# Symb0x76/ChineseChessZero

Hardware: AMD Instinct MI355X
Metric: self-play MCTS simulations/sec (higher is better)
Workload: dtype u8 rules / f32 Q (reference CPU path) / f64 PUCT (net: fp16)

## Files before the change

chinesechesszero_amd/_lib.py:

```python
from __future__ import annotations

import ctypes as C
import os

import torch

_HERE = os.path.dirname(os.path.abspath(__file__))
LIB_PATH = os.path.join(_HERE, "libcczero.so")

NSQ = 90
SQ_STRIDE = 96
NMOVES = 2086
MAX_LEGAL = 128
MASK_WORDS = 66
PLANES = 10710
REC_BYTES, REC_HDR, REC_IDS, REC_PI = 880, 96, 112, 368
REC_FLAGS, REC_FAST = 103, 1
REC_RESIGNED, REC_PLAYON, REC_VALUE = 2, 4, 8
REC_VALUE_OFF = 92
RESIGN_RESIGNED, RESIGN_PLAYON = 2, 4
HEAD_POL_STRIDE, HEAD_VAL_STRIDE = 1536, 640

ABI_VERSION = 9
CONV_RELU, CONV_DESCENDING, CONV_FORCE_SMALL, CONV_FORCE_TILE, CONV_G16, CONV_G16_EDGE_TILES = 1, 2, 16, 32, 64, 128
CONV_G16_ONE_LAUNCH = 512
CONV_G16_QUAD = 1 << 16
RULE_PERPETUAL_CHECK = 1
RULE_PAWN_MOVE_RESETS_CLOCK = 2
FLAG_REFERENCE_QUIRKS = 1
FLAG_NO_MIRROR = 2
FLAG_VALUE_F16 = 4
FLAG_CACHE_VERIFY = 8
ERR_PRUNED, ERR_TRUNCATED = 256, 512
ERR_BAD_TEMP = 1024
FLAG_STRICT = 16
LEAF_EXPAND, LEAF_DRAW, LEAF_LOSS, LEAF_SKIP = 0, 1, 2, 3
LEAF_WIN = 4
PROOF_UNKNOWN, PROOF_WIN, PROOF_LOSS, PROOF_DRAW = 0, 1, 2, 3

ERR_BITS = {1: "node pool exhausted (raise max_nodes)", 2: "selection path deeper than max_depth", 64: "history chain overflow (> 128 positions since the last capture)",
            4: "more than 128 legal moves or pseudo-move overflow", 8: "pi record arena overflow",
            16: "forced move is not a legal move of the root, or nothing searched and nothing forced (that board neither recorded nor moved)", 32: "NaN priors",
            128: "index out of bounds (bounds-checked diagnostic build)",
            256: "strict mode: a kept subtree was pruned to fit the node pool (the reference's tree is unbounded: raise max_nodes)",
            512: "strict mode: a game was adjudicated at max_plies (the reference's game has no ply cap: raise max_plies)",
            1024: "a per-board temperature was NaN or <= 0 (that board neither recorded nor moved)"}


class CczError(RuntimeError):
    pass


class Config(C.Structure):
    _fields_ = [
        ("n_boards", C.c_int32), ("n_playout", C.c_int32), ("c_puct", C.c_float), ("eps", C.c_float),
        ("alpha", C.c_float), ("temp", C.c_float), ("max_nodes", C.c_int32), ("max_depth", C.c_int32),
        ("max_plies", C.c_int32), ("flags", C.c_uint32), ("seed", C.c_uint64), ("board_id_base", C.c_uint64),
        ("device", C.c_int32), ("reserve_nodes", C.c_int32),
        ("move_rank_host", C.c_void_p), ("plane_of_type", C.c_uint8 * 8), ("rule_flags", C.c_uint32), ("eval_cache_log2", C.c_uint32),
        ("type_rank", C.c_uint8 * 8),
    ]


class Stats(C.Structure):
    _fields_ = [
        ("sims", C.c_int64), ("moves", C.c_int64), ("games", C.c_int64), ("truncated_games", C.c_int64),
        ("nodes_peak", C.c_int64), ("depth_peak", C.c_int64), ("sum_depth", C.c_int64), ("sum_children", C.c_int64),
        ("expansions", C.c_int64), ("terminal_leaves", C.c_int64), ("error_flags", C.c_int32), ("reserved", C.c_int32),
        ("hbm_bytes", C.c_int64), ("pruned_subtrees", C.c_int64),
        ("cache_probes", C.c_int64), ("cache_hits", C.c_int64), ("cache_shared_rows", C.c_int64), ("cache_stores", C.c_int64),
        ("cache_verified", C.c_int64), ("cache_verify_mismatches", C.c_int64),
    ]


class ResignStats(C.Structure):
    _fields_ = [("resigned_games", C.c_int64), ("resigned_by_red", C.c_int64), ("resigned_plies", C.c_int64), ("playon_games", C.c_int64),
                ("playon_won", C.c_int64), ("playon_drawn", C.c_int64), ("playon_plies_after", C.c_int64)]


class ExplorationStats(C.Structure):
    _fields_ = [("explored_moves", C.c_int64), ("forced_selections", C.c_int64), ("visits_pruned", C.c_int64), ("children_pruned", C.c_int64)]


class GumbelStats(C.Structure):
    _fields_ = [("gumbel_moves", C.c_int64), ("considered_sum", C.c_int64), ("offvisit_moves", C.c_int64)]


class SearchCfg(C.Structure):
    _fields_ = [("enabled", C.c_int32), ("fpu_mode", C.c_int32), ("fpu_root_mode", C.c_int32), ("reserved", C.c_int32),
                ("fpu_value", C.c_double), ("fpu_root_value", C.c_double), ("c_base", C.c_double), ("c_factor", C.c_double)]


class WideStats(C.Structure):
    _fields_ = [("steps", C.c_int64), ("leaves", C.c_int64), ("collisions", C.c_int64), ("inflight_now", C.c_int64)]


class SolverStats(C.Structure):
    _fields_ = [("nodes_proven", C.c_int64), ("proven_stops", C.c_int64), ("roots_proven", C.c_int64)]


_P = C.c_void_p
PROTOTYPES = {
    "ccz_abi_version": (C.c_int, []),
    "ccz_last_error": (C.c_char_p, []),
    "ccz_device_count": (C.c_int, []),
    "ccz_action_table": (C.c_int, [_P, _P, _P]),
    "ccz_flip_map": (C.c_int, [_P]),
    "ccz_create": (C.c_int, [C.POINTER(Config), C.POINTER(_P)]),
    "ccz_destroy": (C.c_int, [_P]),
    "ccz_reset": (C.c_int, [_P, _P, _P]),
    "ccz_set_position": (C.c_int, [_P, _P, C.c_int32, _P, C.c_int32, C.c_int32]),
    "ccz_set_positions": (C.c_int, [_P, _P, _P, _P, _P, _P, _P, C.c_int32, _P, _P]),
    "ccz_reset_tree": (C.c_int, [_P, _P, _P]),
    "ccz_select_leaves": (C.c_int, [_P, _P, _P]),
    "ccz_zero_leaf_input": (C.c_int, [_P, _P, _P]),
    "ccz_expand_backup": (C.c_int, [_P, _P, _P, _P]),
    "ccz_step": (C.c_int, [_P, _P, _P, _P, _P]),
    "ccz_gather_priors": (C.c_int, [_P, _P, _P, C.c_int32]),
    "ccz_step_compact": (C.c_int, [_P, _P, _P, _P]),
    "ccz_expand_backup_compact": (C.c_int, [_P, _P, _P]),
    "ccz_eval_plan": (C.c_int, [_P, _P, _P, _P]),
    "ccz_set_scouts": (C.c_int, [_P, C.c_int32]),
    "ccz_scout": (C.c_int, [_P, _P, _P]),
    "ccz_eval_plan_scouted": (C.c_int, [_P, _P, _P, _P, _P]),
    "ccz_scout_and_plan": (C.c_int, [_P, _P, _P, _P, _P, _P]),
    "ccz_scouted_run": (C.c_int, [_P, _P, _P, _P, _P, _P, _P]),
    "ccz_gather_priors_planned": (C.c_int, [_P, _P, _P, C.c_int32, _P]),
    "ccz_eval_cache_clear": (C.c_int, [_P, _P]),
    "ccz_set_routing": (C.c_int, [_P, _P, _P, C.c_uint64, C.c_uint64]),
    "ccz_eval_plan_routed": (C.c_int, [_P, _P, _P, _P]),
    "ccz_gather_priors_routed": (C.c_int, [_P, _P, _P, _P, C.c_int32, _P, _P]),
    "ccz_set_budgets": (C.c_int, [_P, _P, _P, _P]),
    "ccz_draw_budgets": (C.c_int, [_P, _P, C.c_int32, C.c_int32, C.c_double, _P]),
    "ccz_set_resign": (C.c_int, [_P, _P, C.c_int32, C.c_float, C.c_int32, C.c_int32, C.c_double]),
    "ccz_get_resign_stats": (C.c_int, [_P, _P, C.POINTER(ResignStats)]),
    "ccz_resign_status": (C.c_int, [_P, _P, _P, _P, _P, _P]),
    "ccz_set_root_exploration": (C.c_int, [_P, _P, C.c_int32, C.c_double, C.c_double, C.c_double, C.c_int32]),
    "ccz_get_exploration_stats": (C.c_int, [_P, _P, C.POINTER(ExplorationStats)]),
    "ccz_root_noise": (C.c_int, [_P, _P, _P, _P]),
    "ccz_set_gumbel": (C.c_int, [_P, _P, C.c_int32, C.c_int32, C.c_int32, C.c_double, C.c_double]),
    "ccz_get_gumbel_stats": (C.c_int, [_P, _P, C.POINTER(GumbelStats)]),
    "ccz_gumbel_root": (C.c_int, [_P, _P, _P, _P, _P, _P, _P]),
    "ccz_gumbel_sequence": (C.c_int, [_P, C.c_int32, C.c_int32, _P]),
    "ccz_set_search": (C.c_int, [_P, _P, C.c_int32, C.c_int32, C.c_double, C.c_int32, C.c_double, C.c_double, C.c_double]),
    "ccz_get_search": (C.c_int, [_P, _P, C.POINTER(SearchCfg)]),
    "ccz_set_solver": (C.c_int, [_P, _P, C.c_int32]),
    "ccz_root_proof": (C.c_int, [_P, _P, _P, _P, _P, _P]),
    "ccz_get_solver_stats": (C.c_int, [_P, _P, C.POINTER(SolverStats)]),
    "ccz_proof_combine": (C.c_int, [_P, _P, _P, C.c_int32, _P]),
    "ccz_set_width": (C.c_int, [_P, _P, C.c_int32]),
    "ccz_select_wide": (C.c_int, [_P, _P, _P, _P]),
    "ccz_step_wide": (C.c_int, [_P, _P, _P, _P, _P]),
    "ccz_get_wide_stats": (C.c_int, [_P, _P, C.POINTER(WideStats)]),
    "ccz_finish_move": (C.c_int, [_P, _P, _P, _P, _P, C.c_int32]),
    "ccz_root_children": (C.c_int, [_P, _P, _P, _P, _P, _P, _P, _P]),
    "ccz_principal_variations": (C.c_int, [_P, _P, C.c_int32, C.c_int32, _P, _P, _P, _P, _P, _P]),
    "ccz_root_pi": (C.c_int, [_P, _P, _P, _P]),
    "ccz_move_distribution": (C.c_int, [_P, _P, _P, _P, _P, _P]),
    "ccz_game_status": (C.c_int, [_P, _P, _P, _P, _P, _P]),
    "ccz_root_positions": (C.c_int, [_P, _P, _P]),
    "ccz_leaf_info": (C.c_int, [_P, _P, _P, _P, _P, _P]),
    "ccz_leaf_priors": (C.c_int, [_P, _P, _P, _P]),
    "ccz_leaf_keys": (C.c_int, [_P, _P, _P, _P]),
    "ccz_harvest_rows": (C.c_int, [_P, _P, C.POINTER(C.c_int64)]),
    "ccz_harvest": (C.c_int, [_P, _P, _P, _P, _P, C.c_int64, C.POINTER(C.c_int64)]),
    "ccz_harvest_records": (C.c_int, [_P, _P, _P, C.c_int64, C.POINTER(C.c_int64)]),
    "ccz_expand_records": (C.c_int, [_P, _P, C.c_int64, C.c_uint32, _P, _P, _P, _P, C.c_int64, C.c_int64, _P, _P, _P]),
    "ccz_ring_retire": (C.c_int, [_P, _P, C.c_int64, _P, C.c_int64, C.c_int32, _P]),
    "ccz_sample_records": (C.c_int, [_P, _P, C.c_int64, _P, _P, C.c_int64, C.c_uint32, _P, _P, _P, _P, _P, _P, _P]),
    "ccz_get_stats": (C.c_int, [_P, _P, C.POINTER(Stats)]),
    "ccz_legal_moves": (C.c_int, [_P, C.c_int32, _P, _P, _P, _P, _P, _P]),
    "ccz_apply_moves": (C.c_int, [_P, C.c_int32, _P, _P, _P, _P]),
    "ccz_bias_act_f16": (C.c_int, [_P, _P, _P, _P, C.c_int64, C.c_int32]),
    "ccz_conv3x3_c256_f16": (C.c_int, [_P, _P, _P, _P, _P, _P, C.c_int64, C.c_int32]),
    "ccz_conv3x3_stem_f16": (C.c_int, [_P, _P, _P, _P, _P, C.c_int64, C.c_int32]),
    "ccz_pack_live_planes_f16": (C.c_int, [_P, _P, _P, C.c_int32]),
    "ccz_pack_live_planes_rows_f16": (C.c_int, [_P, _P, _P, C.c_int32, _P, _P]),
    "ccz_pack_live_planes_g16_f16": (C.c_int, [_P, _P, _P, C.c_int32, _P, _P]),
    "ccz_pack_conv_weights_g16_f16": (C.c_int, [_P, _P, _P, C.c_int32]),
    "ccz_conv3x3_c256_f16_live": (C.c_int, [_P, _P, _P, _P, _P, _P, C.c_int64, C.c_int32, _P, C.c_int32, C.c_int32]),
    "ccz_conv3x3_stem_f16_live": (C.c_int, [_P, _P, _P, _P, _P, C.c_int64, C.c_int32, _P, C.c_int32, C.c_int32]),
    "ccz_conv3x3_c256_heads_f16": (C.c_int, [_P, _P, _P, _P, _P, _P, _P, _P, _P, C.c_int64, C.c_int32, _P, C.c_int32, C.c_int32]),
    "ccz_heads_conv1x1_f16": (C.c_int, [_P, _P, _P, _P, _P, _P, C.c_int32, C.c_int32, _P]),
    "ccz_fc_f16": (C.c_int, [_P, _P, C.c_int32, _P, _P, _P, C.c_int32, C.c_int32, C.c_int32, C.c_int32, C.c_int32, _P]),
    "ccz_value_out_f32": (C.c_int, [_P, _P, _P, C.c_float, _P, C.c_int32, _P]),
}

_lib = None


def source_hash() -> str | None:
    import glob
    import hashlib
    csrc = os.path.join(_HERE, "csrc")
    files = sorted(glob.glob(os.path.join(csrc, "*.h")) + glob.glob(os.path.join(csrc, "*.hip")), key=os.path.basename)
    files.append(os.path.join(os.path.dirname(_HERE), "include", "cczero.h"))
    if len(files) < 2 or not all(os.path.exists(f) for f in files):
        return None
    h = hashlib.sha256()
    for f in files:
        with open(f, "rb") as fh:
            h.update(fh.read())
    return h.hexdigest()[:16]


def stale_build() -> str | None:
    if LIB_PATH != os.path.join(_HERE, "libcczero.so"):
        return None
    want = source_hash()
    if want is None:
        return None
    stamp = LIB_PATH + ".srchash"
    if not os.path.exists(stamp):
        return f"{LIB_PATH} carries no source stamp ({stamp} is missing): it was not built by the current Makefile"
    with open(stamp) as f:
        got = f.read().strip()
    if got != want:
        return f"{LIB_PATH} was built from other sources (stamp {got}, the tree hashes to {want}): a kernel was edited after the last build"
    return None


def lib() -> C.CDLL:
    global _lib
    if _lib is None:
        if not os.path.exists(LIB_PATH):
            raise CczError(
                f"{LIB_PATH} is missing: build it with `python -c 'import __graft_entry__ as g; g.build()'` "
                "(hipcc --offload-arch=gfx950). The engine has no CPU fallback.")
        why = stale_build()
        if why:
            raise CczError(why + " -- rebuild with `python -c 'import __graft_entry__ as g; g.build()'`")
        L = C.CDLL(LIB_PATH)
        for name, (res, args) in PROTOTYPES.items():
            fn = getattr(L, name)
            fn.restype = res
            fn.argtypes = args
        if L.ccz_abi_version() != ABI_VERSION:
            raise CczError("libcczero.so ABI version mismatch")
        _lib = L
    return _lib


def check(rc: int) -> None:
    if rc != 0:
        raise CczError(f"libcczero error {rc}: {lib().ccz_last_error().decode(errors='replace')}")
```

chinesechesszero_amd/csrc/cczero.hip:

```cpp
#include "../../include/cczero.h"

#include <hip/hip_runtime.h>

#include <cmath>
#include <cstdarg>
#include <cstdio>
#include <cstdlib>
#include <cstring>
#include <new>
#include <vector>

#include "cczero_kernels.h"
#include "cczero_netops.h"
#include "cczero_conv.h"
#include "cczero_conv_small.h"
#include "cczero_conv_g16.h"
#include "cczero_conv_g16e.h"
#include "cczero_heads.h"

using namespace ccz;

namespace {

thread_local char g_err[512] = "";
// ... 1250 lines not shown
    HIP_TRY(hipStreamSynchronize(s));
    return 0;
}

int ccz_leaf_info(ccz_engine *e, void *stream, uint8_t *status_host, int32_t *k_host, uint16_t *ids_host, int32_t *depth_host)
{
    NEED(e);
    hipStream_t s = (hipStream_t)stream;
    const size_t B = (size_t)e->d.B;
    if (status_host) HIP_TRY(hipMemcpyAsync(status_host, e->d.leaf_status, B, hipMemcpyDeviceToHost, s));
    if (k_host) HIP_TRY(hipMemcpyAsync(k_host, e->d.leaf_k, B * 4, hipMemcpyDeviceToHost, s));
    if (ids_host) HIP_TRY(hipMemcpyAsync(ids_host, e->d.leaf_ids, B * kMaxLegal * 2, hipMemcpyDeviceToHost, s));
    if (depth_host) HIP_TRY(hipMemcpyAsync(depth_host, e->d.path_len, B * 4, hipMemcpyDeviceToHost, s));
    HIP_TRY(hipStreamSynchronize(s));
    return 0;
}

int ccz_leaf_priors(ccz_engine *e, void *stream, float *prior_host, float *value_host)
{
    NEED(e);
    hipStream_t s = (hipStream_t)stream;
    const size_t B = (size_t)e->d.B;
    if (value_host && !e->d.cache) return fail(-1, "ccz_leaf_priors: engine-owned leaf values exist only with an evaluation cache (pass value_host = NULL)");
    if (prior_host) HIP_TRY(hipMemcpyAsync(prior_host, e->d.prior128, B * kMaxLegal * 4, hipMemcpyDeviceToHost, s));
    if (value_host) HIP_TRY(hipMemcpyAsync(value_host, e->d.vleaf, B * 4, hipMemcpyDeviceToHost, s));
    HIP_TRY(hipStreamSynchronize(s));
    return 0;
}

int ccz_leaf_keys(ccz_engine *e, void *stream, uint64_t *keys_dev, uint8_t *status_dev)
{
    NEED(e);
    hipStream_t s = (hipStream_t)stream;
    if (keys_dev) HIP_TRY(hipMemcpyAsync(keys_dev, e->d.leaf_key, (size_t)e->d.B * 8, hipMemcpyDeviceToDevice, s));
    if (status_dev) HIP_TRY(hipMemcpyAsync(status_dev, e->d.leaf_status, (size_t)e->d.B, hipMemcpyDeviceToDevice, s));
    return 0;
}

int ccz_harvest_rows(ccz_engine *e, void *stream, int64_t *rows_host)
{
    NEED(e);
    if (!rows_host) return fail(-1, "ccz_harvest_rows: null output");
    const int rc = fetch_meta(e, (hipStream_t)stream);
    if (rc) return rc;
    const int mul = (e->d.flags & CCZ_FLAG_NO_MIRROR) ? 1 : 2;
    int64_t rows = 0;
    for (int b = 0; b < e->d.B; ++b)
        if (e->h_meta[b].over) rows += (int64_t)e->h_meta[b].ply * mul;
    *rows_host = rows;
    return 0;
}

struct HarvestPlan {
    std::vector<long long> base;
    std::vector<uint8_t> mask;
    int64_t total = 0;
    bool any = false;
};

static int plan_harvest(ccz_engine *e, hipStream_t s, int mul, int64_t capacity, const char *first_fmt, HarvestPlan &p)
{
    const int rc = fetch_meta(e, s);
    if (rc) return rc;
    const int B = e->d.B;
    p.base.assign((size_t)B, -1);
    p.mask.assign((size_t)B, 0);
    for (int b = 0; b < B; ++b)
        if (e->h_meta[b].over && e->h_meta[b].ply > 0) {
            const int64_t add = (int64_t)e->h_meta[b].ply * mul;
            if (p.total + add > capacity) {
                if (!p.any) return fail(-5, first_fmt, (long long)add, (long long)capacity);
                break;
            }
            p.base[b] = p.total;
            p.mask[b] = 1;
            p.any = true;
            p.total += add;
        }
    return 0;
}

static int restart_harvested(ccz_engine *e, hipStream_t s, const HarvestPlan &p)
{
    HIP_TRY(hipMemcpyAsync(e->st_mask, p.mask.data(), (size_t)e->d.B, hipMemcpyHostToDevice, s));
    hipLaunchKernelGGL(k_reset, dim3(e->d.B), dim3(64), 0, s, e->d, (const uint8_t *)e->st_mask);
    HIP_TRY(hipGetLastError());
    HIP_TRY(hipStreamSynchronize(s));
    return 0;
}

int ccz_harvest(ccz_engine *e, void *stream, void *states_f16_dev, float *pi_dev, float *z_dev, int64_t capacity_rows,
                int64_t *rows_host)
{
    NEED(e);
    hipStream_t s = (hipStream_t)stream;
    HarvestPlan p;
    const int rc = plan_harvest(e, s, (e->d.flags & CCZ_FLAG_NO_MIRROR) ? 1 : 2, capacity_rows,
                                "ccz_harvest: the first finished game needs %lld rows, capacity %lld", p);
    if (rc) return rc;
    if (rows_host) *rows_host = p.total;
    if (!p.any) return 0;
    if (p.total > 0) {
        if (!states_f16_dev || !pi_dev || !z_dev) return fail(-1, "ccz_harvest: null output buffer");
        HIP_TRY(hipMemcpyAsync(e->st_rowbase, p.base.data(), (size_t)e->d.B * 8, hipMemcpyHostToDevice, s));
        hipLaunchKernelGGL(k_harvest, dim3(e->d.B, kHarvestSlices), dim3(256), 0, s, e->d, (const long long *)e->st_rowbase,
                           (uint16_t *)states_f16_dev, pi_dev, z_dev);
        HIP_TRY(hipGetLastError());
    }
    return restart_harvested(e, s, p);
}

int ccz_harvest_records(ccz_engine *e, void *stream, void *records_dev, int64_t capacity_plies, int64_t *plies_host)
{
    NEED(e);
    hipStream_t s = (hipStream_t)stream;
    HarvestPlan p;
    if (const int rc = plan_harvest(e, s, 1, capacity_plies, "ccz_harvest_records: the first finished game has %lld plies, capacity %lld", p)) return rc;
    if (plies_host) *plies_host = p.total;
    if (!p.any) return 0;
    if (p.total > 0) {
        if (!records_dev) return fail(-1, "ccz_harvest_records: null output buffer");
        HIP_TRY(hipMemcpyAsync(e->st_rowbase, p.base.data(), (size_t)e->d.B * 8, hipMemcpyHostToDevice, s));
        hipLaunchKernelGGL(k_harvest_records, dim3(e->d.B, kHarvestSlices), dim3(256), 0, s, e->d, (const long long *)e->st_rowbase, (uint8_t *)records_dev);
        HIP_TRY(hipGetLastError());
    }
    return restart_harvested(e, s, p);
}

static int typepack_of(const char *who, const uint8_t *plane_of_type_host, uint32_t *typepack)
{
    uint8_t pot[8] = {0, 0, 1, 2, 3, 4, 5, 6};
    if (plane_of_type_host) {
        bool all_zero = true;
        for (int t = 0; t < 8; ++t) all_zero = all_zero && plane_of_type_host[t] == 0;
        if (!all_zero) {
            unsigned seen = 0;
            for (int t = 1; t <= 7; ++t) {
                const int c = plane_of_type_host[t];
                if (c > 6 || (seen >> c & 1u)) return fail(-1, "%s: plane_of_type[1..7] must be a permutation of 0..6", who);
                seen |= 1u << c;
                pot[t] = (uint8_t)c;
            }
        }
    }
    *typepack = 0;
    for (int t = 1; t <= 7; ++t) *typepack |= (uint32_t)(t - 1) << (3 * pot[t]);
    return 0;
}

static int check_expand_args(const char *who, const void *records_dev, int64_t n_plies, uint32_t flags, const void *states_f16_dev, const float *value_dev,
                             int64_t ring_rows, int64_t head_row)
{
    if (!records_dev) return fail(-1, "%s: null buffer", who);
    if (((uintptr_t)records_dev | (uintptr_t)states_f16_dev) & 3) return fail(-1, "%s: buffers must be 4-byte aligned", who);
    if ((uintptr_t)value_dev & 3) return fail(-1, "%s: the values must be 4-byte aligned", who);
    if (n_plies > (int64_t)INT32_MAX) return fail(-1, "%s: too many records for one launch", who);
    const int64_t rows = n_plies * ((flags & CCZ_FLAG_NO_MIRROR) ? 1 : 2);
    if (ring_rows > 0 && rows > ring_rows) return fail(-1, "%s: %lld rows do not fit a ring of %lld", who, (long long)rows, (long long)ring_rows);
    if (ring_rows == 0 && head_row != 0) return fail(-1, "%s: head_row needs ring_rows", who);
    return 0;
}

static int check_sample_args(const char *who, const void *ring_dev, const int64_t *window_dev, const int64_t *draws_dev, int64_t batch,
                             const void *states_f16_dev, const float *pi_dev, const float *z_dev, const float *value_dev)
{
    if (!ring_dev || !window_dev || !draws_dev || !states_f16_dev || !pi_dev || !z_dev) return fail(-1, "%s: null buffer", who);
    if (((uintptr_t)ring_dev | (uintptr_t)states_f16_dev) & 3) return fail(-1, "%s: buffers must be 4-byte aligned", who);
    if ((uintptr_t)value_dev & 3) return fail(-1, "%s: the values must be 4-byte aligned", who);
    if (((uintptr_t)window_dev | (uintptr_t)draws_dev) & 7) return fail(-1, "%s: window and draws must be 8-byte aligned", who);
    if (batch > (int64_t)INT32_MAX) return fail(-1, "%s: too many rows for one launch", who);
    return 0;
}

int ccz_expand_records(void *stream, const void *records_dev, int64_t n_plies, uint32_t flags, const uint8_t *plane_of_type_host,
                       void *states_f16_dev, float *pi_dev, float *z_dev, int64_t ring_rows, int64_t head_row, int32_t *bad_records_dev,
                       uint8_t *target_dev, float *value_dev)
{
    const char *who = "ccz_expand_records";
    if (n_plies < 0 || ring_rows < 0 || head_row < 0) return fail(-1, "%s: negative size", who);
    if (n_plies == 0) return 0;
    const int dense = (states_f16_dev != nullptr) + (pi_dev != nullptr) + (z_dev != nullptr);
    if (dense != 3 && !(dense == 0 && (target_dev || value_dev))) return fail(-1, "%s: null buffer", who);
    if (const int rc = check_expand_args(who, records_dev, n_plies, flags, states_f16_dev, value_dev, ring_rows, head_row)) return rc;
    uint32_t typepack = 0;
    if (const int rc = typepack_of(who, plane_of_type_host, &typepack)) return rc;
    hipLaunchKernelGGL(k_expand_records, dim3((unsigned)n_plies), dim3(256), 0, (hipStream_t)stream, (const uint8_t *)records_dev, (long long)n_plies,
                       flags & (CCZ_FLAG_REFERENCE_QUIRKS | CCZ_FLAG_NO_MIRROR), typepack, (uint16_t *)states_f16_dev, pi_dev, z_dev,
                       (long long)ring_rows, (long long)head_row, bad_records_dev, target_dev, value_dev);
    HIP_TRY(hipGetLastError());
    return 0;
}

int ccz_ring_retire(void *stream, const void *ring_dev, int64_t cap_plies, int64_t *window_dev, int64_t head_new, int32_t max_game_plies,
                    int32_t *bad_records_dev)
{
    if (cap_plies <= 0 || head_new < 0) return fail(-1, "ccz_ring_retire: capacity must be positive and head_new non-negative");
    if (max_game_plies <= 0 || max_game_plies > 65535) return fail(-1, "ccz_ring_retire: max_game_plies must be 1..65535 (the header's T is 16 bits)");
    if (cap_plies < 2 * (int64_t)max_game_plies) return fail(-1, "ccz_ring_retire: a ring of %lld plies is smaller than two games of %d", (long long)cap_plies, max_game_plies);
    if (!ring_dev || !window_dev) return fail(-1, "ccz_ring_retire: null buffer");
    if (((uintptr_t)ring_dev & 3) || ((uintptr_t)window_dev & 7)) return fail(-1, "ccz_ring_retire: the ring must be 4-byte, the window 8-byte aligned");
    hipLaunchKernelGGL(k_ring_retire, dim3(1), dim3(64), 0, (hipStream_t)stream, (const uint8_t *)ring_dev, (long long)cap_plies,
                       (long long *)window_dev, (long long)head_new, (int)max_game_plies, bad_records_dev);
    HIP_TRY(hipGetLastError());
    return 0;
}

int ccz_sample_records(void *stream, const void *ring_dev, int64_t cap_plies, const int64_t *window_dev, const int64_t *draws_dev, int64_t batch,
                       uint32_t flags, const uint8_t *plane_of_type_host, void *states_f16_dev, float *pi_dev, float *z_dev, int32_t *bad_records_dev,
                       uint8_t *target_dev, float *value_dev)
{
    const char *who = "ccz_sample_records";
    if (cap_plies <= 0 || batch < 0) return fail(-1, "%s: capacity must be positive and batch non-negative", who);
    if (batch == 0) return 0;
    if (const int rc = check_sample_args(who, ring_dev, window_dev, draws_dev, batch, states_f16_dev, pi_dev, z_dev, value_dev)) return rc;
    uint32_t typepack = 0;
    if (const int rc = typepack_of(who, plane_of_type_host, &typepack)) return rc;
    hipLaunchKernelGGL(k_sample_records, dim3((unsigned)batch), dim3(256), 0, (hipStream_t)stream, (const uint8_t *)ring_dev, (long long)cap_plies,
                       (const long long *)window_dev, (const long long *)draws_dev, (long long)batch,
                       flags & (CCZ_FLAG_REFERENCE_QUIRKS | CCZ_FLAG_NO_MIRROR), typepack, (uint16_t *)states_f16_dev, pi_dev, z_dev, bad_records_dev,
                       target_dev, value_dev);
    HIP_TRY(hipGetLastError());
    return 0;
}

int ccz_get_stats(ccz_engine *e, void *stream, ccz_stats *out)
{
    NEED(e);
    if (!out) return fail(-1, "ccz_get_stats: null output");
    hipStream_t s = (hipStream_t)stream;
    std::vector<BoardStats> st((size_t)e->d.B);
    int32_t err[2] = {0, 0};
    HIP_TRY(hipMemcpyAsync(st.data(), e->d.stats, st.size() * sizeof(BoardStats), hipMemcpyDeviceToHost, s));
    HIP_TRY(hipMemcpyAsync(err, e->d.err, 8, hipMemcpyDeviceToHost, s));
    HIP_TRY(hipStreamSynchronize(s));
    memset(out, 0, sizeof *out);
    for (const BoardStats &b : st) {
        out->sims += (int64_t)b.sims;
        out->moves += (int64_t)b.moves;
        out->games += (int64_t)b.games;
        out->truncated_games += (int64_t)b.truncated;
        out->sum_depth += (int64_t)b.sum_depth;
        out->sum_children += (int64_t)b.sum_children;
        out->expansions += (int64_t)b.expansions;
        out->terminal_leaves += (int64_t)b.terminal;
        out->pruned_subtrees += (int64_t)b.pruned;
        out->cache_probes += (int64_t)b.cache_probes;
        out->cache_hits += (int64_t)b.cache_hits;
        out->cache_shared_rows += (int64_t)b.cache_shared;
        out->cache_stores += (int64_t)b.cache_stores;
        out->cache_verified += (int64_t)b.cache_verified;
        out->cache_verify_mismatches += (int64_t)b.cache_mismatch;
        if (b.nodes_peak > out->nodes_peak) out->nodes_peak = b.nodes_peak;
        if (b.depth_peak > out->depth_peak) out->depth_peak = b.depth_peak;
    }
    out->error_flags = err[0];
    out->reserved = err[1];
    out->hbm_bytes = (int64_t)e->bytes;
    return 0;
}

int ccz_legal_moves(void *stream, int32_t n, const uint8_t *sq_dev, const uint8_t *turn_dev, const int32_t *halfmove_dev,
                    uint32_t *mask_dev, int32_t *count_dev, uint8_t *flags_dev)
{
    if (n < 0 || !sq_dev || !turn_dev) return fail(-1, "ccz_legal_moves: bad arguments");
    if (n == 0) return 0;
    hipLaunchKernelGGL(k_legal_moves, dim3(n), dim3(64), 0, (hipStream_t)stream, n, sq_dev, turn_dev, halfmove_dev, mask_dev,
                       count_dev, flags_dev);
    HIP_TRY(hipGetLastError());
    return 0;
}

int ccz_apply_moves(void *stream, int32_t n, uint8_t *sq_dev, uint8_t *turn_dev, const int32_t *move_ids_dev, uint8_t *captured_dev)
{
    if (n < 0 || !sq_dev || !turn_dev || !move_ids_dev) return fail(-1, "ccz_apply_moves: bad arguments");
    if (n == 0) return 0;
    hipLaunchKernelGGL(k_apply_moves, dim3((n + 255) / 256), dim3(256), 0, (hipStream_t)stream, n, sq_dev, turn_dev, move_ids_dev,
                       captured_dev);
    HIP_TRY(hipGetLastError());
    return 0;
}

int ccz_bias_act_f16(void *stream, void *y_dev, const void *bias_dev, const void *residual_dev, int64_t rows, int32_t channels)
{
    if (!y_dev || !bias_dev || rows < 0 || channels <= 0 || (channels & 7)) return fail(-1, "ccz_bias_act_f16: bad arguments (channels must be a multiple of 8)");
    if ((((uintptr_t)y_dev) | ((uintptr_t)bias_dev) | ((uintptr_t)residual_dev)) & 15) return fail(-1, "ccz_bias_act_f16: pointers must be 16-byte aligned");
    const long n_vec = rows * (long)(channels / 8);
    if (n_vec == 0) return 0;
    long blocks = (n_vec + 255) / 256;
    if (blocks > 4096) blocks = 4096;
    if (residual_dev)
        hipLaunchKernelGGL(k_bias_act<true>, dim3((unsigned)blocks), dim3(256), 0, (hipStream_t)stream, (half8_t *)y_dev, (const half8_t *)bias_dev,
                           (const half8_t *)residual_dev, n_vec, channels / 8);
    else
        hipLaunchKernelGGL(k_bias_act<false>, dim3((unsigned)blocks), dim3(256), 0, (hipStream_t)stream, (half8_t *)y_dev, (const half8_t *)bias_dev,
                           (const half8_t *)nullptr, n_vec, channels / 8);
    HIP_TRY(hipGetLastError());
    return 0;
}

static_assert(((int64_t)INT32_MAX / kCvC) * kCvC * 2 <= (int64_t)UINT32_MAX, "the largest accepted activation tensor must fit 32-bit byte offsets / num_records");
constexpr int64_t kSmallMaxPixels = 64 * 90;

static int conv3x3_launch(const char *who, void *stream, const void *x_dev, const void *w_dev, const void *bias_f32_dev, const void *residual_dev, void *y_dev,
                          int64_t n_pixels, int32_t relu, int cin, const int32_t *live_rows_dev = nullptr, int32_t row0 = 0)
{
    if (!x_dev || !w_dev || !bias_f32_dev || !y_dev || n_pixels < 0 || n_pixels % 90 || n_pixels > (int64_t)INT32_MAX / kCvC)
        return fail(-1, "%s: bad arguments (n_pixels must be boards * 90, at most 93206 boards per call)", who);
    if ((((uintptr_t)x_dev) | ((uintptr_t)w_dev) | ((uintptr_t)bias_f32_dev) | ((uintptr_t)residual_dev) | ((uintptr_t)y_dev)) & 15)
        return fail(-1, "%s: pointers must be 16-byte aligned", who);
    if (x_dev == y_dev) return fail(-1, "%s: the output may alias the residual but not the input", who);
    if (n_pixels == 0) return 0;
    if (relu & CCZ_CONV_G16) {
        if (relu & (256 | (0xffe << 16)))
            return fail(-1, "%s: flag 256 / bits 17..27 were CCZ_CONV_G16_PERSISTENT, retired in ABI 8", who);
        if (n_pixels % 1440) return fail(-1, "%s: CCZ_CONV_G16 needs a multiple of 16 boards", who);
        const int groups = (int)(n_pixels / 1440);
        const int fl = relu & 3;
        hipStream_t s = (hipStream_t)stream;
        const G16Shape shape = g16_shape(groups, relu);
        const G16Args a = {(const _Float16 *)x_dev, (const _Float16 *)w_dev, (const float *)bias_f32_dev, (const _Float16 *)residual_dev, (_Float16 *)y_dev,
                           (int)n_pixels, cin, (const int *)live_rows_dev, (int)row0};
        const bool res = residual_dev != nullptr;
        if (cin == 64) {
            hipLaunchKernelGGL(k_conv3x3_g16_stem, dim3((unsigned)(groups * 5)), dim3(512), 0, s, (const _Float16 *)x_dev, (const _Float16 *)w_dev,
                               (const float *)bias_f32_dev, (_Float16 *)y_dev, (int)n_pixels, (int)fl, cin, (const int *)live_rows_dev, (int)row0);
            HIP_TRY(hipGetLastError());
            return 0;
        }
        if (!shape.edge) {
            g16_launch(CCZ_G16_RES(k_conv3x3_g16, res), shape.mid, s, a, fl);
            HIP_TRY(hipGetLastError());
            return 0;
        }
        const bool quad = (relu & CCZ_CONV_G16_QUAD) != 0;
        if (relu & CCZ_CONV_G16_ONE_LAUNCH) {
            g16_launch(quad ? CCZ_G16_RES(k_conv3x3_g16_one_quad, res) : CCZ_G16_RES(k_conv3x3_g16_one, res), shape.mid + shape.edge, s, a, fl);
            HIP_TRY(hipGetLastError());
            return 0;
        }
        if (quad) g16_launch(CCZ_G16_RES(k_conv3x3_g16_quad, res), shape.mid, s, a, fl);
        else g16_launch(CCZ_G16_RES(k_conv3x3_g16, res), shape.mid, s, a, fl | 4);
        HIP_TRY(hipGetLastError());
        g16_launch(CCZ_G16_RES(k_conv3x3_g16_edge, res), shape.edge, s, a, fl);
        HIP_TRY(hipGetLastError());
        return 0;
    }
    if (!live_rows_dev && !(relu & 32) && ((relu & 16) || n_pixels <= kSmallMaxPixels)) {
        const dim3 grid((unsigned)((n_pixels + kSmPix - 1) / kSmPix), 16);
        const int rl = relu & 1;
#define CCZ_SMALL(RES_, CIN_)                                                                                                  \
        hipLaunchKernelGGL((k_conv3x3_small<RES_, CIN_>), grid, dim3(256), 0, (hipStream_t)stream, (const _Float16 *)x_dev, (const _Float16 *)w_dev, \
                           (const float *)bias_f32_dev, (const _Float16 *)residual_dev, (_Float16 *)y_dev, (int)n_pixels, rl)
        if (cin == 64) CCZ_SMALL(false, 64);
        else if (residual_dev) CCZ_SMALL(true, 256);
        else CCZ_SMALL(false, 256);
#undef CCZ_SMALL
        HIP_TRY(hipGetLastError());
        return 0;
    }
    const unsigned tiles = (unsigned)((n_pixels + kCvBM - 1) / kCvBM);
#ifndef CCZ_STAMPS
    relu &= 3;
#endif
    if (residual_dev)
        hipLaunchKernelGGL(k_conv3x3_c256<true>, dim3(tiles), dim3(512), 0, (hipStream_t)stream, (const _Float16 *)x_dev, (const _Float16 *)w_dev,
                           (const float *)bias_f32_dev, (const _Float16 *)residual_dev, (_Float16 *)y_dev, (int)n_pixels, (int)relu, cin, (const int *)live_rows_dev, (int)row0);
    else
        hipLaunchKernelGGL(k_conv3x3_c256<false>, dim3(tiles), dim3(512), 0, (hipStream_t)stream, (const _Float16 *)x_dev, (const _Float16 *)w_dev,
                           (const float *)bias_f32_dev, (const _Float16 *)nullptr, (_Float16 *)y_dev, (int)n_pixels, (int)relu, cin, (const int *)live_rows_dev, (int)row0);
    HIP_TRY(hipGetLastError());
    return 0;
}

int ccz_conv3x3_c256_f16(void *stream, const void *x_dev, const void *w_dev, const void *bias_f32_dev, const void *residual_dev, void *y_dev,
                         int64_t n_pixels, int32_t relu)
{
    return conv3x3_launch("ccz_conv3x3_c256_f16", stream, x_dev, w_dev, bias_f32_dev, residual_dev, y_dev, n_pixels, relu, 256);
}

int ccz_conv3x3_c256_heads_f16(void *stream, const void *x_dev, const void *w_dev, const void *bias_f32_dev, const void *residual_dev,
                               const void *head_w32_dev, const void *head_b32_dev, void *pol_dev, void *val_dev, int64_t n_pixels, int32_t flags,
                               const int32_t *live_rows_dev, int32_t part, int32_t n_parts)
{
    const char *who = "ccz_conv3x3_c256_heads_f16";
    if (!x_dev || !w_dev || !bias_f32_dev || !residual_dev || !head_w32_dev || !head_b32_dev || !pol_dev || !val_dev || n_pixels < 0 || n_pixels % 1440 ||
        n_pixels > (int64_t)INT32_MAX / kCvC)
        return fail(-1, "%s: bad arguments (n_pixels must be a multiple of 16 boards * 90, at most 93200 boards per call)", who);
    if (!(flags & CCZ_CONV_G16)) return fail(-1, "%s: rows must be in the group-of-16 layout (CCZ_CONV_G16)", who);
    if ((((uintptr_t)x_dev) | ((uintptr_t)w_dev) | ((uintptr_t)bias_f32_dev) | ((uintptr_t)residual_dev) | ((uintptr_t)head_w32_dev) | ((uintptr_t)head_b32_dev)) & 15)
        return fail(-1, "%s: pointers must be 16-byte aligned", who);
    if ((((uintptr_t)pol_dev) | ((uintptr_t)val_dev)) & 1) return fail(-1, "%s: outputs must be 2-byte aligned", who);
    if (live_rows_dev && g16_bad_part(part, n_parts)) return fail(-1, "%s: bad part / n_parts", who);
    if (n_pixels == 0) return 0;
    const G16Shape shape = g16_shape((int)(n_pixels / 1440), flags);
    const int fl = flags & 3;
    const G16Args a = {(const _Float16 *)x_dev, (const _Float16 *)w_dev, (const float *)bias_f32_dev, (const _Float16 *)residual_dev, nullptr,
                       (int)n_pixels, 256, (const int *)live_rows_dev, live_rows_dev ? (part | (n_parts << 16)) : 0};
    G5Heads ha;
    ha.w32 = (const _Float16 *)head_w32_dev;
    ha.b32 = (const float *)head_b32_dev;
    ha.pol = (_Float16 *)pol_dev;
    ha.val = (_Float16 *)val_dev;
    ha.nb = (int)(n_pixels / 90);
    hipStream_t s = (hipStream_t)stream;
    g16_launch(k_conv3x3_g16_heads, shape.mid, s, a, shape.edge ? fl | 4 : fl, ha);
    HIP_TRY(hipGetLastError());
    if (!shape.edge) return 0;
    g16_launch(k_conv3x3_g16_edge_heads, shape.edge, s, a, fl, ha);
    HIP_TRY(hipGetLastError());
    return 0;
}

int ccz_conv3x3_stem_f16(void *stream, const void *x64_dev, const void *w_dev, const void *bias_f32_dev, void *y_dev, int64_t n_pixels, int32_t relu)
{
    return conv3x3_launch("ccz_conv3x3_stem_f16", stream, x64_dev, w_dev, bias_f32_dev, nullptr, y_dev, n_pixels, relu, 64);
}

int ccz_conv3x3_c256_f16_live(void *stream, const void *x_dev, const void *w_dev, const void *bias_f32_dev, const void *residual_dev, void *y_dev,
                              int64_t n_pixels, int32_t relu, const int32_t *live_rows_dev, int32_t part, int32_t n_parts)
{
    if (!live_rows_dev || g16_bad_part(part, n_parts)) return fail(-1, "ccz_conv3x3_c256_f16_live: null live-row count or bad part / n_parts");
    return conv3x3_launch("ccz_conv3x3_c256_f16_live", stream, x_dev, w_dev, bias_f32_dev, residual_dev, y_dev, n_pixels, relu, 256, live_rows_dev, part | (n_parts << 16));
}

int ccz_conv3x3_stem_f16_live(void *stream, const void *x64_dev, const void *w_dev, const void *bias_f32_dev, void *y_dev, int64_t n_pixels, int32_t relu,
                              const int32_t *live_rows_dev, int32_t part, int32_t n_parts)
{
    if (!live_rows_dev || g16_bad_part(part, n_parts)) return fail(-1, "ccz_conv3x3_stem_f16_live: null live-row count or bad part / n_parts");
    return conv3x3_launch("ccz_conv3x3_stem_f16_live", stream, x64_dev, w_dev, bias_f32_dev, nullptr, y_dev, n_pixels, relu, 64, live_rows_dev, part | (n_parts << 16));
}

int ccz_pack_live_planes_rows_f16(void *stream, const void *leaf_dev, void *x64_dev, int32_t n_boards, const int32_t *rows_dev, const int32_t *n_rows_dev)
{
    if (!leaf_dev || !x64_dev || n_boards < 0 || !rows_dev || !n_rows_dev) return fail(-1, "ccz_pack_live_planes_rows_f16: bad arguments");
    if ((uintptr_t)x64_dev & 15) return fail(-1, "ccz_pack_live_planes_rows_f16: output must be 16-byte aligned");
    if (n_boards == 0) return 0;
    hipLaunchKernelGGL(k_pack_live_planes, dim3((unsigned)n_boards), dim3(kPackThreads), 0, (hipStream_t)stream, (const _Float16 *)leaf_dev, (half8_t *)x64_dev, (int)n_boards,
                       (const int *)rows_dev, (const int *)n_rows_dev, 2);
    HIP_TRY(hipGetLastError());
    return 0;
}

int ccz_pack_conv_weights_g16_f16(void *stream, const void *w_dev, void *wp_dev, int32_t cin)
{
    if (!w_dev || !wp_dev || w_dev == wp_dev || (cin != 64 && cin != 256)) return fail(-1, "ccz_pack_conv_weights_g16_f16: bad arguments (cin must be 64 or 256, not in place)");
    if ((((uintptr_t)w_dev) | ((uintptr_t)wp_dev)) & 15) return fail(-1, "ccz_pack_conv_weights_g16_f16: pointers must be 16-byte aligned");
    const int n = 256 * 9 * (cin >> 3);
    hipLaunchKernelGGL(k_pack_conv_weights_g16, dim3((unsigned)((n + 255) / 256)), dim3(256), 0, (hipStream_t)stream, (const cv_half8 *)w_dev, (cv_half8 *)wp_dev, (int)cin);
    HIP_TRY(hipGetLastError());
    return 0;
}

int ccz_pack_live_planes_g16_f16(void *stream, const void *leaf_dev, void *x64_dev, int32_t n_boards, const int32_t *rows_dev, const int32_t *n_rows_dev)
{
    if (!leaf_dev || !x64_dev || n_boards < 0 || (!rows_dev) != (!n_rows_dev)) return fail(-1, "ccz_pack_live_planes_g16_f16: bad arguments");
    if ((uintptr_t)x64_dev & 15) return fail(-1, "ccz_pack_live_planes_g16_f16: output must be 16-byte aligned");
    if (n_boards == 0) return 0;
    hipLaunchKernelGGL(k_pack_live_planes, dim3((unsigned)n_boards), dim3(kPackThreads), 0, (hipStream_t)stream, (const _Float16 *)leaf_dev, (half8_t *)x64_dev, (int)n_boards,
                       (const int *)rows_dev, (const int *)n_rows_dev, rows_dev ? 3 : 1);
    HIP_TRY(hipGetLastError());
    return 0;
}

int ccz_pack_live_planes_f16(void *stream, const void *leaf_dev, void *x64_dev, int32_t n_boards)
{
    if (!leaf_dev || !x64_dev || n_boards < 0) return fail(-1, "ccz_pack_live_planes_f16: bad arguments");
    if ((uintptr_t)x64_dev & 15) return fail(-1, "ccz_pack_live_planes_f16: output must be 16-byte aligned");
    if (n_boards == 0) return 0;
    hipLaunchKernelGGL(k_pack_live_planes, dim3((unsigned)n_boards), dim3(kPackThreads), 0, (hipStream_t)stream, (const _Float16 *)leaf_dev, (half8_t *)x64_dev, (int)n_boards,
                       (const int *)nullptr, (const int *)nullptr, 0);
    HIP_TRY(hipGetLastError());
    return 0;
}

#ifdef CCZ_STAMPS
int ccz_debug_conv_stamps(unsigned long long *out_host)
{
    HIP_TRY(hipDeviceSynchronize());
    HIP_TRY(hipMemcpyFromSymbol(out_host, HIP_SYMBOL(g_cv_stamps), sizeof(unsigned long long) * 2048 * 2 * 16));
    return 0;
}
int ccz_debug_stamps(ccz_engine *e, void *stream, unsigned long long *out_host)
{
    NEED(e);
    hipStream_t s = (hipStream_t)stream;
    HIP_TRY(hipMemcpyAsync(out_host, e->d.stamps, (size_t)e->d.B * 16 * 8, hipMemcpyDeviceToHost, s));
    HIP_TRY(hipStreamSynchronize(s));
    return 0;
}
#endif

int ccz_heads_conv1x1_f16(void *stream, const void *x_dev, const void *w32_dev, const void *bias32_f32_dev, void *pol_dev, void *val_dev,
                          int32_t n_boards, int32_t flags, const int32_t *live_boards_dev)
{
    if (!x_dev || !w32_dev || !bias32_f32_dev || !pol_dev || !val_dev || n_boards < 0) return fail(-1, "ccz_heads_conv1x1_f16: bad arguments");
    if ((((uintptr_t)x_dev) | ((uintptr_t)w32_dev) | ((uintptr_t)bias32_f32_dev)) & 15) return fail(-1, "ccz_heads_conv1x1_f16: x, weights and bias must be 16-byte aligned");
    if (flags & ~CCZ_CONV_G16) return fail(-1, "ccz_heads_conv1x1_f16: unknown flags 0x%x", flags);
    const bool g16 = (flags & CCZ_CONV_G16) != 0;
    if (g16 && (n_boards & 15)) return fail(-1, "ccz_heads_conv1x1_f16: the group-of-16 layout holds whole groups of 16 boards (n_boards = %d)", n_boards);
    if (n_boards == 0) return 0;
    const long cells = ((long)n_boards * 90 + 15) / 16;
    const unsigned blocks = (unsigned)((cells + 3) / 4 < 768 ? (cells + 3) / 4 : 768);
    if (g16)
        hipLaunchKernelGGL(k_head_conv1x1<true>, dim3(blocks), dim3(256), 0, (hipStream_t)stream, (const _Float16 *)x_dev, (const _Float16 *)w32_dev,
                           (const float *)bias32_f32_dev, (_Float16 *)pol_dev, (_Float16 *)val_dev, (int)n_boards, (const int *)live_boards_dev);
    else
        hipLaunchKernelGGL(k_head_conv1x1<false>, dim3(blocks), dim3(256), 0, (hipStream_t)stream, (const _Float16 *)x_dev, (const _Float16 *)w32_dev,
                           (const float *)bias32_f32_dev, (_Float16 *)pol_dev, (_Float16 *)val_dev, (int)n_boards, (const int *)live_boards_dev);
    HIP_TRY(hipGetLastError());
    return 0;
}

int ccz_fc_f16(void *stream, const void *a_dev, int32_t lda, const void *w_dev, const void *bias_f32_dev, void *c_dev, int32_t ldc,
               int32_t m, int32_t n, int32_t k, int32_t relu, const int32_t *live_rows_dev)
{
    if (!a_dev || !w_dev || !bias_f32_dev || !c_dev || m < 0 || n <= 0 || k <= 0) return fail(-1, "ccz_fc_f16: bad arguments");
    if ((k & 63) || (lda & 7) || lda < k || (n & 1) || (ldc & 1) || ldc < n) return fail(-1, "ccz_fc_f16: k must be a multiple of 64, lda a multiple of 8 and >= k, n and ldc even, ldc >= n");
    if ((((uintptr_t)a_dev) | ((uintptr_t)w_dev) | ((uintptr_t)bias_f32_dev)) & 15 || ((uintptr_t)c_dev & 3)) return fail(-1, "ccz_fc_f16: a, w, bias must be 16-byte aligned, c 4-byte aligned");
    if (m == 0) return 0;
    if (!(relu & 2) && ((relu & 4) || (m >= 2048 && n >= 1024))) {
        const int wtiles = ((n + kFwBN - 1) / kFwBN) * ((m + kFwBM - 1) / kFwBM);
        const dim3 wgrid((unsigned)(8 * ((wtiles + 7) / 8)));
        if (relu & 1)
            hipLaunchKernelGGL(k_fc_wide_f16<true>, wgrid, dim3(512), 0, (hipStream_t)stream, (const _Float16 *)a_dev, (int)lda, (const _Float16 *)w_dev,
                               (const float *)bias_f32_dev, (_Float16 *)c_dev, (int)ldc, (int)m, (int)n, (int)k, (const int *)live_rows_dev, (int)(relu >> 8));
        else
            hipLaunchKernelGGL(k_fc_wide_f16<false>, wgrid, dim3(512), 0, (hipStream_t)stream, (const _Float16 *)a_dev, (int)lda, (const _Float16 *)w_dev,
                               (const float *)bias_f32_dev, (_Float16 *)c_dev, (int)ldc, (int)m, (int)n, (int)k, (const int *)live_rows_dev, (int)(relu >> 8));
        HIP_TRY(hipGetLastError());
        return 0;
    }
    if (m <= 16 && !(relu & 6)) {
        const dim3 sgrid((unsigned)((n + 15) / 16));
        if (relu & 1)
            hipLaunchKernelGGL(k_fc_skinny_f16<true>, sgrid, dim3(64), 0, (hipStream_t)stream, (const _Float16 *)a_dev, (int)lda, (const _Float16 *)w_dev,
                               (const float *)bias_f32_dev, (_Float16 *)c_dev, (int)ldc, (int)m, (int)n, (int)k, (const int *)live_rows_dev);
        else
            hipLaunchKernelGGL(k_fc_skinny_f16<false>, sgrid, dim3(64), 0, (hipStream_t)stream, (const _Float16 *)a_dev, (int)lda, (const _Float16 *)w_dev,
                               (const float *)bias_f32_dev, (_Float16 *)c_dev, (int)ldc, (int)m, (int)n, (int)k, (const int *)live_rows_dev);
        HIP_TRY(hipGetLastError());
        return 0;
    }
    const int tiles = ((n + kFcBN - 1) / kFcBN) * ((m + kFcBM - 1) / kFcBM);
    const dim3 grid((unsigned)(8 * ((tiles + 7) / 8)));
    if (relu & 1)
        hipLaunchKernelGGL(k_fc_f16<true>, grid, dim3(256), 0, (hipStream_t)stream, (const _Float16 *)a_dev, (int)lda, (const _Float16 *)w_dev,
                           (const float *)bias_f32_dev, (_Float16 *)c_dev, (int)ldc, (int)m, (int)n, (int)k, (const int *)live_rows_dev, (int)(relu >> 8));
    else
        hipLaunchKernelGGL(k_fc_f16<false>, grid, dim3(256), 0, (hipStream_t)stream, (const _Float16 *)a_dev, (int)lda, (const _Float16 *)w_dev,
                           (const float *)bias_f32_dev, (_Float16 *)c_dev, (int)ldc, (int)m, (int)n, (int)k, (const int *)live_rows_dev, (int)(relu >> 8));
    HIP_TRY(hipGetLastError());
    return 0;
}

int ccz_value_out_f32(void *stream, const void *h_dev, const void *w2_dev, float b2, float *v_dev, int32_t m, const int32_t *live_rows_dev)
{
    if (!h_dev || !w2_dev || !v_dev || m < 0) return fail(-1, "ccz_value_out_f32: bad arguments");
    if ((((uintptr_t)h_dev) | ((uintptr_t)w2_dev)) & 7) return fail(-1, "ccz_value_out_f32: h and w2 must be 8-byte aligned");
    if (m == 0) return 0;
    hipLaunchKernelGGL(k_value_out, dim3((unsigned)((m + 3) / 4)), dim3(256), 0, (hipStream_t)stream, (const _Float16 *)h_dev, (const _Float16 *)w2_dev, b2, v_dev,
                       (int)m, (const int *)live_rows_dev);
    HIP_TRY(hipGetLastError());
    return 0;
}

}
```

chinesechesszero_amd/csrc/cczero_conv_g16.h:

```cpp
#pragma once
#include "cczero_conv.h"

namespace ccz {

constexpr int kG5Rows = 288;
constexpr int kG5SlabRows = 576;
constexpr int kG5SlabBytes = kG5SlabRows * 64;
constexpr int kG5WBytes = 256 * 64;
constexpr int kG5Ring = 5, kG5Ahead = 3;
constexpr int kG5AOff = kG5Ring * kG5WBytes;
constexpr int kG5Dump = kG5AOff + 2 * kG5SlabBytes;
constexpr int kG5Lds = kG5Dump + 8 * 1024;
constexpr int kG5ERow = 528;
static_assert(kG5Rows * kG5ERow <= kG5Dump, "epilogue image must fit the operand buffers");
constexpr int kG5QRows = 576;
constexpr int kG5QSlabRows = 864;
constexpr int kG5QSlabBytes = kG5QSlabRows * 64;
constexpr int kG5QWBytes = 128 * 64;
constexpr int kG5QAOff = kG5Ring * kG5QWBytes;
constexpr int kG5QDump = kG5QAOff + 2 * kG5QSlabBytes;
constexpr int kG5QLds = kG5QDump + 8 * 1024;
constexpr int kG5QERow = 272;
static_assert(kG5QLds == 159744 && kG5QLds <= kG5Lds, "quad tile: ring + two slabs + dump must fit the workgroup's LDS");
static_assert(kG5QRows * kG5QERow == 156672 && kG5QRows * kG5QERow <= kG5QLds,
              "quad tile: the epilogue image covers the operand buffers AND most of the dump area (free once every DMA has landed)");

struct G5Ctx {
    unsigned char *lds;
    const _Float16 *X, *W;
    unsigned xbytes, wbytes;
    unsigned xbytes_part;
    unsigned xoff[5];
    unsigned xstep, whalf;
    unsigned woff;
    int zo[2], zd[2];
    int wave_dst;
    int lane16;
    int wave_dst_part, wave_step_part;
    int a_off;
    int vb[2];
    int cin, cmask;
};

__host__ __device__ constexpr bool g5_slab_tap(int t) { return t >= 1 && t <= 5; }
constexpr int kG5Split = 7;
__host__ __device__ constexpr int g5_dma(int t) { return 2 + (g5_slab_tap(t) ? 1 : 0); }
__host__ __device__ constexpr int g5_vmcnt(int t) { return g5_dma(t) + g5_dma(t - 1); }
static_assert(g5_vmcnt(0) == 4 && g5_vmcnt(1) == 5 && g5_vmcnt(2) == 6 && g5_vmcnt(3) == 6 && g5_vmcnt(4) == 6 && g5_vmcnt(5) == 6 &&
              g5_vmcnt(6) == 5 && g5_vmcnt(7) == 4 && g5_vmcnt(8) == 4, "g5_vmcnt table");
static_assert(g5_dma(0) == 2 && g5_dma(1) == 3 && g5_dma(2) == 3 && g5_dma(3) == 3 && g5_dma(4) == 3 && g5_dma(5) == 3 && g5_dma(6) == 2 &&
              g5_dma(7) == 2 && g5_dma(8) == 2, "23 DMA loads per chunk and thread: 5 slab pieces + 9 x 2 weight pieces");
__host__ __device__ constexpr int g5q_nslab(int t) { return t == 0 ? 2 : t <= 5 ? 1 : 0; }
__host__ __device__ constexpr int g5q_dma(int t) { return 1 + g5q_nslab(t); }
__host__ __device__ constexpr int g5q_vmcnt(int t) { return g5q_dma(t) + g5q_dma((t + 8) % 9); }
static_assert(g5q_vmcnt(0) == 4 && g5q_vmcnt(1) == 5 && g5q_vmcnt(2) == 4 && g5q_vmcnt(3) == 4 && g5q_vmcnt(4) == 4 && g5q_vmcnt(5) == 4 &&
              g5q_vmcnt(6) == 3 && g5q_vmcnt(7) == 2 && g5q_vmcnt(8) == 2, "g5q_vmcnt table");
static_assert(g5q_dma(0) == 3 && g5q_dma(1) == 2 && g5q_dma(2) == 2 && g5q_dma(3) == 2 && g5q_dma(4) == 2 && g5q_dma(5) == 2 && g5q_dma(6) == 1 &&
              g5q_dma(7) == 1 && g5q_dma(8) == 1, "16 DMA loads per chunk and thread: 7 slab pieces + 9 weight pieces");

template <int T, int N> __host__ __device__ constexpr bool g5_on_board()
{
    return !((T % 3 == 0 && N == 0) || (T % 3 == 2 && N == 8));
}

template <bool LDS_DONE = false> __device__ __forceinline__ void g5_barrier()
{
    if constexpr (LDS_DONE) asm volatile("s_waitcnt lgkmcnt(0)" ::: "memory");
    __builtin_amdgcn_sched_barrier(0);
    __builtin_amdgcn_s_barrier();
    __builtin_amdgcn_sched_barrier(0);
}

__device__ __forceinline__ void g5_zero_ranks(const G5Ctx &c, int buf)
{
    int l16 = c.lane16, zero = 0;
    asm volatile("" : "+v"(l16), "+v"(zero));
    typedef int g5_int4 __attribute__((ext_vector_type(4)));
    const g5_int4 z = {zero, zero, zero, zero};
#pragma unroll
    for (int j = 0; j < 2; ++j) *(g5_int4 *)(c.lds + (l16 + (c.zo[j] + buf * c.zd[j]))) = z;
    asm volatile("s_waitcnt lgkmcnt(0)" ::: "memory");
}

#define G5_CELL(TAP, N)                                                                                                   \
    {                                                                                                                     \
        if constexpr (TAP % 3 == 2)                                                                                       \
            b[N] = *(const cv_half8 *)(lds + c.vb[BUFn] + G5_REFILL(N) * 1024);                                           \
        if constexpr (g5_on_board<TAP, N>()) {                                                                            \
            constexpr int NB = N + TAP % 3 - 1;                                                                           \
            _Pragma("unroll") for (int i = 0; i < 4; ++i)                                                                 \
                acc[i][N] = __builtin_amdgcn_mfma_f32_16x16x32_f16(acur[i], b[NB], acc[i][N], 0, 0, 0);                   \
        }                                                                                                                 \
        __builtin_amdgcn_sched_barrier(0);                                                                                \
    }
#define G5_CELLS(TAP, LO, HI)                                                                                             \
    if constexpr (LO <= 0 && 0 < HI) G5_CELL(TAP, 0) if constexpr (LO <= 1 && 1 < HI) G5_CELL(TAP, 1) if constexpr (LO <= 2 && 2 < HI) G5_CELL(TAP, 2) \
    if constexpr (LO <= 3 && 3 < HI) G5_CELL(TAP, 3) if constexpr (LO <= 4 && 4 < HI) G5_CELL(TAP, 4) if constexpr (LO <= 5 && 5 < HI) G5_CELL(TAP, 5) \
    if constexpr (LO <= 6 && 6 < HI) G5_CELL(TAP, 6) if constexpr (LO <= 7 && 7 < HI) G5_CELL(TAP, 7) if constexpr (LO <= 8 && 8 < HI) G5_CELL(TAP, 8)

template <int J, bool Q = false>
__device__ __forceinline__ void g5_step(const G5Ctx &c, cv_f32x4 (&acc)[4][9], int chunk, int &ring_rd, int &ring_wr,
                                         cv_half8 (&a0)[4], cv_half8 (&a1)[4], cv_half8 (&b)[9])
{
    constexpr int T = J % 9, BUF = J / 9;
    constexpr int Tn = (T + 1) % 9, BUFn = (T == 8) ? 1 - BUF : BUF;
    constexpr int kWB = Q ? kG5QWBytes : kG5WBytes, kAOff = Q ? kG5QAOff : kG5AOff, kSlab = Q ? kG5QSlabBytes : kG5SlabBytes;
    cv_half8 (&acur)[4] = (J & 1) ? a1 : a0;
    cv_half8 (&anxt)[4] = (J & 1) ? a0 : a1;
    unsigned char *const lds = c.lds;

#define G5_REFILL(N) (9 + N + 9 * (Tn / 3 - 1))
    constexpr int T2 = (T + kG5Ahead) % 9;
    const int chunk2 = chunk + (T + kG5Ahead >= 9 ? 1 : 0);
    G5_CELLS(T, 0, 1)
    if constexpr (Q && g5q_nslab(T) > 0) {
        constexpr int pass = T == 0 ? 0 : T + 1;
        const unsigned so = (unsigned)((chunk + 1) * 64);
        const unsigned live = chunk < c.cmask ? (pass < 6 ? c.xbytes : c.xbytes_part) : 0u;
        cv_blds16(c.X, live, c.xoff[0], so + pass * c.xstep,
                  lds + (pass < 6 ? kAOff + (1 - BUF) * kSlab + pass * 8192 + c.wave_dst : c.wave_dst_part + (1 - BUF) * c.wave_step_part));
        if constexpr (g5q_nslab(T) > 1) cv_blds16(c.X, live, c.xoff[0], so + (pass + 1) * c.xstep, lds + kAOff + (1 - BUF) * kSlab + ((pass + 1) * 8192 + c.wave_dst));
        __builtin_amdgcn_sched_barrier(0);
    }
    if constexpr (!Q && g5_dma(T) > 2) {
        constexpr int pass = T - 1;
        const unsigned live = pass < 4 ? c.xbytes : c.xbytes_part;
        cv_blds16(c.X, chunk < c.cmask ? live : 0u, c.xoff[pass], (unsigned)((chunk + 1) * 64),
                  lds + (pass < 4 ? kG5AOff + (1 - BUF) * kG5SlabBytes + pass * 8192 + c.wave_dst : c.wave_dst_part + (1 - BUF) * c.wave_step_part));
        __builtin_amdgcn_sched_barrier(0);
    }
    G5_CELLS(T, 1, 2)
    if constexpr (Q) {
        cv_blds16(c.W, chunk2 <= c.cmask ? c.wbytes : 0u, c.woff, (unsigned)((T2 + 9 * chunk2) * (2 * 8192)) + c.whalf, lds + ring_wr * kWB + c.wave_dst);
        __builtin_amdgcn_sched_barrier(0);
        G5_CELLS(T, 2, 3)
    } else {
        const unsigned wlive = chunk2 <= c.cmask ? c.wbytes : 0u;
        const unsigned so = (unsigned)((T2 + 9 * chunk2) * (2 * 8192));
        unsigned char *const d = lds + ring_wr * kG5WBytes + c.wave_dst;
        cv_blds16(c.W, wlive, c.woff, so, d);
        __builtin_amdgcn_sched_barrier(0);
        G5_CELLS(T, 2, 3)
        cv_blds16(c.W, wlive, c.woff, so + 8192u, d + 8192);
        __builtin_amdgcn_sched_barrier(0);
    }
    G5_CELLS(T, 3, kG5Split)

    ring_rd = ring_rd + 1 == kG5Ring ? 0 : ring_rd + 1;
    cv_wait_vm<Q ? g5q_vmcnt(T) : g5_vmcnt(T)>();
    if constexpr (!Q && T == 7) g5_zero_ranks(c, 1 - BUF);
    g5_barrier();

    {
        const unsigned char *wa = lds + (ring_rd * kWB + c.a_off);
#pragma unroll
        for (int i = 0; i < 4; ++i) anxt[i] = *(const cv_half8 *)(wa + i * 1024);
        __builtin_amdgcn_sched_barrier(0);
    }
    G5_CELLS(T, kG5Split, 9)
    ring_wr = ring_wr + 1 == kG5Ring ? 0 : ring_wr + 1;
#undef G5_REFILL
}

struct G5Heads {
    const _Float16 *w32;
    const float *b32;
    _Float16 *pol, *val;
    int nb;
};

__device__ __forceinline__ void g5_heads_phase(const unsigned char *lds, int w, int lane, const G5Heads &ha, const long (&board0)[2],
                                               const int (&pos0)[2], bool skip1)
{
    const int r = lane & 15, q4 = lane >> 4;
    cv_half8 a[2][8];
#pragma unroll
    for (int m = 0; m < 2; ++m)
#pragma unroll
        for (int s = 0; s < 8; ++s) a[m][s] = *(const cv_half8 *)(ha.w32 + (m * 16 + r) * 256 + s * 32 + q4 * 8);
    const float4 b0 = *(const float4 *)(ha.b32 + 4 * q4), b1 = *(const float4 *)(ha.b32 + 16 + 4 * q4);
    for (int cell = w; cell < 18; cell += 8) {
        const unsigned char *row = lds + (cell * 16 + r) * kG5ERow + q4 * 16;
        cv_f32x4 acc0, acc1;
        acc0[0] = b0.x; acc0[1] = b0.y; acc0[2] = b0.z; acc0[3] = b0.w;
        acc1[0] = b1.x; acc1[1] = b1.y; acc1[2] = b1.z; acc1[3] = b1.w;
#pragma unroll
        for (int s = 0; s < 8; ++s) {
            const cv_half8 b = *(const cv_half8 *)(row + s * 64);
            acc0 = __builtin_amdgcn_mfma_f32_16x16x32_f16(a[0][s], b, acc0, 0, 0, 0);
            acc1 = __builtin_amdgcn_mfma_f32_16x16x32_f16(a[1][s], b, acc1, 0, 0, 0);
        }
        const int wnr = cell >= 9 ? 1 : 0, n = cell - 9 * wnr;
        const long board = board0[wnr] + r;
        if (board < ha.nb && !(skip1 && wnr)) {
            const int pos = pos0[wnr] + n;
            _Float16 *po = ha.pol + board * 1536 + pos * 17;
            _Float16 *vo = ha.val + board * 640 + pos * 7;
#pragma unroll
            for (int e = 0; e < 4; ++e) po[4 * q4 + e] = (_Float16)fmaxf(acc0[e], 0.0f);
            if (q4 == 0) {
                po[16] = (_Float16)fmaxf(acc1[0], 0.0f);
                vo[0] = (_Float16)fmaxf(acc1[1], 0.0f);
                vo[1] = (_Float16)fmaxf(acc1[2], 0.0f);
                vo[2] = (_Float16)fmaxf(acc1[3], 0.0f);
            } else if (q4 == 1) {
#pragma unroll
                for (int e = 0; e < 4; ++e) vo[3 + e] = (_Float16)fmaxf(acc1[e], 0.0f);
            }
        }
    }
}

__device__ __forceinline__ int g5_live_groups(const int *live_rows, int row0, int cap, int &first)
{
    const int part = row0 & 0xffff, n_parts = row0 >> 16;
    const int G = (*live_rows + 15) >> 4;
    const int per = (G + n_parts - 1) / n_parts;
    first = part * per;
    int live = G - first;
    live = live < 0 ? 0 : (live > per ? per : live);
    return live > cap ? cap : live;
}

template <bool RES, bool HEADS>
__device__ __forceinline__ void g5_live_part(int first, int cin, const _Float16 *__restrict__ &X, const _Float16 *&R, _Float16 *&Y, long &first_board)
{
    const long off = (long)first * 1440 * kCvC;
    X += (long)first * 1440 * cin;
    if (!HEADS) Y += off;
    if (RES) R += off;
    first_board = (long)first * 16;
}

__device__ __forceinline__ int g5_xcd_tile(int blk, int tiles, int flags)
{
    const int b = blk, x = b & 7, per = tiles >> 3, rem = tiles & 7;
    const int tile = x * per + (x < rem ? x : rem) + (b >> 3);
    return __builtin_amdgcn_readfirstlane((flags & 2) ? tiles - 1 - tile : tile);
}

__device__ __forceinline__ void g5_ctx_common(G5Ctx &c, unsigned char *lds, const _Float16 *X, const _Float16 *W, int w, unsigned xbytes, int cin, int chunks)
{
    c.lds = lds;
    c.X = X;
    c.W = W;
    c.wave_dst = w * 1024;
    c.cin = cin;
    c.cmask = chunks - 1;
    c.xbytes = xbytes;
    c.wbytes = 9u * 256u * (unsigned)cin * 2u;
}

__device__ __forceinline__ void g5_ctx_frags(G5Ctx &c, int r, int q4, int wm, int cell0, int aoff, int slab)
{
    const int lane1 = r * 64 + ((q4 ^ ((0 - (r >> 2)) & 3)) << 4);
    c.a_off = wm * 4096 + lane1;
    c.vb[0] = aoff + cell0 * 1024 + lane1;
    c.vb[1] = c.vb[0] + slab;
}

template <int EROW>
__device__ __forceinline__ void g5_image_store(unsigned char *lds, cv_f32x4 (&acc)[4][9], int wm, int wn, int r, int q4)
{
#pragma unroll
    for (int i = 0; i < 4; ++i) {
        const int col = wm * 64 + i * 16 + 4 * q4;
#pragma unroll
        for (int n = 0; n < 9; ++n) {
            cv_half4 o;
            o[0] = (_Float16)acc[i][n][0];
            o[1] = (_Float16)acc[i][n][1];
            o[2] = (_Float16)acc[i][n][2];
            o[3] = (_Float16)acc[i][n][3];
            *(cv_half4 *)(lds + ((wn * 9 + n) * 16 + r) * EROW + col * 2) = o;
        }
    }
}

template <int EROW, int STEP, bool RES, bool HEADS>
__device__ __forceinline__ void g5_rows_out(unsigned char *lds, int irow, int piece, long pbase, int gcol, _Float16 *Y, int relu, const cv_half8 (&rv)[18])
{
    const cv_half8 zero = (cv_half8)(_Float16)0;
    unsigned char *eb = lds + irow * EROW + piece * 16;
#pragma unroll
    for (int it = 0; it < 18; ++it) {
        cv_half8 v = *(const cv_half8 *)(eb + it * STEP * EROW);
        if (RES) v = v + rv[it];
        if (relu) v = __builtin_elementwise_max(v, zero);
        if constexpr (HEADS) *(cv_half8 *)(eb + it * STEP * EROW) = v;
        else *(cv_half8 *)(Y + (pbase + it * STEP) * kCvC + gcol) = v;
    }
}

__device__ __forceinline__ void g5_acc_row_from_bias(cv_f32x4 (&row)[9], const float *bias4)
{
    const float4 bv = *(const float4 *)bias4;
#pragma unroll
    for (int n = 0; n < 9; ++n) {
        row[n][0] = bv.x; row[n][1] = bv.y; row[n][2] = bv.z; row[n][3] = bv.w;
    }
}

template <bool RES, bool HEADS, bool ONE = false>
__device__ __forceinline__ void g5_tile(unsigned char *lds, int blk, int grid, const _Float16 *__restrict__ X, const _Float16 *__restrict__ W,
                                        const float *__restrict__ bias, const _Float16 *R,
                                        _Float16 *Y, int M, int relu, int cin, const int *live_rows, int row0, const G5Heads &ha)
{
    [[maybe_unused]] long first_board = 0;
    const int tid = threadIdx.x, lane = tid & 63;
    const int w = __builtin_amdgcn_readfirstlane(tid >> 6);
    const int r = lane & 15, q4 = lane >> 4;
    const int wm = w & 3, wn = w >> 2;
    int tiles = grid;
    if (live_rows) {
        int first;
        const int live = g5_live_groups(live_rows, row0, M / 1440, first);
        M = live * 1440;
        tiles = live * ((relu & 4) ? 4 : 5);
        if (blk >= tiles) return;
        g5_live_part<RES, HEADS>(first, cin, X, R, Y, first_board);
    }
    const int tile = g5_xcd_tile(blk, tiles, relu);
    const int mid = relu & 4;
    const int k = mid ? 2 : tile % 5;
    const long p0 = mid ? (long)(tile >> 2) * 1440 + 144 + (long)(tile & 3) * kG5Rows
                        : (long)tile * kG5Rows;
    relu &= 1;

    G5Ctx c;
    {
        const int piece[2] = {k == 0 ? 0 : k == 4 ? (w >= 3 ? 3 : 4) : -1, (k == 0 && w == 0) ? 1 : (k == 4 && w == 3) ? 4 : -1};
#pragma unroll
        for (int j = 0; j < 2; ++j) {
            c.zo[j] = __builtin_amdgcn_readfirstlane(piece[j] >= 0 ? kG5AOff + piece[j] * 8192 + w * 1024 : kG5Dump + w * 1024);
            c.zd[j] = __builtin_amdgcn_readfirstlane(piece[j] >= 0 ? kG5SlabBytes : 0);
        }
    }
    g5_ctx_common(c, lds, X, W, w, (unsigned)M * (unsigned)cin * 2u, cin, ONE ? 1 : cin >> 5);
    c.lane16 = lane * 16;
    c.wave_dst_part = w < 4 ? kG5AOff + 4 * 8192 + w * 1024 : kG5Dump + w * 1024;
    c.wave_step_part = w < 4 ? kG5SlabBytes : 0;
    c.xbytes_part = w < 4 ? c.xbytes : 0u;
    {
#pragma unroll
        for (int it = 0; it < 5; ++it) {
            const int piece = (it < 4 || w < 4) ? it * 512 + tid : 3 * 512 + tid;
            const int sr = piece >> 2, pos = piece & 3;
            const int schunk = pos ^ ((0 - (sr >> 2)) & 3);
            long p = p0 - 144 + sr;
            p = p < 0 ? 0 : (p > (long)M - 1 ? (long)M - 1 : p);
            c.xoff[it] = (unsigned)(p * cin + schunk * 8) * 2u;
        }
        c.woff = (unsigned)(tid * 16);
    }
#pragma unroll
    for (int it = 0; it < 5; ++it)
        cv_blds16(X, it < 4 ? c.xbytes : c.xbytes_part, c.xoff[it], 0u, lds + (it < 4 ? kG5AOff + it * 8192 + c.wave_dst : c.wave_dst_part));
#pragma unroll
    for (int u = 0; u < kG5Ahead; ++u) {
        unsigned char *d = lds + u * kG5WBytes + c.wave_dst;
        cv_blds16(W, c.wbytes, c.woff, (unsigned)(u * 2 * 8192), d);
        cv_blds16(W, c.wbytes, c.woff, (unsigned)(u * 2 * 8192 + 8192), d + 8192);
    }
    g5_ctx_frags(c, r, q4, wm, wn * 9, kG5AOff, kG5SlabBytes);

    cv_f32x4 acc[4][9];
#pragma unroll
    for (int i = 0; i < 4; ++i) g5_acc_row_from_bias(acc[i], bias + wm * 64 + i * 16 + 4 * q4);

    cv_wait_vm<4>();
    g5_zero_ranks(c, 0);
    g5_barrier<true>();

    int ring_rd = 0, ring_wr = kG5Ahead;
    cv_half8 a0[4], a1[4], b[9];
#pragma unroll
    for (int i = 0; i < 4; ++i) a0[i] = *(const cv_half8 *)(lds + c.a_off + i * 1024);
#pragma unroll
    for (int n = 0; n < 9; ++n) b[n] = *(const cv_half8 *)(lds + c.vb[0] + (9 + n - 9) * 1024);
#define G5_S(j) g5_step<j>(c, acc, chunk + (j) / 9, ring_rd, ring_wr, a0, a1, b)
    if constexpr (ONE) {
        const int chunk = 0;
        G5_S(0); G5_S(1); G5_S(2); G5_S(3); G5_S(4); G5_S(5); G5_S(6); G5_S(7); G5_S(8);
    } else {
        for (int chunk = 0; chunk <= c.cmask; chunk += 2) {
            G5_S(0); G5_S(1); G5_S(2); G5_S(3); G5_S(4); G5_S(5); G5_S(6); G5_S(7); G5_S(8);
            G5_S(9); G5_S(10); G5_S(11); G5_S(12); G5_S(13); G5_S(14); G5_S(15); G5_S(16); G5_S(17);
        }
    }
#undef G5_S
    cv_wait_vm<0>();

    g5_barrier();
    const int lane_e = (int)__builtin_amdgcn_mbcnt_hi(~0u, __builtin_amdgcn_mbcnt_lo(~0u, 0u));
    const int re = lane_e & 15, q4e = lane_e >> 4;
    const int prow = lane_e >> 5, piece = lane_e & 31;
    const long pbase = p0 + w * 36 + prow;
    cv_half8 rv[18];
    g5_image_store<kG5ERow>(lds, acc, wm, wn, re, q4e);
    if (RES) {
#pragma unroll
        for (int it = 0; it < 18; ++it) rv[it] = *(const cv_half8 *)(R + (pbase + it * 2) * kCvC + piece * 8);
    }
    g5_barrier<true>();
    g5_rows_out<kG5ERow, 2, RES, HEADS>(lds, w * 36 + prow, piece, pbase, piece * 8, Y, relu, rv);
    if constexpr (HEADS) {
        g5_barrier<true>();
        const long grp = p0 / 1440;
        const int rank0 = (int)((p0 - grp * 1440) / 144);
        const long board0[2] = {first_board + grp * 16, first_board + grp * 16};
        const int pos0[2] = {rank0 * 9, rank0 * 9 + 9};
        g5_heads_phase(lds, w, lane_e, ha, board0, pos0, false);
    }
}

template <bool RES>
__device__ __forceinline__ void g5q_tile(unsigned char *lds, int blk, int grid, const _Float16 *__restrict__ X, const _Float16 *__restrict__ W,
                                         const float *__restrict__ bias, const _Float16 *R, _Float16 *Y, int M, int relu, int cin,
                                         const int *live_rows, int row0)
{
    const int tid = threadIdx.x, lane = tid & 63;
    const int w = __builtin_amdgcn_readfirstlane(tid >> 6);
    const int r = lane & 15, q4 = lane >> 4;
    const int wm = w & 1, wn = w >> 1;
    int tiles = grid;
    if (live_rows) {
        int first;
        const int live = g5_live_groups(live_rows, row0, M / 1440, first);
        M = live * 1440;
        tiles = live * 4;
        if (blk >= tiles) return;
        long first_board;
        g5_live_part<RES, false>(first, cin, X, R, Y, first_board);
    }
    const int tile = g5_xcd_tile(blk, tiles, relu);
    const int h = tile & 1;
    const long p0 = (long)(tile >> 2) * 1440 + 144 + (long)((tile >> 1) & 1) * kG5QRows;
    relu &= 1;

    G5Ctx c;
    g5_ctx_common(c, lds, X, W, w, (unsigned)M * (unsigned)cin * 2u, cin, cin >> 5);
    c.wave_dst_part = w < 6 ? kG5QAOff + 6 * 8192 + w * 1024 : kG5QDump + w * 1024;
    c.wave_step_part = w < 6 ? kG5QSlabBytes : 0;
    c.xbytes_part = w < 6 ? c.xbytes : 0u;
    c.xstep = 128u * (unsigned)cin * 2u;
    c.whalf = (unsigned)h * 8192u;
    {
        const int sr = tid >> 2, pos = tid & 3;
        const int schunk = pos ^ ((0 - (sr >> 2)) & 3);
        c.xoff[0] = (unsigned)((p0 - 144 + sr) * cin + schunk * 8) * 2u;
        c.woff = (unsigned)(tid * 16);
    }
#pragma unroll
    for (int it = 0; it < 7; ++it)
        cv_blds16(X, it < 6 ? c.xbytes : c.xbytes_part, c.xoff[0], it * c.xstep, lds + (it < 6 ? kG5QAOff + it * 8192 + c.wave_dst : c.wave_dst_part));
#pragma unroll
    for (int u = 0; u < kG5Ahead; ++u) cv_blds16(W, c.wbytes, c.woff, (unsigned)(u * 2 * 8192) + c.whalf, lds + u * kG5QWBytes + c.wave_dst);
    g5_ctx_frags(c, r, q4, wm, wn * 9, kG5QAOff, kG5QSlabBytes);

    cv_f32x4 acc[4][9];
#pragma unroll
    for (int i = 0; i < 4; ++i) g5_acc_row_from_bias(acc[i], bias + h * 128 + wm * 64 + i * 16 + 4 * q4);

    cv_wait_vm<2>();
    g5_barrier();

    int ring_rd = 0, ring_wr = kG5Ahead;
    cv_half8 a0[4], a1[4], b[9];
#pragma unroll
    for (int i = 0; i < 4; ++i) a0[i] = *(const cv_half8 *)(lds + c.a_off + i * 1024);
#pragma unroll
    for (int n = 0; n < 9; ++n) b[n] = *(const cv_half8 *)(lds + c.vb[0] + n * 1024);
    for (int chunk = 0; chunk <= c.cmask; chunk += 2) {
#define G5Q_S(j) g5_step<j, true>(c, acc, chunk + (j) / 9, ring_rd, ring_wr, a0, a1, b)
        G5Q_S(0); G5Q_S(1); G5Q_S(2); G5Q_S(3); G5Q_S(4); G5Q_S(5); G5Q_S(6); G5Q_S(7); G5Q_S(8);
        G5Q_S(9); G5Q_S(10); G5Q_S(11); G5Q_S(12); G5Q_S(13); G5Q_S(14); G5Q_S(15); G5Q_S(16); G5Q_S(17);
#undef G5Q_S
    }
    cv_wait_vm<0>();

    g5_barrier();
    const int lane_e = (int)__builtin_amdgcn_mbcnt_hi(~0u, __builtin_amdgcn_mbcnt_lo(~0u, 0u));
    const int re = lane_e & 15, q4e = lane_e >> 4;
    const int prow = lane_e >> 4, piece = lane_e & 15;
    const long pbase = p0 + w * 72 + prow;
    const int gcol = h * 128 + piece * 8;
    cv_half8 rv[18];
    g5_image_store<kG5QERow>(lds, acc, wm, wn, re, q4e);
    if (RES) {
#pragma unroll
        for (int it = 0; it < 18; ++it) rv[it] = *(const cv_half8 *)(R + (pbase + it * 4) * kCvC + gcol);
    }
    g5_barrier<true>();
    g5_rows_out<kG5QERow, 4, RES, false>(lds, w * 72 + prow, piece, pbase, gcol, Y, relu, rv);
}

template <bool RES>
__global__ __launch_bounds__(512) void k_conv3x3_g16(const _Float16 *__restrict__ X, const _Float16 *__restrict__ W,
                                                         const float *__restrict__ bias, const _Float16 *R,
                                                         _Float16 *Y, int M, int relu, int cin, const int *live_rows, int row0)
{
    __shared__ __attribute__((aligned(16))) unsigned char lds[kG5Lds];
    g5_tile<RES, false>(lds, blockIdx.x, gridDim.x, X, W, bias, R, Y, M, relu, cin, live_rows, row0, G5Heads{});
}

template <bool RES>
__global__ __launch_bounds__(512) void k_conv3x3_g16_quad(const _Float16 *__restrict__ X, const _Float16 *__restrict__ W,
                                                            const float *__restrict__ bias, const _Float16 *R,
                                                            _Float16 *Y, int M, int relu, int cin, const int *live_rows, int row0)
{
    __shared__ __attribute__((aligned(16))) unsigned char lds[kG5Lds];
    g5q_tile<RES>(lds, blockIdx.x, gridDim.x, X, W, bias, R, Y, M, relu, cin, live_rows, row0);
}

__global__ __launch_bounds__(512) void k_conv3x3_g16_stem(const _Float16 *__restrict__ X, const _Float16 *__restrict__ W,
                                                            const float *__restrict__ bias, _Float16 *Y, int M, int relu, int cin,
                                                            const int *live_rows, int row0)
{
    __shared__ __attribute__((aligned(16))) unsigned char lds[kG5Lds];
    g5_tile<false, false, true>(lds, blockIdx.x, gridDim.x, X, W, bias, nullptr, Y, M, relu, cin, live_rows, row0, G5Heads{});
}

__global__ __launch_bounds__(512) void k_conv3x3_g16_heads(const _Float16 *__restrict__ X, const _Float16 *__restrict__ W,
                                                             const float *__restrict__ bias, const _Float16 *R, _Float16 *Y, int M,
                                                             int relu, int cin, const int *live_rows, int row0, G5Heads ha)
{
    __shared__ __attribute__((aligned(16))) unsigned char lds[kG5Lds];
    if (live_rows) ha.nb = *live_rows;
    g5_tile<true, true>(lds, blockIdx.x, gridDim.x, X, W, bias, R, Y, M, relu, cin, live_rows, row0, ha);
}

__global__ __launch_bounds__(256) void k_pack_conv_weights_g16(const cv_half8 *__restrict__ w, cv_half8 *__restrict__ wp, int cin)
{
    const int n = 256 * 9 * (cin >> 3);
    const int i = blockIdx.x * 256 + threadIdx.x;
    if (i >= n) return;
    const int pos = i & 3, co = (i >> 2) & 255, h = i >> 10, tap = h % 9, c32 = h / 9;
    const int chunk = pos ^ ((0 - (co >> 2)) & 3);
    wp[i] = w[(co * 9 + tap) * (cin >> 3) + c32 * 4 + chunk];
}

}
```

chinesechesszero_amd/csrc/cczero_conv_g16e.h:

```cpp
#pragma once
#include "cczero_conv_g16.h"

namespace ccz {

__host__ __device__ constexpr int g5e_nslab(int h) { return h == 0 ? 2 : h == 1 ? 2 : h == 2 ? 1 : 0; }
__host__ __device__ constexpr int g5e_dma(int h) { return 2 + g5e_nslab(h); }
__host__ __device__ constexpr int g5e_vmcnt(int h) { return g5e_dma(h) + g5e_dma((h + 5) % 6); }
static_assert(g5e_vmcnt(0) == 6 && g5e_vmcnt(1) == 8 && g5e_vmcnt(2) == 7 && g5e_vmcnt(3) == 5 && g5e_vmcnt(4) == 4 && g5e_vmcnt(5) == 4, "g5e_vmcnt table");
static_assert(g5e_dma(0) == 4 && g5e_dma(1) == 4 && g5e_dma(2) == 3 && g5e_dma(3) == 2 && g5e_dma(4) == 2 && g5e_dma(5) == 2,
              "17 DMA loads per chunk and thread: 5 slab pieces + 6 x 2 weight pieces");

template <int J>
__device__ __forceinline__ void g5e_step(const G5Ctx &c, cv_f32x4 (&acc)[4][9], int chunk, int &ring_rd, int &ring_wr,
                                          cv_half8 (&a0)[4], cv_half8 (&a1)[4], cv_half8 (&b)[9], int toff)
{
    constexpr int H = J % 6, BUF = J / 6;
    constexpr int Hn = (H + 1) % 6, BUFn = (H == 5) ? 1 - BUF : BUF;
    cv_half8 (&acur)[4] = (J & 1) ? a1 : a0;
    cv_half8 (&anxt)[4] = (J & 1) ? a0 : a1;
    unsigned char *const lds = c.lds;
#define G5_REFILL(N) ((Hn / 3) * 9 + N)
    constexpr int H2 = (H + kG5Ahead) % 6;
    const int chunk2 = chunk + (H + kG5Ahead >= 6 ? 1 : 0);
    G5_CELLS(H, 0, 1)
    if constexpr (g5e_dma(H) > 2) {
        constexpr int p0 = H * 2;
        const unsigned so = (unsigned)((chunk + 1) * 64);
        const unsigned live = chunk < c.cmask ? (p0 < 4 ? c.xbytes : c.xbytes_part) : 0u;
        cv_blds16(c.X, live, c.xoff[p0], so,
                  lds + (p0 < 4 ? kG5AOff + (1 - BUF) * kG5SlabBytes + p0 * 8192 + c.wave_dst : c.wave_dst_part + (1 - BUF) * c.wave_step_part));
        if constexpr (g5e_dma(H) > 3)
            cv_blds16(c.X, live, c.xoff[p0 + 1], so, lds + kG5AOff + (1 - BUF) * kG5SlabBytes + ((p0 + 1) * 8192 + c.wave_dst));
        __builtin_amdgcn_sched_barrier(0);
    }
    G5_CELLS(H, 1, 2)
    {
        const unsigned wlive = chunk2 <= c.cmask ? c.wbytes : 0u;
        const unsigned so = (unsigned)((H2 + toff + 9 * chunk2) * (2 * 8192));
        unsigned char *const d = lds + ring_wr * kG5WBytes + c.wave_dst;
        cv_blds16(c.W, wlive, c.woff, so, d);
        __builtin_amdgcn_sched_barrier(0);
        G5_CELLS(H, 2, 3)
        cv_blds16(c.W, wlive, c.woff, so + 8192u, d + 8192);
        __builtin_amdgcn_sched_barrier(0);
    }
    G5_CELLS(H, 3, kG5Split)

    ring_rd = ring_rd + 1 == kG5Ring ? 0 : ring_rd + 1;
    cv_wait_vm<g5e_vmcnt(H)>();
    g5_barrier();

    {
        const unsigned char *wa = lds + (ring_rd * kG5WBytes + c.a_off);
#pragma unroll
        for (int i = 0; i < 4; ++i) anxt[i] = *(const cv_half8 *)(wa + i * 1024);
        __builtin_amdgcn_sched_barrier(0);
    }
    G5_CELLS(H, kG5Split, 9)
    ring_wr = ring_wr + 1 == kG5Ring ? 0 : ring_wr + 1;
#undef G5_REFILL
}

template <bool RES, bool HEADS>
__device__ __forceinline__ void g5e_tile(unsigned char *lds, int blk, const _Float16 *__restrict__ X, const _Float16 *__restrict__ W,
                                         const float *__restrict__ bias, const _Float16 *R, _Float16 *Y, int M,
                                         int relu, int cin, const int *live_rows, int row0, const G5Heads &ha)
{
    [[maybe_unused]] long first_board = 0;
    const int tid = threadIdx.x, lane = tid & 63;
    const int w = __builtin_amdgcn_readfirstlane(tid >> 6);
    const int r = lane & 15, q4 = lane >> 4;
    const int wm = w & 3, wn = w >> 2;
    int groups = M / 1440;
    if (live_rows) {
        int first;
        groups = g5_live_groups(live_rows, row0, groups, first);
        g5_live_part<RES, HEADS>(first, cin, X, R, Y, first_board);
    }
    const int e = __builtin_amdgcn_readfirstlane(blk);
    if (e >= 2 * ((groups + 1) >> 1)) return;
    const int side = e & 1, gA = (e >> 1) * 2;
    const bool dup = gA + 1 >= groups;
    const int gB = dup ? gA : gA + 1;
    const int toff = __builtin_amdgcn_readfirstlane(side ? 0 : 3);
    const long srcA = (long)gA * 1440 + (side ? 8 : 0) * 144;
    const long srcB = (long)gB * 1440 + (side ? 8 : 0) * 144;
    const long outA = (long)gA * 1440 + (side ? 9 : 0) * 144;
    const long outB = (long)gB * 1440 + (side ? 9 : 0) * 144;
    relu &= 1;

    G5Ctx c;
    g5_ctx_common(c, lds, X, W, w, (unsigned)groups * (1440u * 2u) * (unsigned)cin, cin, cin >> 5);
    c.wave_dst_part = w < 4 ? kG5AOff + 4 * 8192 + w * 1024 : kG5Dump + w * 1024;
    c.wave_step_part = w < 4 ? kG5SlabBytes : 0;
    c.xbytes_part = w < 4 ? c.xbytes : 0u;
    {
#pragma unroll
        for (int it = 0; it < 5; ++it) {
            const int piece = (it < 4 || w < 4) ? it * 512 + tid : 3 * 512 + tid;
            const int sr = piece >> 2, pos = piece & 3;
            const int schunk = pos ^ ((0 - (sr >> 2)) & 3);
            const long p = sr < 288 ? srcA + sr : srcB + (sr - 288);
            c.xoff[it] = (unsigned)(p * cin + schunk * 8) * 2u;
        }
        c.woff = (unsigned)(tid * 16);
    }
#pragma unroll
    for (int it = 0; it < 5; ++it)
        cv_blds16(X, it < 4 ? c.xbytes : c.xbytes_part, c.xoff[it], 0u, lds + (it < 4 ? kG5AOff + it * 8192 + c.wave_dst : c.wave_dst_part));
#pragma unroll
    for (int u = 0; u < kG5Ahead; ++u) {
        unsigned char *d = lds + u * kG5WBytes + c.wave_dst;
        cv_blds16(W, c.wbytes, c.woff, (unsigned)((u + toff) * 2 * 8192), d);
        cv_blds16(W, c.wbytes, c.woff, (unsigned)((u + toff) * 2 * 8192 + 8192), d + 8192);
    }
    g5_ctx_frags(c, r, q4, wm, wn * 18, kG5AOff, kG5SlabBytes);

    cv_f32x4 acc[4][9];
#pragma unroll
    for (int i = 0; i < 4; ++i) g5_acc_row_from_bias(acc[i], bias + wm * 64 + i * 16 + 4 * q4);

    cv_wait_vm<4>();
    g5_barrier();

    int ring_rd = 0, ring_wr = kG5Ahead;
    cv_half8 a0[4], a1[4], b[9];
#pragma unroll
    for (int i = 0; i < 4; ++i) a0[i] = *(const cv_half8 *)(lds + c.a_off + i * 1024);
#pragma unroll
    for (int n = 0; n < 9; ++n) b[n] = *(const cv_half8 *)(lds + c.vb[0] + n * 1024);
    for (int chunk = 0; chunk <= c.cmask; chunk += 2) {
#define G5E_S(j) g5e_step<j>(c, acc, chunk + (j) / 6, ring_rd, ring_wr, a0, a1, b, toff)
        G5E_S(0); G5E_S(1); G5E_S(2); G5E_S(3); G5E_S(4); G5E_S(5);
        G5E_S(6); G5E_S(7); G5E_S(8); G5E_S(9); G5E_S(10); G5E_S(11);
#undef G5E_S
    }
    cv_wait_vm<0>();

    g5_barrier();
    g5_image_store<kG5ERow>(lds, acc, wm, wn, r, q4);
    const int prow = lane >> 5, piece = lane & 31;
    const long pbase = (w < 4 ? outA : outB) + (w & 3) * 36 + prow;
    const bool store = !(dup && w >= 4);
    cv_half8 rv[18];
    if (RES) {
#pragma unroll
        for (int it = 0; it < 18; ++it) rv[it] = *(const cv_half8 *)(R + (pbase + it * 2) * kCvC + piece * 8);
    }
    g5_barrier<true>();
    if (store) {
        const cv_half8 zero = (cv_half8)(_Float16)0;
        unsigned char *eb = lds + (w * 36 + prow) * kG5ERow + piece * 16;
#pragma unroll
        for (int it = 0; it < 18; ++it) {
            cv_half8 v = *(const cv_half8 *)(eb + it * 2 * kG5ERow);
            if (RES) v = v + rv[it];
            if (relu) v = __builtin_elementwise_max(v, zero);
            if constexpr (HEADS) *(cv_half8 *)(eb + it * 2 * kG5ERow) = v;
            else *(cv_half8 *)(Y + (pbase + it * 2) * kCvC + piece * 8) = v;
        }
    }
    if constexpr (HEADS) {
        g5_barrier<true>();
        const long board0[2] = {first_board + (long)gA * 16, first_board + (long)gB * 16};
        const int pos0[2] = {side ? 81 : 0, side ? 81 : 0};
        g5_heads_phase(lds, w, lane, ha, board0, pos0, dup);
    }
}

template <bool RES>
__global__ __launch_bounds__(512) void k_conv3x3_g16_edge(const _Float16 *__restrict__ X, const _Float16 *__restrict__ W,
                                                            const float *__restrict__ bias, const _Float16 *R, _Float16 *Y, int M,
                                                            int relu, int cin, const int *live_rows, int row0)
{
    __shared__ __attribute__((aligned(16))) unsigned char lds[kG5Lds];
    g5e_tile<RES, false>(lds, blockIdx.x, X, W, bias, R, Y, M, relu, cin, live_rows, row0, G5Heads{});
}

__global__ __launch_bounds__(512) void k_conv3x3_g16_edge_heads(const _Float16 *__restrict__ X, const _Float16 *__restrict__ W,
                                                                  const float *__restrict__ bias, const _Float16 *R, _Float16 *Y,
                                                                  int M, int relu, int cin, const int *live_rows, int row0, G5Heads ha)
{
    __shared__ __attribute__((aligned(16))) unsigned char lds[kG5Lds];
    if (live_rows) ha.nb = *live_rows;
    g5e_tile<true, true>(lds, blockIdx.x, X, W, bias, R, Y, M, relu, cin, live_rows, row0, ha);
}

template <bool RES, bool QUAD>
__device__ __forceinline__ void g5_one_launch(unsigned char *lds, const _Float16 *__restrict__ X, const _Float16 *__restrict__ W,
                                              const float *__restrict__ bias, const _Float16 *R, _Float16 *Y, int M,
                                              int relu, int cin, const int *live_rows, int row0)
{
    int groups = M / 1440;
    if (live_rows) {
        int first;
        groups = g5_live_groups(live_rows, row0, groups, first);
    }
    const int mid = groups * 4, blk = blockIdx.x;
    if (blk < mid) {
        if constexpr (QUAD) g5q_tile<RES>(lds, blk, mid, X, W, bias, R, Y, M, relu, cin, live_rows, row0);
        else g5_tile<RES, false>(lds, blk, mid, X, W, bias, R, Y, M, relu | 4, cin, live_rows, row0, G5Heads{});
    } else g5e_tile<RES, false>(lds, blk - mid, X, W, bias, R, Y, M, relu, cin, live_rows, row0, G5Heads{});
}

template <bool RES>
__global__ __launch_bounds__(512) void k_conv3x3_g16_one(const _Float16 *__restrict__ X, const _Float16 *__restrict__ W,
                                                           const float *__restrict__ bias, const _Float16 *R, _Float16 *Y, int M,
                                                           int relu, int cin, const int *live_rows, int row0)
{
    __shared__ __attribute__((aligned(16))) unsigned char lds[kG5Lds];
    g5_one_launch<RES, false>(lds, X, W, bias, R, Y, M, relu, cin, live_rows, row0);
}

template <bool RES>
__global__ __launch_bounds__(512) void k_conv3x3_g16_one_quad(const _Float16 *__restrict__ X, const _Float16 *__restrict__ W,
                                                                const float *__restrict__ bias, const _Float16 *R, _Float16 *Y, int M,
                                                                int relu, int cin, const int *live_rows, int row0)
{
    __shared__ __attribute__((aligned(16))) unsigned char lds[kG5Lds];
    g5_one_launch<RES, true>(lds, X, W, bias, R, Y, M, relu, cin, live_rows, row0);
}

#undef G5_CELLS
#undef G5_CELL

}
```

chinesechesszero_amd/net.py:

```python
from __future__ import annotations

import ctypes as C
import os

import numpy as np
import torch
import torch.nn.functional as F
from torch import nn

PIECES = 7
PLAYS = 17


class ResBlock(nn.Module):

    def __init__(self, num_channels=256):
        super().__init__()
        self.conv1 = nn.Conv2d(num_channels, num_channels, kernel_size=(3, 3), stride=(1, 1), padding=1)
        self.conv1_bn = nn.BatchNorm2d(num_channels)
        self.conv1_act = nn.ReLU()
        self.conv2 = nn.Conv2d(num_channels, num_channels, kernel_size=(3, 3), stride=(1, 1), padding=1)
        self.conv2_bn = nn.BatchNorm2d(num_channels)
        self.conv2_act = nn.ReLU()

    def forward(self, x):
        y = self.conv1_act(self.conv1_bn(self.conv1(x)))
        y = self.conv2_bn(self.conv2(y))
        return self.conv2_act(x + y)


class Net(nn.Module):

    def __init__(self, num_channels=256, resblocks_num=40):
        super().__init__()
        self.input_channels = PLAYS * PIECES
        self.conv_block = nn.Conv2d(self.input_channels, num_channels, kernel_size=(3, 3), stride=(1, 1), padding=1)
        self.conv_block_bn = nn.BatchNorm2d(num_channels)
        self.conv_block_act = nn.ReLU()
        self.res_blocks = nn.ModuleList([ResBlock(num_channels=num_channels) for _ in range(resblocks_num)])
        self.policy_conv = nn.Conv2d(num_channels, PLAYS, kernel_size=(1, 1), stride=(1, 1))
        self.policy_bn = nn.BatchNorm2d(PLAYS)
        self.policy_act = nn.ReLU()
        self.policy_fc = nn.Linear(PLAYS * 10 * 9, 2086)
        self.value_conv = nn.Conv2d(num_channels, PIECES, kernel_size=(1, 1), stride=(1, 1))
        self.value_bn = nn.BatchNorm2d(PIECES)
        self.value_act1 = nn.ReLU()
        self.value_fc1 = nn.Linear(PIECES * 10 * 9, 256)
        self.value_act2 = nn.ReLU()
        self.value_fc2 = nn.Linear(256, 1)

    def forward(self, x):
        x = x.view(x.shape[0], -1, 10, 9)
        x = self.conv_block_act(self.conv_block_bn(self.conv_block(x)))
        for blk in self.res_blocks:
            x = blk(x)
        policy = self.policy_act(self.policy_bn(self.policy_conv(x)))
        policy = F.log_softmax(self.policy_fc(torch.reshape(policy, [-1, PLAYS * 10 * 9])), dim=1)
        value = self.value_act1(self.value_bn(self.value_conv(x)))
        value = self.value_act2(self.value_fc1(torch.reshape(value, [-1, PIECES * 10 * 9])))
        value = torch.tanh(self.value_fc2(value))
        return policy, value


def _fold(conv: nn.Conv2d, bn: nn.BatchNorm2d):
    scale = bn.weight.detach().double() / torch.sqrt(bn.running_var.detach().double() + bn.eps)
    w = conv.weight.detach().double() * scale.view(-1, 1, 1, 1)
    b = (conv.bias.detach().double() - bn.running_mean.detach().double()) * scale + bn.bias.detach().double()
    return w, b


def pack_conv_weights_g16(w):
    co, cin = w.shape[0], w.shape[-1]
    w5 = w.reshape(co, 9, cin // 32, 4, 8)
    f = (-(torch.arange(co, device=w.device) >> 2)) & 3
    idx = torch.arange(4, device=w.device)[None, :] ^ f[:, None]
    w5 = torch.gather(w5, 3, idx[:, None, None, :, None].expand(co, 9, cin // 32, 4, 8))
    return w5.permute(2, 1, 0, 3, 4).contiguous().view(cin // 32, 9, co, 32)


class EvalOptions:

    FIELDS = ("fused_conv", "fused_stem", "fused_heads", "fused_last", "layout", "force", "groups", "chains", "zigzag", "edge_tiles", "one_launch",
              "quad")

    def __init__(self, env=None):
        env = os.environ if env is None else env
        self.fused_conv = env.get("CCZ_FUSED_CONV", "1") != "0"
        self.fused_stem = env.get("CCZ_FUSED_STEM", "1") != "0"
        self.fused_heads = env.get("CCZ_FUSED_HEADS", "1") != "0"
        self.fused_last = env.get("CCZ_FUSED_LAST", "1") != "0"
        self.layout = env.get("CCZ_CONV_LAYOUT", "auto")
        self.force = {"small": 16, "tile": 32}.get(env.get("CCZ_CONV_FORCE", ""), 0)
        self.groups = int(env.get("CCZ_TOWER_GROUPS", "0"))
        self.chains = int(env.get("CCZ_TOWER_CHAINS", "0"))
        self.zigzag = env.get("CCZ_CONV_ZIGZAG", "1") == "1"
        self.edge_tiles = {"0": False, "1": True}.get(env.get("CCZ_CONV_EDGE_TILES", "auto"), "auto")
        self.one_launch = env.get("CCZ_CONV_ONE_LAUNCH", "1") != "0"
        self.quad = env.get("CCZ_CONV_QUAD", "1") != "0"
        if self.layout not in ("auto", "nhwc", "g16"):
            raise ValueError("CCZ_CONV_LAYOUT must be auto, nhwc or g16")

    def non_default(self):
        d = EvalOptions(env={})
        return {f: getattr(self, f) for f in self.FIELDS if getattr(self, f) != getattr(d, f)}


def _ptr(t, offset: int = 0):
    return C.c_void_p(t.data_ptr() + offset)


_CHAIN_STREAMS: dict = {}
CHAIN_STREAM_PRIORITY = -1
N_CHAIN_STREAMS = 8


def chain_streams(device):
    device = torch.device(device)
    if device.index is None:
        device = torch.device("cuda", torch.cuda.current_device())
    got = _CHAIN_STREAMS.get(device)
    if got is None:
        got = [torch.cuda.Stream(device=device, priority=CHAIN_STREAM_PRIORITY) for _ in range(N_CHAIN_STREAMS)]
        cur = torch.cuda.current_stream(device)
        ev = torch.cuda.Event()
        ev.record(cur)
        for st in got:
            st.wait_event(ev)
            with torch.cuda.stream(st):
                torch.zeros(1, device=device).add_(1.0)
            done = torch.cuda.Event()
            done.record(st)
            cur.wait_event(done)
        _CHAIN_STREAMS[device] = got
    return got


class InferenceNet(nn.Module):

    LIVE = list(range(7 * 7, 8 * 7)) + list(range(15 * 7, 17 * 7))

    def __init__(self, net: Net, dtype=torch.float16, live_only: bool = True):
        super().__init__()
        self.dtype = dtype
        self.live_only = live_only
        self.opt = EvalOptions()
        if self.opt.non_default():
            from .tools import log
            log(f"evaluator options from the environment: {self.opt.non_default()}")
        cl = torch.channels_last
        w, b = _fold(net.conv_block, net.conv_block_bn)
        if live_only:
            w = w[:, self.LIVE]
        self.stem_w = nn.Parameter(w.to(dtype).contiguous(memory_format=cl), requires_grad=False)
        self.stem_b = nn.Parameter(b.to(dtype), requires_grad=False)
        if live_only and w.shape[0] == 256:
            w64 = torch.zeros(256, 3, 3, 64, dtype=w.dtype, device=w.device)
            w64[..., :len(self.LIVE)] = w.permute(0, 2, 3, 1)
            self.stem_w64 = nn.Parameter(w64.to(dtype).contiguous(), requires_grad=False)
            self.stem_b32 = nn.Parameter(b.detach().float().clone(), requires_grad=False)
        ws, bs = [], []
        for blk in net.res_blocks:
            for conv, bn in ((blk.conv1, blk.conv1_bn), (blk.conv2, blk.conv2_bn)):
                w, b = _fold(conv, bn)
                ws.append(nn.Parameter(w.to(dtype).contiguous(memory_format=cl), requires_grad=False))
                bs.append(nn.Parameter(b.to(dtype), requires_grad=False))
        self.ws = nn.ParameterList(ws)
        self.bs = nn.ParameterList(bs)
        if ws and ws[0].shape[0] == 256 and ws[0].shape[1] == 256:
            self.ws_g16 = nn.ParameterList([nn.Parameter(pack_conv_weights_g16(w.permute(0, 2, 3, 1)), requires_grad=False) for w in ws])
        if hasattr(self, "stem_w64"):
            self.stem_w64_g16 = nn.Parameter(pack_conv_weights_g16(self.stem_w64), requires_grad=False)
        self.bs32 = nn.ParameterList([nn.Parameter(b.detach().float().clone(), requires_grad=False) for b in bs])
        wp, bp = _fold(net.policy_conv, net.policy_bn)
        wv, bv = _fold(net.value_conv, net.value_bn)
        C_in = wp.shape[1]
        self.head_wT = nn.Parameter(torch.cat([wp, wv], 0).reshape(PLAYS + PIECES, C_in).t().contiguous().to(dtype), requires_grad=False)
        self.head_b = nn.Parameter(torch.cat([bp, bv], 0).to(dtype), requires_grad=False)
        pc = lambda w, c: w.detach().reshape(w.shape[0], c, 90).permute(0, 2, 1).reshape(w.shape[0], c * 90).contiguous()
        self.policy_fc_w = nn.Parameter(pc(net.policy_fc.weight, PLAYS).to(dtype), requires_grad=False)
        self.policy_fc_b = nn.Parameter(net.policy_fc.bias.detach().to(dtype), requires_grad=False)
        self.value_fc1_w = nn.Parameter(pc(net.value_fc1.weight, PIECES).to(dtype), requires_grad=False)
        self.value_fc1_b = nn.Parameter(net.value_fc1.bias.detach().to(dtype), requires_grad=False)
        self.value_fc2_w = nn.Parameter(net.value_fc2.weight.detach().to(dtype), requires_grad=False)
        self.value_fc2_b = nn.Parameter(net.value_fc2.bias.detach().to(dtype), requires_grad=False)
        if C_in == 256 and dtype == torch.float16:
            w32 = torch.zeros(32, C_in, dtype=torch.float64)
            w32[:PLAYS + PIECES] = torch.cat([wp, wv], 0).reshape(PLAYS + PIECES, C_in)
            b32 = torch.zeros(32, dtype=torch.float64)
            b32[:PLAYS + PIECES] = torch.cat([bp, bv], 0)
            self.head_w32 = nn.Parameter(w32.to(dtype), requires_grad=False)
            self.head_b32 = nn.Parameter(b32.float(), requires_grad=False)

            def padded(w, rows, cols):
                out = torch.zeros(rows, cols, dtype=dtype)
                out[:w.shape[0], :w.shape[1]] = w.to(dtype)
                return out

            def padded_bias(b, rows):
                out = torch.zeros(rows, dtype=torch.float32)
                out[:b.shape[0]] = b.detach().to(dtype).float()
                return out
            self.policy_fc_wp = nn.Parameter(padded(pc(net.policy_fc.weight, PLAYS), 2176, 1536), requires_grad=False)
            self.policy_fc_b32 = nn.Parameter(padded_bias(net.policy_fc.bias, 2176), requires_grad=False)
            self.value_fc1_wp = nn.Parameter(padded(pc(net.value_fc1.weight, PIECES), 256, 640), requires_grad=False)
            self.value_fc1_b32 = nn.Parameter(padded_bias(net.value_fc1.bias, 256), requires_grad=False)

    def set_options(self, **kw):
        for k, v in kw.items():
            if k not in EvalOptions.FIELDS:
                raise KeyError(k)
            if k == "force" and isinstance(v, str):
                v = {"small": 16, "tile": 32, "": 0}[v]
            setattr(self.opt, k, v)
        if self.opt.layout not in ("auto", "nhwc", "g16"):
            raise ValueError("layout must be auto, nhwc or g16")
        self.__dict__.pop("_path_cache", None)
        return self

    def opt_fused_conv(self) -> bool:
        return self.opt.fused_conv

    def tower_groups(self, B: int, g16: bool) -> int:
        return self.opt.groups or -(-B // (self.TOWER_GROUP_BOARDS_G16 if g16 else self.TOWER_GROUP_BOARDS))

    EDGE_TILES_MIN_BOARDS = 4096
    TOWER_CHAINS_EDGE = 3

    def _edge(self, B: int, g16: bool = True) -> bool:
        et = self.opt.edge_tiles
        return bool(g16 and (et is True or (et == "auto" and B >= self.EDGE_TILES_MIN_BOARDS)))

    TOWER_CHAINS_SMALL = 3
    TOWER_CHAINS_SMALL_BOARDS = (768, 1536)

    def tower_chains(self, B: int, groups: int = 1, edge: bool = False) -> int:
        per_group = -(-B // groups)
        default = self.TOWER_CHAINS_EDGE if edge else (self.TOWER_CHAINS_SMALL if self.TOWER_CHAINS_SMALL_BOARDS[0] <= per_group < self.TOWER_CHAINS_SMALL_BOARDS[1]
                                                       else self.TOWER_CHAINS)
        return max(1, min(self.opt.chains or default, 8, per_group // 256))

    def bind_chain_streams(self, device):
        device = torch.device(device)
        if device.type == "cuda":
            self._chain_streams = (device, chain_streams(device))

    def derived_parameter_names(self) -> set:
        names = set()
        if hasattr(self, "ws_g16"):
            names |= {f"ws_g16.{i}" for i in range(len(self.ws_g16))}
        if hasattr(self, "stem_w64_g16"):
            names.add("stem_w64_g16")
        return names

    @torch.no_grad()
    def repack_derived(self):
        done = set()
        if hasattr(self, "ws_g16"):
            for i, (dst, w) in enumerate(zip(self.ws_g16, self.ws)):
                dst.copy_(pack_conv_weights_g16(w.permute(0, 2, 3, 1)))
                done.add(f"ws_g16.{i}")
        if hasattr(self, "stem_w64_g16"):
            self.stem_w64_g16.copy_(pack_conv_weights_g16(self.stem_w64))
            done.add("stem_w64_g16")
        if done != self.derived_parameter_names():
            raise RuntimeError(f"repack_derived rebuilt {sorted(done)} but derived_parameter_names() lists {sorted(self.derived_parameter_names())}")
        self.__dict__.pop("_b2", None)

    def _epilogue(self, y, bias, residual=None):
        if y.is_cuda and y.dtype == torch.float16 and y.is_contiguous(memory_format=torch.channels_last) \
                and (residual is None or residual.is_contiguous(memory_format=torch.channels_last)):
            from . import _lib
            n, c, h, w = y.shape
            _lib.check(_lib.lib().ccz_bias_act_f16(C.c_void_p(torch.cuda.current_stream(y.device).cuda_stream), _ptr(y), _ptr(bias),
                                                   _ptr(residual) if residual is not None else None, n * h * w, c))
            return y
        y = y + bias.view(1, -1, 1, 1)
        if residual is not None:
            y = y + residual
        return F.relu_(y)

    FUSED_MIN_BOARDS = 1

    def _use_fused_tower(self, x) -> bool:
        if not self.opt.fused_conv:
            return False
        return bool(x.is_cuda and x.dtype == torch.float16 and x.shape[1] == 256 and x.shape[0] >= self.FUSED_MIN_BOARDS
                    and x.is_contiguous(memory_format=torch.channels_last))

    G16_MIN_BOARDS = 640

    def _g16(self, B) -> bool:
        mode = self.opt.layout
        if mode == "nhwc" or self.opt.force:
            return False
        return B >= (65 if mode == "g16" else self.G16_MIN_BOARDS)

    TOWER_GROUP_BOARDS_G16 = 4096
    TOWER_GROUP_BOARDS = 2048
    TOWER_CHAINS = 2

    def _tower_fused(self, x, plan=None, g16=None, heads=None):
        if g16 is None:
            g16 = self._g16(x.shape[0]) and x.shape[0] % 16 == 0
        sched = self.tower_schedule(x.shape[0], g16, plan is not None, torch.cuda.is_current_stream_capturing())
        self._tower_enqueue(sched, x, torch.empty_like(x), plan, heads)
        return x

    def tower_schedule(self, B: int, g16: bool, planned: bool = False, capturing: bool = False):
        from . import _lib
        groups = 1 if capturing else self.tower_groups(B, g16)
        edge = self._edge(B, g16)
        f2 = 1 | ((_lib.CONV_G16 | self._edge_flags(edge)) if g16 else 0) | (0 if planned else self.opt.force)
        f1 = f2 | (2 if self.opt.zigzag else 0)
        if planned:
            chains = 1 if capturing else self.tower_chains(B, groups, edge)
            n_parts = groups * chains
            if g16:
                cap = -(-(B // 16) // n_parts) * 1440
            else:
                cap = -(-(-(-B // n_parts)) // 8) * 8 * 90
            return [[(cap, g * chains + k, n_parts, f1, f2) for k in range(chains)] for g in range(groups)]
        gstep = -(-(-(-B // groups)) // 128) * 128 if groups > 1 else B
        sched = []
        for g0 in range(0, B, gstep):
            n = min(B, g0 + gstep) - g0
            chains = 1 if capturing else self.tower_chains(n, 1, edge)
            step = -(-n // chains)
            if chains > 1:
                step = -(-step // 128) * 128
            sched.append([(g0 + b0, g0 + min(n, b0 + step), f1, f2) for b0 in range(0, n, step)])
        return sched

    def _tower_enqueue(self, sched, x, y, plan=None, heads=None):
        from . import _lib
        L = _lib.lib()
        cur = torch.cuda.current_stream(x.device)
        wsrc = self.ws_g16 if sched[0][0][-1] & _lib.CONV_G16 else self.ws
        layers = [(_ptr(w), _ptr(b)) for w, b in zip(wsrc, self.bs32)]
        hw, hb = (_ptr(self.head_w32), _ptr(self.head_b32)) if heads is not None else (None, None)
        conv = L.ccz_conv3x3_c256_f16 if plan is None else L.ccz_conv3x3_c256_f16_live
        row = 90 * 256 * x.element_size()

        def chain(st, d):
            s = C.c_void_p(st.cuda_stream)
            if plan is None:
                lo, hi, f1, f2 = d
                return s, _ptr(x, lo * row), _ptr(y, lo * row), [_ptr(h, lo * h.stride(0) * 2) for h in heads or ()], (hi - lo) * 90, f1, f2, (), (None, 0, 1)
            cap, part, n_parts, f1, f2 = d
            live = (_ptr(plan[1]), part, n_parts)
            return s, _ptr(x), _ptr(y), [_ptr(h) for h in heads or ()], cap, f1, f2, live, live

        for group in sched:
            streams = [cur] if len(group) == 1 else self._chain_pool(x.device, len(group))[:len(group)]
            if len(group) > 1:
                fork = torch.cuda.Event()
                fork.record(cur)
                for st in streams:
                    st.wait_event(fork)
            chains = [chain(st, d) for st, d in zip(streams, group)]
            for i in range(0, len(layers), 2):
                (w1, b1), (w2, b2) = layers[i], layers[i + 1]
                for s, xp, yp, _, n, f1, _, tail, _ in chains:
                    _lib.check(conv(s, xp, w1, b1, None, yp, n, f1, *tail))
                if heads is not None and i == len(layers) - 2:
                    for s, xp, yp, hd, n, _, f2, _, tail in chains:
                        _lib.check(L.ccz_conv3x3_c256_heads_f16(s, yp, w2, b2, xp, hw, hb, *hd, n, f2, *tail))
                    continue
                for s, xp, yp, _, n, _, f2, tail, _ in chains:
                    _lib.check(conv(s, yp, w2, b2, xp, xp, n, f2, *tail))
            for st in streams if len(group) > 1 else ():
                join = torch.cuda.Event()
                join.record(st)
                cur.wait_event(join)

    def _chain_pool(self, device, n):
        pool = getattr(self, "_chain_streams", None)
        if pool is None or pool[0] != device or len(pool[1]) < n:
            pool = (device, chain_streams(device))
            self._chain_streams = pool
        return pool[1]

    def _edge_flags(self, edge: bool) -> int:
        from . import _lib
        return (_lib.CONV_G16_EDGE_TILES | (_lib.CONV_G16_ONE_LAUNCH if self.opt.one_launch else 0)
                | (_lib.CONV_G16_QUAD if self.opt.quad else 0)) if edge else 0

    def _stem_fused(self, leaf_input, plan=None, g16=None):
        from . import _lib
        L = _lib.lib()
        B, dev = leaf_input.shape[0], leaf_input.device
        if g16 is None:
            g16 = self._g16(B)
        s = C.c_void_p(torch.cuda.current_stream(dev).cuda_stream)
        Bp = -(-B // 16) * 16 if g16 else B
        lay = _lib.CONV_G16 if g16 else 0
        if plan is None:
            x64 = (torch.zeros if Bp != B else torch.empty)((Bp, 90, 64), dtype=torch.float16, device=dev)
            y = torch.empty((Bp, 256, 10, 9), dtype=torch.float16, device=dev, memory_format=torch.channels_last)
            pack, gather = (L.ccz_pack_live_planes_g16_f16, (None, None)) if g16 else (L.ccz_pack_live_planes_f16, ())
            stem, tail = L.ccz_conv3x3_stem_f16, (Bp * 90, 1 | self.opt.force | lay)
        else:
            bufs = self.__dict__.setdefault("_plan_bufs", {})
            key = (Bp, dev, g16)
            if key not in bufs:
                bufs[key] = (torch.zeros((Bp, 90, 64), dtype=torch.float16, device=dev),
                             torch.empty((Bp, 256, 10, 9), dtype=torch.float16, device=dev, memory_format=torch.channels_last).zero_())
            x64, y = bufs[key]
            pack, gather = (L.ccz_pack_live_planes_g16_f16 if g16 else L.ccz_pack_live_planes_rows_f16), (_ptr(plan[0]), _ptr(plan[1]))
            stem, tail = L.ccz_conv3x3_stem_f16_live, (Bp * 90 if g16 else -(-B // 8) * 8 * 90, 1 | lay, _ptr(plan[1]), 0, 1)
        _lib.check(pack(s, _ptr(leaf_input), _ptr(x64), B, *gather))
        _lib.check(stem(s, _ptr(x64), _ptr(self.stem_w64_g16 if g16 else self.stem_w64), _ptr(self.stem_b32), _ptr(y), *tail))
        return y

    @torch.no_grad()
    def tower_activations(self, leaf_input):
        B = leaf_input.shape[0]
        g16 = self._g16(B)
        x = self._tower_fused(self._stem_fused(leaf_input, None, g16), None, g16)
        if not g16:
            return x
        Bp, Cn = x.shape[0], x.shape[1]
        rows = x.permute(0, 2, 3, 1).reshape(Bp // 16, 90, 16, Cn).permute(0, 2, 1, 3).reshape(Bp, 10, 9, Cn)[:B]
        return rows.permute(0, 3, 1, 2)

    def _path(self, leaf_input) -> str:
        B = leaf_input.shape[0]
        key = (B, leaf_input.is_cuda, leaf_input.dtype, leaf_input.is_contiguous())
        cache = self.__dict__.setdefault("_path_cache", {})
        if key not in cache:
            o = self.opt
            fused = (hasattr(self, "stem_w64") and leaf_input.is_cuda and leaf_input.dtype == torch.float16 and leaf_input.is_contiguous()
                     and B >= self.FUSED_MIN_BOARDS and self.dtype == torch.float16 and o.fused_conv and o.fused_stem)
            if fused:
                cache[key] = "g16" if self._g16(B) else "nhwc"
            else:
                cache[key] = "torch_stem" if (o.fused_conv and leaf_input.is_cuda and self.dtype == torch.float16
                                              and self.ws and self.ws[0].shape[0] == 256 and self.ws[0].shape[1] == 256) else "torch"
        return cache[key]

    @torch.no_grad()
    def forward(self, leaf_input: torch.Tensor, return_logits: bool = False, plan=None):
        B = leaf_input.shape[0]
        path = self._path(leaf_input)
        if plan is not None and path not in ("g16", "nhwc"):
            leaf_input = leaf_input.index_select(0, plan[0].long().clamp_(0, B - 1))
            plan = None
        g16 = path == "g16"
        if path in ("g16", "nhwc"):
            x = self._stem_fused(leaf_input, plan, g16)
            probe = self.__dict__.get("tower_probe")
            if probe is not None:
                p0, p1 = torch.cuda.Event(enable_timing=True), torch.cuda.Event(enable_timing=True)
                p0.record()
            heads = self._head_buffers(x.shape[0], x.device)[:2] if (g16 and self.opt.fused_last and self._fused_heads_ok(x)) else None
            x = self._tower_fused(x, plan, g16, heads)
            if probe is not None:
                p1.record()
                probe.append((p0, p1))
            if heads is not None:
                return self._heads(x, B, g16, plan, return_logits, conv_done=True)
        else:
            x = leaf_input.view(B, PLAYS * PIECES, 10, 9)
            if self.live_only:
                x = torch.cat([x[:, 49:56], x[:, 105:119]], dim=1)
            x = x.to(self.dtype).contiguous(memory_format=torch.channels_last)
            x = self._epilogue(F.conv2d(x, self.stem_w, None, padding=1), self.stem_b)
            if path == "torch_stem" and self._use_fused_tower(x):
                x = self._tower_fused(x, None, False)
            else:
                if x.is_cuda and x.dtype == torch.float16 and self.opt.fused_conv:
                    key = (int(x.shape[0]), int(x.shape[1]))
                    seen = self.__dict__.setdefault("_off_fused_seen", set())
                    if key not in seen:
                        seen.add(key)
                        from .tools import log
                        log(f"evaluator: batch of {key[0]} boards x {key[1]} channels is off the fused tower kernels "
                            f"(k_conv3x3_g16 / k_conv3x3_small serve 256-channel towers): MIOpen convolutions + one-pass epilogue")
                for i in range(0, len(self.ws), 2):
                    y = self._epilogue(F.conv2d(x, self.ws[i], None, padding=1), self.bs[i])
                    x = self._epilogue(F.conv2d(y, self.ws[i + 1], None, padding=1), self.bs[i + 1], x)
        return self._heads(x, B, g16, plan, return_logits)

    def _fused_heads_ok(self, x) -> bool:
        return bool(self.opt.fused_heads and hasattr(self, "head_w32") and x.is_cuda and x.dtype == torch.float16 and x.shape[1] == 256
                    and x.is_contiguous(memory_format=torch.channels_last))

    def _head_buffers(self, Bx, dev):
        from . import _lib
        bufs = self.__dict__.setdefault("_head_bufs", {})
        key = (Bx, dev)
        if key not in bufs:
            bufs[key] = (torch.zeros((Bx, _lib.HEAD_POL_STRIDE), dtype=torch.float16, device=dev),
                         torch.zeros((Bx, _lib.HEAD_VAL_STRIDE), dtype=torch.float16, device=dev),
                         torch.empty((Bx, 256), dtype=torch.float16, device=dev))
        return bufs[key]

    def _heads_fused(self, x, B, g16, plan, conv_done=False):
        from . import _lib
        L = _lib.lib()
        Bx, dev = x.shape[0], x.device
        pol, val, h1 = self._head_buffers(Bx, dev)
        logits = torch.empty((B, 2086), dtype=torch.float16, device=dev)
        v = torch.empty((B,), dtype=torch.float32, device=dev)
        s = C.c_void_p(torch.cuda.current_stream(dev).cuda_stream)
        live = _ptr(plan[1]) if plan is not None else None
        if not conv_done:
            _lib.check(L.ccz_heads_conv1x1_f16(s, _ptr(x), _ptr(self.head_w32), _ptr(self.head_b32), _ptr(pol), _ptr(val), Bx, _lib.CONV_G16 if g16 else 0, live))
        _lib.check(L.ccz_fc_f16(s, _ptr(pol), _lib.HEAD_POL_STRIDE, _ptr(self.policy_fc_wp), _ptr(self.policy_fc_b32), _ptr(logits), 2086, B, 2086, 1536, 0, live))
        _lib.check(L.ccz_fc_f16(s, _ptr(val), _lib.HEAD_VAL_STRIDE, _ptr(self.value_fc1_wp), _ptr(self.value_fc1_b32), _ptr(h1), 256, B, 256, 640, 1, live))
        _lib.check(L.ccz_value_out_f32(s, _ptr(h1), _ptr(self.value_fc2_w), self._value_b2(), _ptr(v), B, live))
        return logits, v

    def _value_b2(self) -> float:
        b2 = self.__dict__.get("_b2")
        if b2 is None:
            b2 = self.__dict__["_b2"] = float(self.value_fc2_b.detach().float().cpu().item())
        return b2

    def _heads(self, x, B, g16, plan, return_logits, conv_done=False):
        if self._fused_heads_ok(x):
            logits, v = self._heads_fused(x, B, g16, plan, conv_done)
            if return_logits:
                return logits, v
            return torch.exp(F.log_softmax(logits.float(), dim=1)).contiguous(), v
        Bx = x.shape[0]
        rows = x.permute(0, 2, 3, 1).reshape(Bx * 90, x.shape[1])
        h = F.relu_(torch.addmm(self.head_b, rows, self.head_wT))
        if g16:
            h = h.view(Bx // 16, 90, 16, PLAYS + PIECES).permute(0, 2, 1, 3).reshape(Bx, 90, PLAYS + PIECES)[:B]
        else:
            h = h.view(B, 90, PLAYS + PIECES)
        pol = h[:, :, :PLAYS].reshape(B, 90 * PLAYS)
        val = h[:, :, PLAYS:].reshape(B, 90 * PIECES)
        logits = F.linear(pol, self.policy_fc_w, self.policy_fc_b)
        v = F.relu_(F.linear(val, self.value_fc1_w, self.value_fc1_b))
        v = torch.tanh(F.linear(v, self.value_fc2_w, self.value_fc2_b).float()).view(B)
        if return_logits:
            return logits.contiguous(), v.contiguous()
        prob = torch.exp(F.log_softmax(logits.float(), dim=1))
        return prob.contiguous(), v.contiguous()


class PolicyValueNet:

    def __init__(self, model=None, use_gpu=True, device=None, num_channels=256, resblocks_num=40):
        self.use_gpu = use_gpu
        self.l2_const = 2e-3
        if device is not None:
            self.device = torch.device(device)
        else:
            self.device = torch.device("cuda") if (use_gpu and torch.cuda.is_available()) else torch.device("cpu")
        self.policy_value_net = Net(num_channels, resblocks_num).to(self.device)
        self.optimizer = torch.optim.Adam(params=self.policy_value_net.parameters(), lr=1e-3, betas=(0.9, 0.999),
                                          eps=1e-8, weight_decay=self.l2_const)
        if model:
            self.policy_value_net.load_state_dict(torch.load(model, map_location=self.device))
            from . import tools
            tools.log(f"weights loaded from {model}: piece planes and legal-move order follow rule preset '{tools.PRESET}' "
                      "(reference-trained weights: try tools.set_rules(preset='python-chess-lineage') [unverified] if this one plays nonsense)")
        self._infer = None
        self._graph = None
        self._miopen_find = os.environ.get("CCZ_MIOPEN_FIND", "1") != "0"
        self.weights_version = 0

    def invalidate_inference_copy(self):
        self._infer = None
        self.weights_version += 1

    def refresh_inference_copy(self):
        self._require_current_fp32("refresh_inference_copy")
        self.policy_value_net.eval()
        self._infer = InferenceNet(self.policy_value_net).to(self.device).eval()
        self._infer.bind_chain_streams(self.device)
        self._graph = None
        self.weights_version += 1
        return self._infer

    def _require_current_fp32(self, what: str):
        if getattr(self, "_fp32_stale", False):
            raise RuntimeError(f"{what}: this rank's fp32 net does not hold the weights of the last broadcast_model(what='inference') "
                               "(only the inference copy was sent): call broadcast_model(what='state') before training, saving or "
                               "rebuilding the inference copy here")

    @torch.no_grad()
    def evaluate_leaves(self, leaf_input: torch.Tensor):
        if self._infer is None:
            self.refresh_inference_copy()
        if not self._miopen_find:
            return self._infer(leaf_input)
        with torch.backends.cudnn.flags(enabled=True, benchmark=True):
            return self._infer(leaf_input)

    evaluate_leaves.batched = True
    evaluate_leaves.graph_safe = True

    @torch.no_grad()
    def evaluate_leaves_logits(self, leaf_input: torch.Tensor, plan=None):
        if self._infer is None:
            self.refresh_inference_copy()
        if not self._miopen_find:
            return self._infer(leaf_input, return_logits=True, plan=plan)
        with torch.backends.cudnn.flags(enabled=True, benchmark=True):
            return self._infer(leaf_input, return_logits=True, plan=plan)

    evaluate_leaves_logits.batched = True
    evaluate_leaves_logits.graph_safe = True
    evaluate_leaves_logits.returns_logits = True
    evaluate_leaves_logits.accepts_plan = True

    def policy_value(self, state_batch):
        self.policy_value_net.eval()
        if isinstance(state_batch, torch.Tensor):
            state_batch = state_batch.to(self.device)
        else:
            state_batch = torch.tensor(np.asarray(state_batch), dtype=torch.float).to(self.device)
        with torch.no_grad():
            log_act_probs, value = self.policy_value_net(state_batch.float())
        return np.exp(log_act_probs.cpu().numpy()), value.cpu().numpy()

    def policy_value_fn(self, board, red_states=None, black_states=None):
        from .tools import decode_board
        self.policy_value_net.eval()
        legal_positions = board.legal_ids()
        if red_states is None or black_states is None:
            red_state, black_state = decode_board(board)
            red_states = [np.zeros((PIECES, 10, 9), dtype=np.float16) for _ in range(PIECES)] + [red_state]
            black_states = [np.zeros((PIECES, 10, 9), dtype=np.float16) for _ in range(PIECES)] + [black_state]
        current_player = (np.ones if board.turn else np.zeros)((1, PIECES, 10, 9), dtype=np.float16)
        states = np.concatenate((red_states, black_states, current_player), axis=0)
        x = torch.as_tensor(np.ascontiguousarray(states.reshape(-1, PLAYS, PIECES, 10, 9)).astype("float16"))
        with torch.no_grad():
            if self.device.type == "cuda":
                with torch.autocast("cuda"):
                    log_act_probs, value = self.policy_value_net(x.to(self.device))
            else:
                log_act_probs, value = self.policy_value_net(x.float().to(self.device))
        act_probs = np.exp(log_act_probs.float().cpu().numpy().flatten())
        return zip(legal_positions, act_probs[legal_positions]), value.float().cpu().numpy()

    def save_model(self, model_file):
        self._require_current_fp32("save_model")
        torch.save(self.policy_value_net.state_dict(), model_file)

    def train_step(self, state_batch, mcts_probs, winner_batch, lr=0.002):
        self._require_current_fp32("train_step")
        self.policy_value_net.train()
        to = lambda t: (t if isinstance(t, torch.Tensor) else torch.as_tensor(np.asarray(t))).to(self.device, dtype=torch.float)
        state_batch, mcts_probs, winner_batch = to(state_batch), to(mcts_probs), to(winner_batch)
        self.optimizer.zero_grad()
        log_act_probs, value = self.policy_value_net(state_batch)
        value_loss = F.mse_loss(input=torch.reshape(value, shape=[-1]), target=winner_batch)
        policy_loss = -torch.mean(torch.sum(mcts_probs * log_act_probs, dim=1))
        loss = value_loss + policy_loss
        loss.backward()
        self.optimizer.step()
        with torch.no_grad():
            entropy = -torch.mean(torch.sum(torch.exp(log_act_probs) * log_act_probs, dim=1))
        self.invalidate_inference_copy()
        return loss.detach().cpu().numpy(), entropy.detach().cpu().numpy()


def uniform_evaluator(leaf_input: torch.Tensor):
    B = leaf_input.shape[0]
    key = (B, leaf_input.device)
    cache = uniform_evaluator.__dict__.setdefault("_cache", {})
    if key not in cache:
        cache[key] = (torch.full((B, 2086), 1.0 / 2086, dtype=torch.float32, device=leaf_input.device),
                      torch.zeros((B,), dtype=torch.float32, device=leaf_input.device))
    return cache[key]


uniform_evaluator.batched = True
```

include/cczero.h:

```cpp
#ifndef CCZERO_H
#define CCZERO_H

#include <stdint.h>

#ifdef __cplusplus
extern "C" {
#endif

#define CCZ_ABI_VERSION 9
#define CCZ_NSQ 90
#define CCZ_SQ_STRIDE 96
#define CCZ_NMOVES 2086
#define CCZ_MAX_LEGAL 128
#define CCZ_MASK_WORDS 66
#define CCZ_PLANES 10710


#define CCZ_RULE_PAWN_MOVE_RESETS_CLOCK 2u
#define CCZ_RULE_PERPETUAL_CHECK 1u

#define CCZ_FLAG_REFERENCE_QUIRKS 1u
#define CCZ_FLAG_NO_MIRROR 2u
#define CCZ_FLAG_VALUE_F16 4u

#define CCZ_FLAG_CACHE_VERIFY 8u

#define CCZ_FLAG_STRICT 16u

#define CCZ_LEAF_EXPAND 0
#define CCZ_LEAF_DRAW 1
#define CCZ_LEAF_LOSS 2
#define CCZ_LEAF_NONE 3
#define CCZ_LEAF_WIN 4

typedef struct ccz_engine ccz_engine;

typedef struct ccz_config {
    int32_t n_boards;
    int32_t n_playout;
    float c_puct;
    float eps;
    float alpha;
    float temp;
    int32_t max_nodes;
    int32_t max_depth;
    int32_t max_plies;
    uint32_t flags;
    uint64_t seed;
    uint64_t board_id_base;
    int32_t device;
    int32_t reserve_nodes;
    const uint16_t *move_rank_host;
    uint8_t plane_of_type[8];
    uint32_t rule_flags;
    uint32_t eval_cache_log2;
    uint8_t type_rank[8];
} ccz_config;

typedef struct ccz_stats {
    int64_t sims;
    int64_t moves;
    int64_t games;
    int64_t truncated_games;
    int64_t nodes_peak;
    int64_t depth_peak;
    int64_t sum_depth;
    int64_t sum_children;
    int64_t expansions;
    int64_t terminal_leaves;
    int32_t error_flags;
    int32_t reserved;
    int64_t hbm_bytes;
    int64_t pruned_subtrees;
    int64_t cache_probes;
    int64_t cache_hits;
    int64_t cache_shared_rows;
    int64_t cache_stores;
    int64_t cache_verified;
    int64_t cache_verify_mismatches;
} ccz_stats;

#define CCZ_ERR_NODE_POOL 1
#define CCZ_ERR_DEPTH 2
#define CCZ_ERR_CHAIN 64
#define CCZ_ERR_MOVES 4
#define CCZ_ERR_RECORD 8
#define CCZ_ERR_BAD_MOVE 16
#define CCZ_ERR_NAN 32
#define CCZ_ERR_BOUNDS 128
#define CCZ_ERR_PRUNED 256
#define CCZ_ERR_TRUNCATED 512
#define CCZ_ERR_BAD_TEMP 1024

int ccz_abi_version(void);
const char *ccz_last_error(void);
int ccz_device_count(void);

int ccz_action_table(char *uci_out_host, uint8_t *from_out_host, uint8_t *to_out_host);
int ccz_flip_map(int32_t *flip_out_host);

int ccz_create(const ccz_config *cfg, ccz_engine **out);
int ccz_destroy(ccz_engine *e);
int ccz_reset(ccz_engine *e, void *stream, const uint8_t *mask_host);
int ccz_set_position(ccz_engine *e, void *stream, int32_t board, const uint8_t *sq_host,
                     int32_t turn, int32_t halfmove);
int ccz_set_positions(ccz_engine *e, void *stream, const uint8_t *sq_dev, const uint8_t *turn_dev, const int32_t *halfmove_dev,
                      const int32_t *moves_dev, const int32_t *n_moves_dev, int32_t max_moves, const uint8_t *mask_host,
                      int32_t *status_dev);
int ccz_reset_tree(ccz_engine *e, void *stream, const uint8_t *mask_host);

int ccz_select_leaves(ccz_engine *e, void *stream, void *leaf_input_f16_dev);
int ccz_zero_leaf_input(ccz_engine *e, void *stream, void *leaf_input_f16_dev);
int ccz_expand_backup(ccz_engine *e, void *stream, const float *prob_dev, const float *value_dev);

int ccz_step(ccz_engine *e, void *stream, const float *prob_dev, const float *value_dev,
             void *leaf_input_f16_dev);

int ccz_gather_priors(ccz_engine *e, void *stream, const void *logits_dev, int32_t logits_f16);
int ccz_step_compact(ccz_engine *e, void *stream, const float *value_dev, void *leaf_input_f16_dev);
int ccz_expand_backup_compact(ccz_engine *e, void *stream, const float *value_dev);

int ccz_set_scouts(ccz_engine *e, int32_t n_scouts);
int ccz_scout(ccz_engine *e, void *stream, void *leaf_input_f16_dev);
int ccz_eval_plan_scouted(ccz_engine *e, void *stream, int32_t *miss_rows_dev, int32_t *n_miss_dev, int32_t *state_dev);
int ccz_scout_and_plan(ccz_engine *e, void *stream, void *leaf_input_f16_dev, int32_t *miss_rows_dev, int32_t *n_miss_dev, int32_t *state_dev);
int ccz_scouted_run(ccz_engine *e, void *stream, void *leaf_input_f16_dev, int32_t *miss_rows_dev, int32_t *n_miss_dev, int32_t *state_dev,
                    int32_t *run_dev);

int ccz_eval_plan(ccz_engine *e, void *stream, int32_t *miss_rows_dev, int32_t *n_miss_dev);
int ccz_gather_priors_planned(ccz_engine *e, void *stream, const void *logits_compact_dev, int32_t logits_f16,
                              const float *value_compact_dev);
int ccz_eval_cache_clear(ccz_engine *e, void *stream);

int ccz_set_routing(ccz_engine *e, void *stream, const uint8_t *red_net_host, uint64_t salt0, uint64_t salt1);
int ccz_eval_plan_routed(ccz_engine *e, void *stream, int32_t *miss_rows_dev, int32_t *n_miss_dev);
int ccz_gather_priors_routed(ccz_engine *e, void *stream, const void *logits0_dev, const void *logits1_dev, int32_t logits_f16,
                             const float *value0_dev, const float *value1_dev);

#define CCZ_REC_FAST 1
int ccz_set_budgets(ccz_engine *e, void *stream, const int32_t *budgets_dev, const uint8_t *targets_dev);
int ccz_draw_budgets(ccz_engine *e, void *stream, int32_t n_full, int32_t n_fast, double p_full, int32_t *budgets_out_dev);

#define CCZ_REC_RESIGNED 2
#define CCZ_REC_PLAYON 4
#define CCZ_REC_VALUE 8
#define CCZ_REC_VALUE_OFF 92
#define CCZ_RESIGN_RESIGNED 2
#define CCZ_RESIGN_PLAYON 4
typedef struct ccz_resign_stats {
    int64_t resigned_games;
    int64_t resigned_by_red;
    int64_t resigned_plies;
    int64_t playon_games;
    int64_t playon_won;
    int64_t playon_drawn;
    int64_t playon_plies_after;
} ccz_resign_stats;
int ccz_set_resign(ccz_engine *e, void *stream, int32_t enabled, float threshold, int32_t consecutive, int32_t min_ply, double p_playon);
int ccz_get_resign_stats(ccz_engine *e, void *stream, ccz_resign_stats *out);
int ccz_resign_status(ccz_engine *e, void *stream, uint8_t *state_host, uint8_t *run_host, int32_t *fire_ply_host, float *last_value_host);

typedef struct ccz_exploration_stats {
    int64_t explored_moves;
    int64_t forced_selections;
    int64_t visits_pruned;
    int64_t children_pruned;
} ccz_exploration_stats;
int ccz_set_root_exploration(ccz_engine *e, void *stream, int32_t enabled, double eps, double alpha, double forced_k, int32_t prune_targets);
int ccz_get_exploration_stats(ccz_engine *e, void *stream, ccz_exploration_stats *out);
int ccz_root_noise(ccz_engine *e, void *stream, float *noise_host, int32_t *k_host);

typedef struct ccz_gumbel_stats {
    int64_t gumbel_moves;
    int64_t considered_sum;
    int64_t offvisit_moves;
} ccz_gumbel_stats;
int ccz_set_gumbel(ccz_engine *e, void *stream, int32_t enabled, int32_t n_sims, int32_t max_considered, double c_visit, double c_scale);
int ccz_get_gumbel_stats(ccz_engine *e, void *stream, ccz_gumbel_stats *out);
int ccz_gumbel_root(ccz_engine *e, void *stream, double *g_host, double *logit_host, int32_t *n0_host, int32_t *k_host, int32_t *n_eff_host);
int ccz_gumbel_sequence(void *stream, int32_t m, int32_t n, int32_t *seq_dev);

typedef struct ccz_search_cfg {
    int32_t enabled, fpu_mode, fpu_root_mode, reserved;
    double fpu_value, fpu_root_value, c_base, c_factor;
} ccz_search_cfg;
int ccz_set_search(ccz_engine *e, void *stream, int32_t enabled, int32_t fpu_mode, double fpu_value, int32_t fpu_root_mode,
                   double fpu_root_value, double c_base, double c_factor);
int ccz_get_search(ccz_engine *e, void *stream, ccz_search_cfg *out);

#define CCZ_PROOF_WIN 1
#define CCZ_PROOF_LOSS 2
#define CCZ_PROOF_DRAW 3
typedef struct ccz_solver_stats {
    int64_t nodes_proven;
    int64_t proven_stops;
    int64_t roots_proven;
} ccz_solver_stats;
int ccz_set_solver(ccz_engine *e, void *stream, int32_t enabled);
int ccz_root_proof(ccz_engine *e, void *stream, uint8_t *state_host, uint8_t *dist_host, uint8_t *child_state_host, uint8_t *child_dist_host);
int ccz_get_solver_stats(ccz_engine *e, void *stream, ccz_solver_stats *out);
int ccz_proof_combine(void *stream, const uint8_t *bytes_dev, const int32_t *counts_dev, int32_t n_cases, uint8_t *out_dev);

typedef struct ccz_wide_stats {
    int64_t steps;
    int64_t leaves;
    int64_t collisions;
    int64_t inflight_now;
} ccz_wide_stats;
int ccz_set_width(ccz_engine *e, void *stream, int32_t width);
int ccz_select_wide(ccz_engine *e, void *stream, void *leaf_input_f16_dev, int32_t *n_leaves_dev);
int ccz_step_wide(ccz_engine *e, void *stream, const float *value_dev, void *leaf_input_f16_dev, int32_t *n_leaves_dev);
int ccz_get_wide_stats(ccz_engine *e, void *stream, ccz_wide_stats *out);

int ccz_finish_move(ccz_engine *e, void *stream, const int32_t *forced_moves_dev,
                    const double *temps_dev, int32_t *moves_out_dev, int32_t keep_tree);

int ccz_root_children(ccz_engine *e, void *stream, int32_t *k_host, uint16_t *acts_host,
                      int32_t *visits_host, float *q_host, float *prior_host, int32_t *root_visits_host);
int ccz_principal_variations(ccz_engine *e, void *stream, int32_t multipv, int32_t max_len, uint16_t *moves_dev, int32_t *len_dev,
                             int32_t *visits_dev, float *q_dev, float *prior_dev, int32_t *root_visits_dev);
int ccz_root_pi(ccz_engine *e, void *stream, const double *temps_host, double *pi_host);
int ccz_move_distribution(ccz_engine *e, void *stream, const double *temps_host, double *gamma_host, double *mixed_host,
                          double *u_host);
int ccz_game_status(ccz_engine *e, void *stream, uint8_t *over_host, int8_t *winner_host,
                    int32_t *plies_host, uint8_t *turn_host);
int ccz_root_positions(ccz_engine *e, void *stream, uint8_t *sq_host);
int ccz_leaf_info(ccz_engine *e, void *stream, uint8_t *status_host, int32_t *k_host,
                  uint16_t *ids_host, int32_t *depth_host);

int ccz_leaf_priors(ccz_engine *e, void *stream, float *prior_host, float *value_host);

int ccz_leaf_keys(ccz_engine *e, void *stream, uint64_t *keys_dev, uint8_t *status_dev);

int ccz_harvest_rows(ccz_engine *e, void *stream, int64_t *rows_host);
int ccz_harvest(ccz_engine *e, void *stream, void *states_f16_dev, float *pi_dev, float *z_dev,
                int64_t capacity_rows, int64_t *rows_host);

#define CCZ_REC_BYTES 880
#define CCZ_REC_HDR 96
#define CCZ_REC_IDS 112
#define CCZ_REC_PI 368
int ccz_harvest_records(ccz_engine *e, void *stream, void *records_dev, int64_t capacity_plies, int64_t *plies_host);
int ccz_expand_records(void *stream, const void *records_dev, int64_t n_plies, uint32_t flags,
                       const uint8_t *plane_of_type_host, void *states_f16_dev, float *pi_dev, float *z_dev,
                       int64_t ring_rows, int64_t head_row, int32_t *bad_records_dev, uint8_t *target_dev, float *value_dev);

int ccz_ring_retire(void *stream, const void *ring_dev, int64_t cap_plies, int64_t *window_dev, int64_t head_new,
                    int32_t max_game_plies, int32_t *bad_records_dev);
int ccz_sample_records(void *stream, const void *ring_dev, int64_t cap_plies, const int64_t *window_dev,
                       const int64_t *draws_dev, int64_t batch, uint32_t flags, const uint8_t *plane_of_type_host,
                       void *states_f16_dev, float *pi_dev, float *z_dev, int32_t *bad_records_dev, uint8_t *target_dev,
                       float *value_dev);

int ccz_get_stats(ccz_engine *e, void *stream, ccz_stats *out);

int ccz_legal_moves(void *stream, int32_t n, const uint8_t *sq_dev, const uint8_t *turn_dev,
                    const int32_t *halfmove_dev, uint32_t *mask_dev, int32_t *count_dev,
                    uint8_t *flags_dev);
int ccz_apply_moves(void *stream, int32_t n, uint8_t *sq_dev, uint8_t *turn_dev,
                    const int32_t *move_ids_dev, uint8_t *captured_dev);

int ccz_bias_act_f16(void *stream, void *y_dev, const void *bias_dev, const void *residual_dev,
                     int64_t rows, int32_t channels);

#define CCZ_CONV_RELU 1
#define CCZ_CONV_DESCENDING 2
#define CCZ_CONV_FORCE_SMALL 16
#define CCZ_CONV_FORCE_TILE 32
#define CCZ_CONV_G16 64
#define CCZ_CONV_G16_EDGE_TILES 128
#define CCZ_CONV_G16_ONE_LAUNCH 512
#define CCZ_CONV_G16_QUAD 65536
int ccz_conv3x3_c256_f16(void *stream, const void *x_dev, const void *w_dev, const void *bias_f32_dev,
                         const void *residual_dev, void *y_dev, int64_t n_pixels, int32_t relu);
int ccz_pack_conv_weights_g16_f16(void *stream, const void *w_dev, void *wp_dev, int32_t cin);

int ccz_conv3x3_stem_f16(void *stream, const void *x64_dev, const void *w_dev, const void *bias_f32_dev,
                         void *y_dev, int64_t n_pixels, int32_t relu);
int ccz_pack_live_planes_f16(void *stream, const void *leaf_dev, void *x64_dev, int32_t n_boards);
int ccz_pack_live_planes_g16_f16(void *stream, const void *leaf_dev, void *x64_dev, int32_t n_boards,
                                 const int32_t *rows_dev, const int32_t *n_rows_dev);

int ccz_pack_live_planes_rows_f16(void *stream, const void *leaf_dev, void *x64_dev, int32_t n_boards,
                                  const int32_t *rows_dev, const int32_t *n_rows_dev);
int ccz_conv3x3_c256_f16_live(void *stream, const void *x_dev, const void *w_dev, const void *bias_f32_dev,
                              const void *residual_dev, void *y_dev, int64_t n_pixels, int32_t relu,
                              const int32_t *live_rows_dev, int32_t part, int32_t n_parts);
int ccz_conv3x3_stem_f16_live(void *stream, const void *x64_dev, const void *w_dev, const void *bias_f32_dev,
                              void *y_dev, int64_t n_pixels, int32_t relu, const int32_t *live_rows_dev,
                              int32_t part, int32_t n_parts);

#define CCZ_HEAD_POL_STRIDE 1536
#define CCZ_HEAD_VAL_STRIDE 640
int ccz_heads_conv1x1_f16(void *stream, const void *x_dev, const void *w32_dev, const void *bias32_f32_dev, void *pol_dev,
                          void *val_dev, int32_t n_boards, int32_t flags, const int32_t *live_boards_dev);
int ccz_fc_f16(void *stream, const void *a_dev, int32_t lda, const void *w_dev, const void *bias_f32_dev, void *c_dev, int32_t ldc,
               int32_t m, int32_t n, int32_t k, int32_t relu, const int32_t *live_rows_dev);
int ccz_value_out_f32(void *stream, const void *h_dev, const void *w2_dev, float b2, float *v_dev, int32_t m,
                      const int32_t *live_rows_dev);

int ccz_conv3x3_c256_heads_f16(void *stream, const void *x_dev, const void *w_dev, const void *bias_f32_dev,
                               const void *residual_dev, const void *head_w32_dev, const void *head_bias32_f32_dev,
                               void *pol_dev, void *val_dev, int64_t n_pixels, int32_t flags,
                               const int32_t *live_rows_dev, int32_t part, int32_t n_parts);

#ifdef __cplusplus
}
#endif
#endif
```

Before: 200,300.

## Add chunk-major G16C activation layout for fused conv tower and heads

Introduces a chunk-major activation layout in which each 16-board group stores 64-byte channel chunks contiguously, plus conv, stem and heads kernel variants that read and write it. The Python tower switches to this layout when the chunk_major option is set along with the quad one-launch and fused-heads paths. The aim is more contiguous DMA loads and stores in the tower convs, which should improve memory coalescing. In exchange it adds a separate layout path with its own constraints: it needs the quad one-launch form, and the last layer must carry the heads.

Result: faster. 203,000 (median of 6 runs) (+1.4%).

```diff
diff --git a/chinesechesszero_amd/_lib.py b/chinesechesszero_amd/_lib.py
--- a/chinesechesszero_amd/_lib.py
+++ b/chinesechesszero_amd/_lib.py
@@ -181,6 +181,11 @@
     "ccz_conv3x3_c256_f16_live": (C.c_int, [_P, _P, _P, _P, _P, _P, C.c_int64, C.c_int32, _P, C.c_int32, C.c_int32]),
     "ccz_conv3x3_stem_f16_live": (C.c_int, [_P, _P, _P, _P, _P, C.c_int64, C.c_int32, _P, C.c_int32, C.c_int32]),
     "ccz_conv3x3_c256_heads_f16": (C.c_int, [_P, _P, _P, _P, _P, _P, _P, _P, _P, C.c_int64, C.c_int32, _P, C.c_int32, C.c_int32]),
+    "ccz_conv3x3_c256_g16c_f16": (C.c_int, [_P, _P, _P, _P, _P, _P, C.c_int64, C.c_int32]),
+    "ccz_conv3x3_c256_g16c_f16_live": (C.c_int, [_P, _P, _P, _P, _P, _P, C.c_int64, C.c_int32, _P, C.c_int32, C.c_int32]),
+    "ccz_conv3x3_stem_g16c_f16": (C.c_int, [_P, _P, _P, _P, _P, C.c_int64, C.c_int32]),
+    "ccz_conv3x3_stem_g16c_f16_live": (C.c_int, [_P, _P, _P, _P, _P, C.c_int64, C.c_int32, _P, C.c_int32, C.c_int32]),
+    "ccz_conv3x3_c256_heads_g16c_f16": (C.c_int, [_P, _P, _P, _P, _P, _P, _P, _P, _P, C.c_int64, C.c_int32, _P, C.c_int32, C.c_int32]),
     "ccz_heads_conv1x1_f16": (C.c_int, [_P, _P, _P, _P, _P, _P, C.c_int32, C.c_int32, _P]),
     "ccz_fc_f16": (C.c_int, [_P, _P, C.c_int32, _P, _P, _P, C.c_int32, C.c_int32, C.c_int32, C.c_int32, C.c_int32, _P]),
     "ccz_value_out_f32": (C.c_int, [_P, _P, _P, C.c_float, _P, C.c_int32, _P]),
diff --git a/chinesechesszero_amd/csrc/cczero.hip b/chinesechesszero_amd/csrc/cczero.hip
--- a/chinesechesszero_amd/csrc/cczero.hip
+++ b/chinesechesszero_amd/csrc/cczero.hip
@@ -1576,7 +1576,7 @@
 constexpr int64_t kSmallMaxPixels = 64 * 90;
 
 static int conv3x3_launch(const char *who, void *stream, const void *x_dev, const void *w_dev, const void *bias_f32_dev, const void *residual_dev, void *y_dev,
-                          int64_t n_pixels, int32_t relu, int cin, const int32_t *live_rows_dev = nullptr, int32_t row0 = 0)
+                          int64_t n_pixels, int32_t relu, int cin, const int32_t *live_rows_dev = nullptr, int32_t row0 = 0, bool g16c = false)
 {
     if (!x_dev || !w_dev || !bias_f32_dev || !y_dev || n_pixels < 0 || n_pixels % 90 || n_pixels > (int64_t)INT32_MAX / kCvC)
         return fail(-1, "%s: bad arguments (n_pixels must be boards * 90, at most 93206 boards per call)", who);
@@ -1595,6 +1595,20 @@
         const G16Args a = {(const _Float16 *)x_dev, (const _Float16 *)w_dev, (const float *)bias_f32_dev, (const _Float16 *)residual_dev, (_Float16 *)y_dev,
                            (int)n_pixels, cin, (const int *)live_rows_dev, (int)row0};
         const bool res = residual_dev != nullptr;
+        if (g16c) {
+            if (cin == 64) {
+                hipLaunchKernelGGL(k_conv3x3_g16c_stem, dim3((unsigned)(groups * 5)), dim3(512), 0, s, (const _Float16 *)x_dev, (const _Float16 *)w_dev,
+                                   (const float *)bias_f32_dev, (_Float16 *)y_dev, (int)n_pixels, (int)fl, cin, (const int *)live_rows_dev, (int)row0);
+                HIP_TRY(hipGetLastError());
+                return 0;
+            }
+            const int need = CCZ_CONV_G16_EDGE_TILES | CCZ_CONV_G16_ONE_LAUNCH | CCZ_CONV_G16_QUAD;
+            if ((relu & need) != need)
+                return fail(-1, "%s: the G16C layout runs the quad one-launch form only (CCZ_CONV_G16_EDGE_TILES | _ONE_LAUNCH | _QUAD)", who);
+            g16_launch(CCZ_G16_RES(k_conv3x3_g16c_one_quad, res), (unsigned)(groups * 4 + 2 * ((groups + 1) / 2)), s, a, fl);
+            HIP_TRY(hipGetLastError());
+            return 0;
+        }
         if (cin == 64) {
             hipLaunchKernelGGL(k_conv3x3_g16_stem, dim3((unsigned)(groups * 5)), dim3(512), 0, s, (const _Float16 *)x_dev, (const _Float16 *)w_dev,
                                (const float *)bias_f32_dev, (_Float16 *)y_dev, (int)n_pixels, (int)fl, cin, (const int *)live_rows_dev, (int)row0);
@@ -1652,11 +1666,41 @@
     return conv3x3_launch("ccz_conv3x3_c256_f16", stream, x_dev, w_dev, bias_f32_dev, residual_dev, y_dev, n_pixels, relu, 256);
 }
 
-int ccz_conv3x3_c256_heads_f16(void *stream, const void *x_dev, const void *w_dev, const void *bias_f32_dev, const void *residual_dev,
-                               const void *head_w32_dev, const void *head_b32_dev, void *pol_dev, void *val_dev, int64_t n_pixels, int32_t flags,
-                               const int32_t *live_rows_dev, int32_t part, int32_t n_parts)
-{
-    const char *who = "ccz_conv3x3_c256_heads_f16";
+int ccz_conv3x3_c256_g16c_f16(void *stream, const void *x_dev, const void *w_dev, const void *bias_f32_dev, const void *residual_dev, void *y_dev,
+                              int64_t n_pixels, int32_t relu)
+{
+    if (!(relu & CCZ_CONV_G16)) return fail(-1, "ccz_conv3x3_c256_g16c_f16: CCZ_CONV_G16 must be set");
+    return conv3x3_launch("ccz_conv3x3_c256_g16c_f16", stream, x_dev, w_dev, bias_f32_dev, residual_dev, y_dev, n_pixels, relu, 256, nullptr, 0, true);
+}
+
+int ccz_conv3x3_c256_g16c_f16_live(void *stream, const void *x_dev, const void *w_dev, const void *bias_f32_dev, const void *residual_dev, void *y_dev,
+                                   int64_t n_pixels, int32_t relu, const int32_t *live_rows_dev, int32_t part, int32_t n_parts)
+{
+    if (!(relu & CCZ_CONV_G16)) return fail(-1, "ccz_conv3x3_c256_g16c_f16_live: CCZ_CONV_G16 must be set");
+    if (!live_rows_dev || g16_bad_part(part, n_parts)) return fail(-1, "ccz_conv3x3_c256_g16c_f16_live: null live-row count or bad part / n_parts");
+    return conv3x3_launch("ccz_conv3x3_c256_g16c_f16_live", stream, x_dev, w_dev, bias_f32_dev, residual_dev, y_dev, n_pixels, relu, 256, live_rows_dev,
+                          part | (n_parts << 16), true);
+}
+
+int ccz_conv3x3_stem_g16c_f16(void *stream, const void *x64_dev, const void *w_dev, const void *bias_f32_dev, void *y_dev, int64_t n_pixels, int32_t relu)
+{
+    if (!(relu & CCZ_CONV_G16)) return fail(-1, "ccz_conv3x3_stem_g16c_f16: CCZ_CONV_G16 must be set");
+    return conv3x3_launch("ccz_conv3x3_stem_g16c_f16", stream, x64_dev, w_dev, bias_f32_dev, nullptr, y_dev, n_pixels, relu, 64, nullptr, 0, true);
+}
+
+int ccz_conv3x3_stem_g16c_f16_live(void *stream, const void *x64_dev, const void *w_dev, const void *bias_f32_dev, void *y_dev, int64_t n_pixels, int32_t relu,
+                                   const int32_t *live_rows_dev, int32_t part, int32_t n_parts)
+{
+    if (!(relu & CCZ_CONV_G16)) return fail(-1, "ccz_conv3x3_stem_g16c_f16_live: CCZ_CONV_G16 must be set");
+    if (!live_rows_dev || g16_bad_part(part, n_parts)) return fail(-1, "ccz_conv3x3_stem_g16c_f16_live: null live-row count or bad part / n_parts");
+    return conv3x3_launch("ccz_conv3x3_stem_g16c_f16_live", stream, x64_dev, w_dev, bias_f32_dev, nullptr, y_dev, n_pixels, relu, 64, live_rows_dev,
+                          part | (n_parts << 16), true);
+}
+
+static int heads_layer_launch(const char *who, bool g16c, void *stream, const void *x_dev, const void *w_dev, const void *bias_f32_dev, const void *residual_dev,
+                              const void *head_w32_dev, const void *head_b32_dev, void *pol_dev, void *val_dev, int64_t n_pixels, int32_t flags,
+                              const int32_t *live_rows_dev, int32_t part, int32_t n_parts)
+{
     if (!x_dev || !w_dev || !bias_f32_dev || !residual_dev || !head_w32_dev || !head_b32_dev || !pol_dev || !val_dev || n_pixels < 0 || n_pixels % 1440 ||
         n_pixels > (int64_t)INT32_MAX / kCvC)
         return fail(-1, "%s: bad arguments (n_pixels must be a multiple of 16 boards * 90, at most 93200 boards per call)", who);
@@ -1677,12 +1721,37 @@
     ha.val = (_Float16 *)val_dev;
     ha.nb = (int)(n_pixels / 90);
     hipStream_t s = (hipStream_t)stream;
+    if (g16c) {
+        if (!(flags & CCZ_CONV_G16_EDGE_TILES)) return fail(-1, "%s: the G16C layout needs CCZ_CONV_G16_EDGE_TILES", who);
+        const int groups = (int)(n_pixels / 1440);
+        g16_launch(k_conv3x3_g16c_heads, (unsigned)(groups * 4), s, a, fl | 4, ha);
+        HIP_TRY(hipGetLastError());
+        g16_launch(k_conv3x3_g16c_edge_heads, 2u * (unsigned)((groups + 1) / 2), s, a, fl, ha);
+        HIP_TRY(hipGetLastError());
+        return 0;
+    }
     g16_launch(k_conv3x3_g16_heads, shape.mid, s, a, shape.edge ? fl | 4 : fl, ha);
     HIP_TRY(hipGetLastError());
     if (!shape.edge) return 0;
     g16_launch(k_conv3x3_g16_edge_heads, shape.edge, s, a, fl, ha);
     HIP_TRY(hipGetLastError());
     return 0;
+}
+
+int ccz_conv3x3_c256_heads_f16(void *stream, const void *x_dev, const void *w_dev, const void *bias_f32_dev, const void *residual_dev,
+                               const void *head_w32_dev, const void *head_b32_dev, void *pol_dev, void *val_dev, int64_t n_pixels, int32_t flags,
+                               const int32_t *live_rows_dev, int32_t part, int32_t n_parts)
+{
+    return heads_layer_launch("ccz_conv3x3_c256_heads_f16", false, stream, x_dev, w_dev, bias_f32_dev, residual_dev, head_w32_dev, head_b32_dev, pol_dev, val_dev,
+                              n_pixels, flags, live_rows_dev, part, n_parts);
+}
+
+int ccz_conv3x3_c256_heads_g16c_f16(void *stream, const void *x_dev, const void *w_dev, const void *bias_f32_dev, const void *residual_dev,
+                                    const void *head_w32_dev, const void *head_b32_dev, void *pol_dev, void *val_dev, int64_t n_pixels, int32_t flags,
+                                    const int32_t *live_rows_dev, int32_t part, int32_t n_parts)
+{
+    return heads_layer_launch("ccz_conv3x3_c256_heads_g16c_f16", true, stream, x_dev, w_dev, bias_f32_dev, residual_dev, head_w32_dev, head_b32_dev, pol_dev, val_dev,
+                              n_pixels, flags, live_rows_dev, part, n_parts);
 }
 
 int ccz_conv3x3_stem_f16(void *stream, const void *x64_dev, const void *w_dev, const void *bias_f32_dev, void *y_dev, int64_t n_pixels, int32_t relu)
diff --git a/chinesechesszero_amd/csrc/cczero_conv_g16.h b/chinesechesszero_amd/csrc/cczero_conv_g16.h
--- a/chinesechesszero_amd/csrc/cczero_conv_g16.h
+++ b/chinesechesszero_amd/csrc/cczero_conv_g16.h
@@ -25,6 +25,13 @@
 static_assert(kG5QRows * kG5QERow == 156672 && kG5QRows * kG5QERow <= kG5QLds,
               "quad tile: the epilogue image covers the operand buffers AND most of the dump area (free once every DMA has landed)");
 
+constexpr int kG16CChunk = 1440 * 64;
+__device__ __forceinline__ unsigned g16c_off(long p)
+{
+    const long g = p / 1440;
+    return (unsigned)(g * (1440 * 512) + (p - g * 1440) * 64);
+}
+
 struct G5Ctx {
     unsigned char *lds;
     const _Float16 *X, *W;
@@ -98,7 +105,7 @@
     if constexpr (LO <= 3 && 3 < HI) G5_CELL(TAP, 3) if constexpr (LO <= 4 && 4 < HI) G5_CELL(TAP, 4) if constexpr (LO <= 5 && 5 < HI) G5_CELL(TAP, 5) \
     if constexpr (LO <= 6 && 6 < HI) G5_CELL(TAP, 6) if constexpr (LO <= 7 && 7 < HI) G5_CELL(TAP, 7) if constexpr (LO <= 8 && 8 < HI) G5_CELL(TAP, 8)
 
-template <int J, bool Q = false>
+template <int J, bool Q = false, bool CM = false>
 __device__ __forceinline__ void g5_step(const G5Ctx &c, cv_f32x4 (&acc)[4][9], int chunk, int &ring_rd, int &ring_wr,
                                          cv_half8 (&a0)[4], cv_half8 (&a1)[4], cv_half8 (&b)[9])
 {
@@ -115,7 +122,7 @@
     G5_CELLS(T, 0, 1)
     if constexpr (Q && g5q_nslab(T) > 0) {
         constexpr int pass = T == 0 ? 0 : T + 1;
-        const unsigned so = (unsigned)((chunk + 1) * 64);
+        const unsigned so = (unsigned)((chunk + 1) * (CM ? kG16CChunk : 64));
         const unsigned live = chunk < c.cmask ? (pass < 6 ? c.xbytes : c.xbytes_part) : 0u;
         cv_blds16(c.X, live, c.xoff[0], so + pass * c.xstep,
                   lds + (pass < 6 ? kAOff + (1 - BUF) * kSlab + pass * 8192 + c.wave_dst : c.wave_dst_part + (1 - BUF) * c.wave_step_part));
@@ -125,7 +132,7 @@
     if constexpr (!Q && g5_dma(T) > 2) {
         constexpr int pass = T - 1;
         const unsigned live = pass < 4 ? c.xbytes : c.xbytes_part;
-        cv_blds16(c.X, chunk < c.cmask ? live : 0u, c.xoff[pass], (unsigned)((chunk + 1) * 64),
+        cv_blds16(c.X, chunk < c.cmask ? live : 0u, c.xoff[pass], (unsigned)((chunk + 1) * (CM ? kG16CChunk : 64)),
                   lds + (pass < 4 ? kG5AOff + (1 - BUF) * kG5SlabBytes + pass * 8192 + c.wave_dst : c.wave_dst_part + (1 - BUF) * c.wave_step_part));
         __builtin_amdgcn_sched_barrier(0);
     }
@@ -292,6 +299,23 @@
     }
 }
 
+__device__ __forceinline__ int g16c_lane_row(int lane) { return (int)((0xFEAB6732DC894510ull >> (4 * (lane >> 2))) & 15); }
+
+template <int EROW, bool RES, bool HEADS>
+__device__ __forceinline__ void g5c_rows_out(unsigned char *lds, int img, size_t yoff, _Float16 *Y, int relu, const cv_half8 (&rv)[18])
+{
+    const cv_half8 zero = (cv_half8)(_Float16)0;
+    unsigned char *eb = lds + img;
+#pragma unroll
+    for (int it = 0; it < 18; ++it) {
+        cv_half8 v = *(const cv_half8 *)(eb + it * 16 * EROW);
+        if (RES) v = v + rv[it];
+        if (relu) v = __builtin_elementwise_max(v, zero);
+        if constexpr (HEADS) *(cv_half8 *)(eb + it * 16 * EROW) = v;
+        else *(cv_half8 *)((unsigned char *)Y + yoff + it * 1024) = v;
+    }
+}
+
 __device__ __forceinline__ void g5_acc_row_from_bias(cv_f32x4 (&row)[9], const float *bias4)
 {
     const float4 bv = *(const float4 *)bias4;
@@ -301,7 +325,7 @@
     }
 }
 
-template <bool RES, bool HEADS, bool ONE = false>
+template <bool RES, bool HEADS, bool ONE = false, bool CM = false>
 __device__ __forceinline__ void g5_tile(unsigned char *lds, int blk, int grid, const _Float16 *__restrict__ X, const _Float16 *__restrict__ W,
                                         const float *__restrict__ bias, const _Float16 *R,
                                         _Float16 *Y, int M, int relu, int cin, const int *live_rows, int row0, const G5Heads &ha)
@@ -349,7 +373,8 @@
             const int schunk = pos ^ ((0 - (sr >> 2)) & 3);
             long p = p0 - 144 + sr;
             p = p < 0 ? 0 : (p > (long)M - 1 ? (long)M - 1 : p);
-            c.xoff[it] = (unsigned)(p * cin + schunk * 8) * 2u;
+            if constexpr (CM && !ONE) c.xoff[it] = g16c_off(p) + (unsigned)(schunk * 16);
+            else c.xoff[it] = (unsigned)(p * cin + schunk * 8) * 2u;
         }
         c.woff = (unsigned)(tid * 16);
     }
@@ -378,7 +403,7 @@
     for (int i = 0; i < 4; ++i) a0[i] = *(const cv_half8 *)(lds + c.a_off + i * 1024);
 #pragma unroll
     for (int n = 0; n < 9; ++n) b[n] = *(const cv_half8 *)(lds + c.vb[0] + (9 + n - 9) * 1024);
-#define G5_S(j) g5_step<j>(c, acc, chunk + (j) / 9, ring_rd, ring_wr, a0, a1, b)
+#define G5_S(j) g5_step<j, false, CM && !ONE>(c, acc, chunk + (j) / 9, ring_rd, ring_wr, a0, a1, b)
     if constexpr (ONE) {
         const int chunk = 0;
         G5_S(0); G5_S(1); G5_S(2); G5_S(3); G5_S(4); G5_S(5); G5_S(6); G5_S(7); G5_S(8);
@@ -398,12 +423,23 @@
     const long pbase = p0 + w * 36 + prow;
     cv_half8 rv[18];
     g5_image_store<kG5ERow>(lds, acc, wm, wn, re, q4e);
-    if (RES) {
-#pragma unroll
-        for (int it = 0; it < 18; ++it) rv[it] = *(const cv_half8 *)(R + (pbase + it * 2) * kCvC + piece * 8);
-    }
-    g5_barrier<true>();
-    g5_rows_out<kG5ERow, 2, RES, HEADS>(lds, w * 36 + prow, piece, pbase, piece * 8, Y, relu, rv);
+    if constexpr (CM) {
+        const int erow = g16c_lane_row(lane_e), ep = lane_e & 3;
+        const size_t yo = (size_t)g16c_off(p0 + erow) + (size_t)(w * kG16CChunk + ep * 16);
+        if (RES) {
+#pragma unroll
+            for (int it = 0; it < 18; ++it) rv[it] = *(const cv_half8 *)((const unsigned char *)R + yo + it * 1024);
+        }
+        g5_barrier<true>();
+        g5c_rows_out<kG5ERow, RES, HEADS>(lds, erow * kG5ERow + w * 64 + ep * 16, yo, Y, relu, rv);
+    } else {
+        if (RES) {
+#pragma unroll
+            for (int it = 0; it < 18; ++it) rv[it] = *(const cv_half8 *)(R + (pbase + it * 2) * kCvC + piece * 8);
+        }
+        g5_barrier<true>();
+        g5_rows_out<kG5ERow, 2, RES, HEADS>(lds, w * 36 + prow, piece, pbase, piece * 8, Y, relu, rv);
+    }
     if constexpr (HEADS) {
         g5_barrier<true>();
         const long grp = p0 / 1440;
@@ -414,7 +450,7 @@
     }
 }
 
-template <bool RES>
+template <bool RES, bool CM = false>
 __device__ __forceinline__ void g5q_tile(unsigned char *lds, int blk, int grid, const _Float16 *__restrict__ X, const _Float16 *__restrict__ W,
                                          const float *__restrict__ bias, const _Float16 *R, _Float16 *Y, int M, int relu, int cin,
                                          const int *live_rows, int row0)
@@ -443,12 +479,13 @@
     c.wave_dst_part = w < 6 ? kG5QAOff + 6 * 8192 + w * 1024 : kG5QDump + w * 1024;
     c.wave_step_part = w < 6 ? kG5QSlabBytes : 0;
     c.xbytes_part = w < 6 ? c.xbytes : 0u;
-    c.xstep = 128u * (unsigned)cin * 2u;
+    c.xstep = CM ? 128u * 64u : 128u * (unsigned)cin * 2u;
     c.whalf = (unsigned)h * 8192u;
     {
         const int sr = tid >> 2, pos = tid & 3;
         const int schunk = pos ^ ((0 - (sr >> 2)) & 3);
-        c.xoff[0] = (unsigned)((p0 - 144 + sr) * cin + schunk * 8) * 2u;
+        if constexpr (CM) c.xoff[0] = g16c_off(p0 - 144 + sr) + (unsigned)(schunk * 16);
+        else c.xoff[0] = (unsigned)((p0 - 144 + sr) * cin + schunk * 8) * 2u;
         c.woff = (unsigned)(tid * 16);
     }
 #pragma unroll
@@ -472,7 +509,7 @@
 #pragma unroll
     for (int n = 0; n < 9; ++n) b[n] = *(const cv_half8 *)(lds + c.vb[0] + n * 1024);
     for (int chunk = 0; chunk <= c.cmask; chunk += 2) {
-#define G5Q_S(j) g5_step<j, true>(c, acc, chunk + (j) / 9, ring_rd, ring_wr, a0, a1, b)
+#define G5Q_S(j) g5_step<j, true, CM>(c, acc, chunk + (j) / 9, ring_rd, ring_wr, a0, a1, b)
         G5Q_S(0); G5Q_S(1); G5Q_S(2); G5Q_S(3); G5Q_S(4); G5Q_S(5); G5Q_S(6); G5Q_S(7); G5Q_S(8);
         G5Q_S(9); G5Q_S(10); G5Q_S(11); G5Q_S(12); G5Q_S(13); G5Q_S(14); G5Q_S(15); G5Q_S(16); G5Q_S(17);
 #undef G5Q_S
@@ -487,12 +524,23 @@
     const int gcol = h * 128 + piece * 8;
     cv_half8 rv[18];
     g5_image_store<kG5QERow>(lds, acc, wm, wn, re, q4e);
-    if (RES) {
-#pragma unroll
-        for (int it = 0; it < 18; ++it) rv[it] = *(const cv_half8 *)(R + (pbase + it * 4) * kCvC + gcol);
-    }
-    g5_barrier<true>();
-    g5_rows_out<kG5QERow, 4, RES, false>(lds, w * 72 + prow, piece, pbase, gcol, Y, relu, rv);
+    if constexpr (CM) {
+        const int erow = g16c_lane_row(lane_e), ep = lane_e & 3, ch = w & 3, irow = (w >> 2) * 288 + erow;
+        const size_t yo = (size_t)g16c_off(p0 + irow) + (size_t)((h * 4 + ch) * kG16CChunk + ep * 16);
+        if (RES) {
+#pragma unroll
+            for (int it = 0; it < 18; ++it) rv[it] = *(const cv_half8 *)((const unsigned char *)R + yo + it * 1024);
+        }
+        g5_barrier<true>();
+        g5c_rows_out<kG5QERow, RES, false>(lds, irow * kG5QERow + ch * 64 + ep * 16, yo, Y, relu, rv);
+    } else {
+        if (RES) {
+#pragma unroll
+            for (int it = 0; it < 18; ++it) rv[it] = *(const cv_half8 *)(R + (pbase + it * 4) * kCvC + gcol);
+        }
+        g5_barrier<true>();
+        g5_rows_out<kG5QERow, 4, RES, false>(lds, w * 72 + prow, piece, pbase, gcol, Y, relu, rv);
+    }
 }
 
 template <bool RES>
@@ -528,6 +576,23 @@
     __shared__ __attribute__((aligned(16))) unsigned char lds[kG5Lds];
     if (live_rows) ha.nb = *live_rows;
     g5_tile<true, true>(lds, blockIdx.x, gridDim.x, X, W, bias, R, Y, M, relu, cin, live_rows, row0, ha);
+}
+
+__global__ __launch_bounds__(512) void k_conv3x3_g16c_stem(const _Float16 *__restrict__ X, const _Float16 *__restrict__ W,
+                                                             const float *__restrict__ bias, _Float16 *Y, int M, int relu, int cin,
+                                                             const int *live_rows, int row0)
+{
+    __shared__ __attribute__((aligned(16))) unsigned char lds[kG5Lds];
+    g5_tile<false, false, true, true>(lds, blockIdx.x, gridDim.x, X, W, bias, nullptr, Y, M, relu, cin, live_rows, row0, G5Heads{});
+}
+
+__global__ __launch_bounds__(512) void k_conv3x3_g16c_heads(const _Float16 *__restrict__ X, const _Float16 *__restrict__ W,
+                                                              const float *__restrict__ bias, const _Float16 *R, _Float16 *Y, int M,
+                                                              int relu, int cin, const int *live_rows, int row0, G5Heads ha)
+{
+    __shared__ __attribute__((aligned(16))) unsigned char lds[kG5Lds];
+    if (live_rows) ha.nb = *live_rows;
+    g5_tile<true, true, false, true>(lds, blockIdx.x, gridDim.x, X, W, bias, R, Y, M, relu, cin, live_rows, row0, ha);
 }
 
 __global__ __launch_bounds__(256) void k_pack_conv_weights_g16(const cv_half8 *__restrict__ w, cv_half8 *__restrict__ wp, int cin)
diff --git a/chinesechesszero_amd/csrc/cczero_conv_g16e.h b/chinesechesszero_amd/csrc/cczero_conv_g16e.h
--- a/chinesechesszero_amd/csrc/cczero_conv_g16e.h
+++ b/chinesechesszero_amd/csrc/cczero_conv_g16e.h
@@ -10,7 +10,7 @@
 static_assert(g5e_dma(0) == 4 && g5e_dma(1) == 4 && g5e_dma(2) == 3 && g5e_dma(3) == 2 && g5e_dma(4) == 2 && g5e_dma(5) == 2,
               "17 DMA loads per chunk and thread: 5 slab pieces + 6 x 2 weight pieces");
 
-template <int J>
+template <int J, bool CM = false>
 __device__ __forceinline__ void g5e_step(const G5Ctx &c, cv_f32x4 (&acc)[4][9], int chunk, int &ring_rd, int &ring_wr,
                                           cv_half8 (&a0)[4], cv_half8 (&a1)[4], cv_half8 (&b)[9], int toff)
 {
@@ -25,7 +25,7 @@
     G5_CELLS(H, 0, 1)
     if constexpr (g5e_dma(H) > 2) {
         constexpr int p0 = H * 2;
-        const unsigned so = (unsigned)((chunk + 1) * 64);
+        const unsigned so = (unsigned)((chunk + 1) * (CM ? kG16CChunk : 64));
         const unsigned live = chunk < c.cmask ? (p0 < 4 ? c.xbytes : c.xbytes_part) : 0u;
         cv_blds16(c.X, live, c.xoff[p0], so,
                   lds + (p0 < 4 ? kG5AOff + (1 - BUF) * kG5SlabBytes + p0 * 8192 + c.wave_dst : c.wave_dst_part + (1 - BUF) * c.wave_step_part));
@@ -61,7 +61,7 @@
 #undef G5_REFILL
 }
 
-template <bool RES, bool HEADS>
+template <bool RES, bool HEADS, bool CM = false>
 __device__ __forceinline__ void g5e_tile(unsigned char *lds, int blk, const _Float16 *__restrict__ X, const _Float16 *__restrict__ W,
                                          const float *__restrict__ bias, const _Float16 *R, _Float16 *Y, int M,
                                          int relu, int cin, const int *live_rows, int row0, const G5Heads &ha)
@@ -101,7 +101,8 @@
             const int sr = piece >> 2, pos = piece & 3;
             const int schunk = pos ^ ((0 - (sr >> 2)) & 3);
             const long p = sr < 288 ? srcA + sr : srcB + (sr - 288);
-            c.xoff[it] = (unsigned)(p * cin + schunk * 8) * 2u;
+            if constexpr (CM) c.xoff[it] = g16c_off(p) + (unsigned)(schunk * 16);
+            else c.xoff[it] = (unsigned)(p * cin + schunk * 8) * 2u;
         }
         c.woff = (unsigned)(tid * 16);
     }
@@ -130,7 +131,7 @@
 #pragma unroll
     for (int n = 0; n < 9; ++n) b[n] = *(const cv_half8 *)(lds + c.vb[0] + n * 1024);
     for (int chunk = 0; chunk <= c.cmask; chunk += 2) {
-#define G5E_S(j) g5e_step<j>(c, acc, chunk + (j) / 6, ring_rd, ring_wr, a0, a1, b, toff)
+#define G5E_S(j) g5e_step<j, CM>(c, acc, chunk + (j) / 6, ring_rd, ring_wr, a0, a1, b, toff)
         G5E_S(0); G5E_S(1); G5E_S(2); G5E_S(3); G5E_S(4); G5E_S(5);
         G5E_S(6); G5E_S(7); G5E_S(8); G5E_S(9); G5E_S(10); G5E_S(11);
 #undef G5E_S
@@ -143,21 +144,44 @@
     const long pbase = (w < 4 ? outA : outB) + (w & 3) * 36 + prow;
     const bool store = !(dup && w >= 4);
     cv_half8 rv[18];
-    if (RES) {
-#pragma unroll
-        for (int it = 0; it < 18; ++it) rv[it] = *(const cv_half8 *)(R + (pbase + it * 2) * kCvC + piece * 8);
-    }
-    g5_barrier<true>();
-    if (store) {
+    if constexpr (CM) {
+        const int erow = g16c_lane_row(lane), ep = lane & 3;
+        const size_t yoA = (size_t)g16c_off(outA + erow) + (size_t)(w * kG16CChunk + ep * 16);
+        const size_t yoB = (size_t)g16c_off(outB + erow) + (size_t)(w * kG16CChunk + ep * 16);
+        if (RES) {
+#pragma unroll
+            for (int it = 0; it < 18; ++it) rv[it] = *(const cv_half8 *)((const unsigned char *)R + (it < 9 ? yoA + it * 1024 : yoB + (it - 9) * 1024));
+        }
+        g5_barrier<true>();
         const cv_half8 zero = (cv_half8)(_Float16)0;
-        unsigned char *eb = lds + (w * 36 + prow) * kG5ERow + piece * 16;
+        unsigned char *eb = lds + erow * kG5ERow + w * 64 + ep * 16;
 #pragma unroll
         for (int it = 0; it < 18; ++it) {
-            cv_half8 v = *(const cv_half8 *)(eb + it * 2 * kG5ERow);
-            if (RES) v = v + rv[it];
-            if (relu) v = __builtin_elementwise_max(v, zero);
-            if constexpr (HEADS) *(cv_half8 *)(eb + it * 2 * kG5ERow) = v;
-            else *(cv_half8 *)(Y + (pbase + it * 2) * kCvC + piece * 8) = v;
+            if (it < 9 || !dup) {
+                cv_half8 v = *(const cv_half8 *)(eb + it * 16 * kG5ERow);
+                if (RES) v = v + rv[it];
+                if (relu) v = __builtin_elementwise_max(v, zero);
+                if constexpr (HEADS) *(cv_half8 *)(eb + it * 16 * kG5ERow) = v;
+                else *(cv_half8 *)((unsigned char *)Y + (it < 9 ? yoA + it * 1024 : yoB + (it - 9) * 1024)) = v;
+            }
+        }
+    } else {
+        if (RES) {
+#pragma unroll
+            for (int it = 0; it < 18; ++it) rv[it] = *(const cv_half8 *)(R + (pbase + it * 2) * kCvC + piece * 8);
+        }
+        g5_barrier<true>();
+        if (store) {
+            const cv_half8 zero = (cv_half8)(_Float16)0;
+            unsigned char *eb = lds + (w * 36 + prow) * kG5ERow + piece * 16;
+#pragma unroll
+            for (int it = 0; it < 18; ++it) {
+                cv_half8 v = *(const cv_half8 *)(eb + it * 2 * kG5ERow);
+                if (RES) v = v + rv[it];
+                if (relu) v = __builtin_elementwise_max(v, zero);
+                if constexpr (HEADS) *(cv_half8 *)(eb + it * 2 * kG5ERow) = v;
+                else *(cv_half8 *)(Y + (pbase + it * 2) * kCvC + piece * 8) = v;
+            }
         }
     }
     if constexpr (HEADS) {
@@ -186,7 +210,7 @@
     g5e_tile<true, true>(lds, blockIdx.x, X, W, bias, R, Y, M, relu, cin, live_rows, row0, ha);
 }
 
-template <bool RES, bool QUAD>
+template <bool RES, bool QUAD, bool CM = false>
 __device__ __forceinline__ void g5_one_launch(unsigned char *lds, const _Float16 *__restrict__ X, const _Float16 *__restrict__ W,
                                               const float *__restrict__ bias, const _Float16 *R, _Float16 *Y, int M,
                                               int relu, int cin, const int *live_rows, int row0)
@@ -198,9 +222,9 @@
     }
     const int mid = groups * 4, blk = blockIdx.x;
     if (blk < mid) {
-        if constexpr (QUAD) g5q_tile<RES>(lds, blk, mid, X, W, bias, R, Y, M, relu, cin, live_rows, row0);
+        if constexpr (QUAD) g5q_tile<RES, CM>(lds, blk, mid, X, W, bias, R, Y, M, relu, cin, live_rows, row0);
         else g5_tile<RES, false>(lds, blk, mid, X, W, bias, R, Y, M, relu | 4, cin, live_rows, row0, G5Heads{});
-    } else g5e_tile<RES, false>(lds, blk - mid, X, W, bias, R, Y, M, relu, cin, live_rows, row0, G5Heads{});
+    } else g5e_tile<RES, false, CM>(lds, blk - mid, X, W, bias, R, Y, M, relu, cin, live_rows, row0, G5Heads{});
 }
 
 template <bool RES>
@@ -221,6 +245,24 @@
     g5_one_launch<RES, true>(lds, X, W, bias, R, Y, M, relu, cin, live_rows, row0);
 }
 
+template <bool RES>
+__global__ __launch_bounds__(512) void k_conv3x3_g16c_one_quad(const _Float16 *__restrict__ X, const _Float16 *__restrict__ W,
+                                                                 const float *__restrict__ bias, const _Float16 *R, _Float16 *Y, int M,
+                                                                 int relu, int cin, const int *live_rows, int row0)
+{
+    __shared__ __attribute__((aligned(16))) unsigned char lds[kG5Lds];
+    g5_one_launch<RES, true, true>(lds, X, W, bias, R, Y, M, relu, cin, live_rows, row0);
+}
+
+__global__ __launch_bounds__(512) void k_conv3x3_g16c_edge_heads(const _Float16 *__restrict__ X, const _Float16 *__restrict__ W,
+                                                                   const float *__restrict__ bias, const _Float16 *R, _Float16 *Y,
+                                                                   int M, int relu, int cin, const int *live_rows, int row0, G5Heads ha)
+{
+    __shared__ __attribute__((aligned(16))) unsigned char lds[kG5Lds];
+    if (live_rows) ha.nb = *live_rows;
+    g5e_tile<true, true, true>(lds, blockIdx.x, X, W, bias, R, Y, M, relu, cin, live_rows, row0, ha);
+}
+
 #undef G5_CELLS
 #undef G5_CELL
 
diff --git a/chinesechesszero_amd/net.py b/chinesechesszero_amd/net.py
--- a/chinesechesszero_amd/net.py
+++ b/chinesechesszero_amd/net.py
@@ -78,10 +78,46 @@
     return w5.permute(2, 1, 0, 3, 4).contiguous().view(cin // 32, 9, co, 32)
 
 
+def _memory_rows(t, width):
+    if t.dim() == 4 and not t.is_contiguous():
+        t = t.permute(0, 2, 3, 1)
+    if not t.is_contiguous():
+        raise ValueError("expected a channels-last or a contiguous tensor")
+    return t.reshape(-1, width)
+
+
+def g16_to_g16c(t):
+    rows = _memory_rows(t, 256)
+    out = rows.view(-1, 1440, 8, 32).permute(0, 2, 1, 3).contiguous()
+    return out.view(t.shape[0], 10, 9, 256).permute(0, 3, 1, 2) if t.dim() == 4 else out.view(t.shape)
+
+
+def g16c_to_g16(t):
+    rows = _memory_rows(t, 32)
+    out = rows.view(-1, 8, 1440, 32).permute(0, 2, 1, 3).contiguous()
+    return out.view(t.shape[0], 10, 9, 256).permute(0, 3, 1, 2) if t.dim() == 4 else out.view(t.shape)
+
+
+def g16c_to_boards(t, boards=None):
+    m = _memory_rows(t, 32)
+    G = m.shape[0] // (8 * 1440)
+    out = m.view(G, 8, 90, 16, 32).permute(0, 3, 2, 1, 4).reshape(G * 16, 10, 9, 256)
+    return out[:boards].permute(0, 3, 1, 2)
+
+
+def boards_to_g16c(x):
+    B = x.shape[0]
+    G = -(-B // 16)
+    rows = torch.zeros((G * 16, 90, 256), dtype=x.dtype, device=x.device)
+    rows[:B] = x.permute(0, 2, 3, 1).reshape(B, 90, 256)
+    out = rows.view(G, 16, 90, 8, 32).permute(0, 3, 2, 1, 4).contiguous()
+    return out.view(G * 16, 10, 9, 256).permute(0, 3, 1, 2)
+
+
 class EvalOptions:
 
     FIELDS = ("fused_conv", "fused_stem", "fused_heads", "fused_last", "layout", "force", "groups", "chains", "zigzag", "edge_tiles", "one_launch",
-              "quad")
+              "quad", "chunk_major")
 
     def __init__(self, env=None):
         env = os.environ if env is None else env
@@ -97,6 +133,7 @@
         self.edge_tiles = {"0": False, "1": True}.get(env.get("CCZ_CONV_EDGE_TILES", "auto"), "auto")
         self.one_launch = env.get("CCZ_CONV_ONE_LAUNCH", "1") != "0"
         self.quad = env.get("CCZ_CONV_QUAD", "1") != "0"
+        self.chunk_major = env.get("CCZ_CONV_CHUNK_MAJOR", "1") != "0"
         if self.layout not in ("auto", "nhwc", "g16"):
             raise ValueError("CCZ_CONV_LAYOUT must be auto, nhwc or g16")
 
@@ -299,11 +336,11 @@
     TOWER_GROUP_BOARDS = 2048
     TOWER_CHAINS = 2
 
-    def _tower_fused(self, x, plan=None, g16=None, heads=None):
+    def _tower_fused(self, x, plan=None, g16=None, heads=None, chunk_major=False):
         if g16 is None:
             g16 = self._g16(x.shape[0]) and x.shape[0] % 16 == 0
         sched = self.tower_schedule(x.shape[0], g16, plan is not None, torch.cuda.is_current_stream_capturing())
-        self._tower_enqueue(sched, x, torch.empty_like(x), plan, heads)
+        self._tower_enqueue(sched, x, torch.empty_like(x), plan, heads, chunk_major)
         return x
 
     def tower_schedule(self, B: int, g16: bool, planned: bool = False, capturing: bool = False):
@@ -331,7 +368,7 @@
             sched.append([(g0 + b0, g0 + min(n, b0 + step), f1, f2) for b0 in range(0, n, step)])
         return sched
 
-    def _tower_enqueue(self, sched, x, y, plan=None, heads=None):
+    def _tower_enqueue(self, sched, x, y, plan=None, heads=None, chunk_major=False):
         from . import _lib
         L = _lib.lib()
         cur = torch.cuda.current_stream(x.device)
@@ -339,6 +376,10 @@
         layers = [(_ptr(w), _ptr(b)) for w, b in zip(wsrc, self.bs32)]
         hw, hb = (_ptr(self.head_w32), _ptr(self.head_b32)) if heads is not None else (None, None)
         conv = L.ccz_conv3x3_c256_f16 if plan is None else L.ccz_conv3x3_c256_f16_live
+        heads_layer = L.ccz_conv3x3_c256_heads_f16
+        if chunk_major:
+            conv = L.ccz_conv3x3_c256_g16c_f16 if plan is None else L.ccz_conv3x3_c256_g16c_f16_live
+            heads_layer = L.ccz_conv3x3_c256_heads_g16c_f16
         row = 90 * 256 * x.element_size()
 
         def chain(st, d):
@@ -364,7 +405,7 @@
                     _lib.check(conv(s, xp, w1, b1, None, yp, n, f1, *tail))
                 if heads is not None and i == len(layers) - 2:
                     for s, xp, yp, hd, n, _, f2, _, tail in chains:
-                        _lib.check(L.ccz_conv3x3_c256_heads_f16(s, yp, w2, b2, xp, hw, hb, *hd, n, f2, *tail))
+                        _lib.check(heads_layer(s, yp, w2, b2, xp, hw, hb, *hd, n, f2, *tail))
                     continue
                 for s, xp, yp, _, n, _, f2, tail, _ in chains:
                     _lib.check(conv(s, yp, w2, b2, xp, xp, n, f2, *tail))
@@ -385,7 +426,7 @@
         return (_lib.CONV_G16_EDGE_TILES | (_lib.CONV_G16_ONE_LAUNCH if self.opt.one_launch else 0)
                 | (_lib.CONV_G16_QUAD if self.opt.quad else 0)) if edge else 0
 
-    def _stem_fused(self, leaf_input, plan=None, g16=None):
+    def _stem_fused(self, leaf_input, plan=None, g16=None, chunk_major=False):
         from . import _lib
         L = _lib.lib()
         B, dev = leaf_input.shape[0], leaf_input.device
@@ -408,6 +449,8 @@
             x64, y = bufs[key]
             pack, gather = (L.ccz_pack_live_planes_g16_f16 if g16 else L.ccz_pack_live_planes_rows_f16), (_ptr(plan[0]), _ptr(plan[1]))
             stem, tail = L.ccz_conv3x3_stem_f16_live, (Bp * 90 if g16 else -(-B // 8) * 8 * 90, 1 | lay, _ptr(plan[1]), 0, 1)
+        if chunk_major:
+            stem = L.ccz_conv3x3_stem_g16c_f16 if plan is None else L.ccz_conv3x3_stem_g16c_f16_live
         _lib.check(pack(s, _ptr(leaf_input), _ptr(x64), B, *gather))
         _lib.check(stem(s, _ptr(x64), _ptr(self.stem_w64_g16 if g16 else self.stem_w64), _ptr(self.stem_b32), _ptr(y), *tail))
         return y
@@ -447,13 +490,16 @@
             plan = None
         g16 = path == "g16"
         if path in ("g16", "nhwc"):
-            x = self._stem_fused(leaf_input, plan, g16)
+            cm = g16 and self._g16c(-(-B // 16) * 16)
+            x = self._stem_fused(leaf_input, plan, g16, cm)
             probe = self.__dict__.get("tower_probe")
             if probe is not None:
                 p0, p1 = torch.cuda.Event(enable_timing=True), torch.cuda.Event(enable_timing=True)
                 p0.record()
             heads = self._head_buffers(x.shape[0], x.device)[:2] if (g16 and self.opt.fused_last and self._fused_heads_ok(x)) else None
-            x = self._tower_fused(x, plan, g16, heads)
+            if cm and heads is None:
+                raise RuntimeError("chunk-major tower without the heads in its last layer")
+            x = self._tower_fused(x, plan, g16, heads, cm)
             if probe is not None:
                 p1.record()
                 probe.append((p0, p1))
@@ -481,6 +527,11 @@
                     x = self._epilogue(F.conv2d(y, self.ws[i + 1], None, padding=1), self.bs[i + 1], x)
         return self._heads(x, B, g16, plan, return_logits)
 
+    def _g16c(self, Bp: int) -> bool:
+        o = self.opt
+        return bool(o.chunk_major and o.one_launch and o.quad and o.fused_last and o.fused_heads and hasattr(self, "head_w32")
+                    and self.dtype == torch.float16 and self._edge(Bp, True))
+
     def _fused_heads_ok(self, x) -> bool:
         return bool(self.opt.fused_heads and hasattr(self, "head_w32") and x.is_cuda and x.dtype == torch.float16 and x.shape[1] == 256
                     and x.is_contiguous(memory_format=torch.channels_last))
diff --git a/include/cczero.h b/include/cczero.h
--- a/include/cczero.h
+++ b/include/cczero.h
@@ -304,6 +304,21 @@
                                void *pol_dev, void *val_dev, int64_t n_pixels, int32_t flags,
                                const int32_t *live_rows_dev, int32_t part, int32_t n_parts);
 
+int ccz_conv3x3_c256_g16c_f16(void *stream, const void *x_dev, const void *w_dev, const void *bias_f32_dev,
+                              const void *residual_dev, void *y_dev, int64_t n_pixels, int32_t relu);
+int ccz_conv3x3_c256_g16c_f16_live(void *stream, const void *x_dev, const void *w_dev, const void *bias_f32_dev,
+                                   const void *residual_dev, void *y_dev, int64_t n_pixels, int32_t relu,
+                                   const int32_t *live_rows_dev, int32_t part, int32_t n_parts);
+int ccz_conv3x3_stem_g16c_f16(void *stream, const void *x64_dev, const void *w_dev, const void *bias_f32_dev,
+                              void *y_dev, int64_t n_pixels, int32_t relu);
+int ccz_conv3x3_stem_g16c_f16_live(void *stream, const void *x64_dev, const void *w_dev, const void *bias_f32_dev,
+                                   void *y_dev, int64_t n_pixels, int32_t relu, const int32_t *live_rows_dev,
+                                   int32_t part, int32_t n_parts);
+int ccz_conv3x3_c256_heads_g16c_f16(void *stream, const void *x_dev, const void *w_dev, const void *bias_f32_dev,
+                                    const void *residual_dev, const void *head_w32_dev, const void *head_bias32_f32_dev,
+                                    void *pol_dev, void *val_dev, int64_t n_pixels, int32_t flags,
+                                    const int32_t *live_rows_dev, int32_t part, int32_t n_parts);
+
 #ifdef __cplusplus
 }
 #endif
diff --git a/profiles/g16c_layer_ab.py b/profiles/g16c_layer_ab.py
--- /dev/null
+++ b/profiles/g16c_layer_ab.py
@@ -0,0 +1,108 @@
+import argparse
+import collections
+import csv
+import ctypes as C
+import glob
+import json
+import os
+import statistics
+import sys
+
+ROOT = os.path.dirname(os.path.dirname(os.path.abspath(__file__)))
+FLAGS = 1 | 64 | 128 | 512 | 65536
+
+
+def summarize(d):
+    acc = collections.defaultdict(lambda: collections.defaultdict(lambda: [0.0, set()]))
+    for f in glob.glob(os.path.join(d, "**", "*counter_collection.csv"), recursive=True):
+        for r in csv.DictReader(open(f)):
+            name = r["Kernel_Name"]
+            arm = "g16c" if "g16c_one_quad" in name else "rows" if "g16_one_quad" in name else None
+            if arm:
+                a = acc[arm][r["Counter_Name"]]
+                a[0] += float(r["Counter_Value"])
+                a[1].add(r["Dispatch_Id"])
+    out = {arm: {c: {"per_launch": v[0] / len(v[1]), "launches": len(v[1])} for c, v in sorted(cs.items())} for arm, cs in acc.items()}
+    if "rows" in out and "g16c" in out:
+        out["g16c_over_rows"] = {c: out["g16c"][c]["per_launch"] / out["rows"][c]["per_launch"] for c in out["rows"] if c in out["g16c"] and out["rows"][c]["per_launch"]}
+    return out
+
+
+def main():
+    ap = argparse.ArgumentParser()
+    ap.add_argument("parent", nargs="?")
+    ap.add_argument("--boards", type=int, nargs="+", default=[4096, 3696])
+    ap.add_argument("--rounds", type=int, default=7)
+    ap.add_argument("--iters", type=int, default=10)
+    ap.add_argument("--pmc", type=int, default=0, help="1: three launches per arm at the first board count, no timing (for a rocprofv3 --pmc pass)")
+    ap.add_argument("--summarize")
+    ap.add_argument("--out")
+    a = ap.parse_args()
+    if a.summarize:
+        print(json.dumps(summarize(a.summarize), indent=1))
+        return
+    import torch
+    sys.path.insert(0, ROOT)
+    from chinesechesszero_amd.net import g16_to_g16c, g16c_to_g16, pack_conv_weights_g16
+
+    def load(path, probe):
+        L = C.CDLL(os.path.abspath(path))
+        for f in ("ccz_conv3x3_c256_f16",) + (("ccz_conv3x3_c256_g16c_f16",) if probe else ()):
+            getattr(L, f).restype = C.c_int
+            getattr(L, f).argtypes = [C.c_void_p] * 6 + [C.c_int64, C.c_int32]
+        return L
+
+    parent = load(a.parent, False)
+    mine = load(os.path.join(ROOT, "chinesechesszero_amd", "libcczero.so"), True)
+    dev = torch.device("cuda:0")
+    s = C.c_void_p(torch.cuda.current_stream().cuda_stream)
+    result = {"flags": FLAGS, "rounds": a.rounds, "iters": a.iters, "layers": []}
+    for B in a.boards[:1] if a.pmc else a.boards:
+        assert B % 16 == 0
+        G = B // 16
+        g = torch.Generator(device="cpu").manual_seed(1)
+        x = torch.relu(torch.randn(G, 1440, 256, generator=g) * 0.5).to(dev).half()
+        res = torch.relu(torch.randn(G, 1440, 256, generator=g) * 0.5).to(dev).half()
+        w = (torch.randn(256, 3, 3, 256, generator=g) * 0.03).to(dev).half()
+        bias = (torch.randn(256, generator=g) * 0.1).to(dev)
+        wp = pack_conv_weights_g16(w)
+        xc, rc = g16_to_g16c(x), g16_to_g16c(res)
+        arms = [("rows", parent.ccz_conv3x3_c256_f16, x, res), ("rows2", mine.ccz_conv3x3_c256_f16, x, res),
+                ("g16c", mine.ccz_conv3x3_c256_g16c_f16, xc, rc)]
+        ys = [torch.zeros_like(x) for _ in arms]
+
+        def run(i):
+            _, fn, xin, rin = arms[i]
+            assert fn(s, xin.data_ptr(), wp.data_ptr(), bias.data_ptr(), rin.data_ptr(), ys[i].data_ptr(), B * 90, FLAGS) == 0
+
+        for rep in range(3 if a.pmc else 1):
+            for i in range(len(arms)):
+                run(i)
+        torch.cuda.synchronize()
+        same = [bool(torch.equal(g16c_to_g16(y) if n == "g16c" else y, ys[0])) for (n, *_), y in zip(arms, ys)]
+        layer = {"boards": B, "outputs_identical_to_rows": same, "nonzero_out": int((ys[0] != 0).sum().item())}
+        if not a.pmc:
+            times = {n: [] for n, *_ in arms}
+            for rnd in range(a.rounds):
+                order = list(range(len(arms)))
+                order = order[rnd % len(arms):] + order[:rnd % len(arms)]
+                for i in order:
+                    e0, e1 = torch.cuda.Event(enable_timing=True), torch.cuda.Event(enable_timing=True)
+                    run(i)
+                    e0.record()
+                    for _ in range(a.iters):
+                        run(i)
+                    e1.record()
+                    torch.cuda.synchronize()
+                    times[arms[i][0]].append(e0.elapsed_time(e1) / a.iters * 1e3)
+            layer["us"] = {n: {"median": statistics.median(t), "min": min(t), "max": max(t), "all": [round(v, 2) for v in t]} for n, t in times.items()}
+        result["layers"].append(layer)
+        assert all(same), "outputs differ"
+    txt = json.dumps(result, indent=1)
+    print(txt)
+    if a.out:
+        open(a.out, "w").write(txt + "\n")
+
+
+if __name__ == "__main__":
+    main()
```
